# Illumina/Pisces

Hardware: AMD Instinct MI355X
Metric: candidate loci/s at 500x depth (higher is better)
Workload: dtype int32 counts + f64 likelihoods; 1 GPU; BASELINE config 2: synthetic 100000 loci x 500x amplicon pileup, SNV-only, gVCF, per GPU per step; device-resident packed tuples; depth=500, ring_batches=6, tile_loci=56, parallelism=interval-shard x1

## Files before the change

pisces_amd/csrc/device_math.hip.h:

```cpp
#pragma once
#include <hip/hip_runtime.h>
#include <stdint.h>

#include "../../include/pisces_hip.h"

namespace pisces {

struct DeviceParams {
    int32_t min_bq, noise_level, max_vq, min_vq, vq_filter, min_cov, low_depth_filter;
    int32_t min_gq, max_gq, low_gq_filter, sb_model, filter_single_strand, include_ref, emit_zero_cov;
    int32_t rmxn_max_len, rmxn_min_rep;
    float min_freq, vf_filter, gt_min_freq, target_lod, nocall_thr, rmxn_freq_limit;
    double sb_threshold;
    double err_q;
    double err_sb;
    double ln10;
    unsigned long long* totals;
    const double* q_to_p_lut;
    int32_t q_to_p_n;
    const double* gq_tail;
    int32_t gq_tail_a, gq_tail_cov;
    int32_t refs_only;
    int32_t variants_only;
    const int16_t* vq_tab;
    const double* sb_tab;
    const double* sb0_tab;
    const int16_t* gq_cap;
    int32_t vq_tab_k, sb_tab_k, tab_cov;
    const uint32_t* dirty_bits;
    int32_t dirty_first, dirty_n;
    int32_t* folded_out;
    int32_t folded_first, folded_n;
};

__device__ __forceinline__ bool locus_is_dirty(const DeviceParams& P, int pos)
{
    if (!P.dirty_bits) return false;
    const unsigned rel = (unsigned)(pos - P.dirty_first);
    return rel < (unsigned)P.dirty_n && ((P.dirty_bits[rel >> 5] >> (rel & 31u)) & 1u) != 0u;
}

__device__ __forceinline__ double lanczos_approximation(double p)
{
    double x = p;
    double tmp = x + 5.5;
    tmp = tmp - (x + 0.5) * log(tmp);
    double ser = 1.000000000190015 + 76.18009172947146 / (p + 1.0);
    ser -= 86.50532032941678 / (p + 2.0);
    ser += 24.01409824083091 / (p + 3.0);
    ser -= 1.231739572450155 / (p + 4.0);
    ser += 0.001208650973866179 / (p + 5.0);
    ser -= 5.395239384953E-06 / (p + 6.0);
    return (log(2.506628274631001 * ser / x) - tmp);
}

__device__ __forceinline__ double stirling_approximation(double n)
{
    return (0.5 * log(2.0 * 3.14159265358979323846) + (0.5 + n) * log(n) - n);
}

__device__ inline double gamma_continued_fraction(double a, double x, double g)
{
    const double kFpmin = 1.0E-50, kEpsilon = 1.0E-20;
    double b = x + 1.0 - a;
    double c = 1.0 / kFpmin;
    double d = 1.0 / b;
    double h = d;
    int i;
    for (i = 1; i <= 300; i++) {
        double an = i * (a - i);
        b += 2.0;
        d = an * d + b;
        if (fabs(d) < kFpmin) d = kFpmin;
        c = b + an / c;
        if (fabs(c) < kFpmin) c = kFpmin;
        d = 1.0 / d;
        double del = d * c;
        h *= del;
        if (fabs(del - 1.0) < kEpsilon) break;
    }
    if (i > 300) return -1.0;
    return exp(a * log(x) - x - g) * h;
}

__device__ inline double gamma_series(double a, double x, double g)
{
    const double kEpsilon = 1.0E-20;
    double retval = -1.0;
    if (x == 0.0) return 0.0;
    if (x < 0.0) return retval;
    double sum = 1.0 / a;
    double del = sum;
    bool done = false;
    for (int i = 1; i <= 300 && !done; i += 4) {
        const double ap0 = a + (double)i;
        const double q0 = x / ap0, q1 = x / (ap0 + 1.0), q2 = x / (ap0 + 2.0), q3 = x / (ap0 + 3.0);
        del *= q0; sum += del;
        if (fabs(del) < fabs(sum) * kEpsilon) { done = true; break; }
        del *= q1; sum += del;
        if (fabs(del) < fabs(sum) * kEpsilon) { done = true; break; }
        del *= q2; sum += del;
        if (fabs(del) < fabs(sum) * kEpsilon) { done = true; break; }
        del *= q3; sum += del;
        if (fabs(del) < fabs(sum) * kEpsilon) { done = true; break; }
    }
    if (done) retval = sum * exp(a * log(x) - x - g);
    return retval;
}

__device__ inline double incomplete_gamma_function(double a, double x)
{
// ... 69 lines not shown
    *gamma_ln_a = gl;
    double ax = (a * log(x)) - x - gl;
    if (ax < -709.78271289338399) return a < x ? 1.0 : 0.0;

    if (x <= 1 || x <= a) {
        double r2 = a, c2 = 1, ans2 = 1;
        do {
            r2 = r2 + 1;
            c2 = c2 * x / r2;
            ans2 += c2;
        } while ((c2 / ans2) > epsilon);
        return exp(ax) * ans2 / a;
    }

    int c = 0;
    double y = 1 - a;
    double z = x + y + 1;
    double p3 = 1, q3 = x, p2 = x + 1, q2 = z * x;
    double ans = p2 / q2;
    double error;
    do {
        c++;
        y += 1;
        z += 2;
        double yc = y * c;
        double p = (p2 * z) - (p3 * yc);
        double q = (q2 * z) - (q3 * yc);
        if (q != 0) {
            double nextans = p / q;
            error = fabs((ans - nextans) / nextans);
            ans = nextans;
        } else {
            error = 1;
        }
        p3 = p2; p2 = p; q3 = q2; q2 = q;
        if (fabs(p) > big) {
            p3 *= bigInv; p2 *= bigInv; q3 *= bigInv; q2 *= bigInv;
        }
    } while (error > epsilon);
    return 1.0 - (exp(ax) * ans);
}

struct QParams { int32_t max_vq; double ln10; };
__device__ inline int32_t poisson_qscore_core(int32_t callCount, int32_t coverage, double err, const QParams P)
{
    if ((callCount <= 0) || (coverage <= 0)) return 0;
    double callCountMinusOne = callCount - 1;
    double callCountDouble = callCount;
    double lambda = err * coverage;
    if (P.max_vq <= 110 && callCount >= 3 && callCountDouble >= 2.0 * lambda) {
        const double km1 = callCountMinusOne;
        const double need = ((double)P.max_vq + 1.0) * 0.23025850929940458 + 1e-3;
        const double r = km1 / lambda;
        if (km1 * (ln_lower_bound(r) - 1.0) >= need) return P.max_vq;
        if (km1 * (log(r) - 1.0) >= need) return P.max_vq;
    }
    double gamma_ln_k;
    double pValue = 1 - (1.0 - mathnet_gamma_lower_regularized(callCountMinusOne + 1, lambda, &gamma_ln_k));
    double rawQ;
    if (pValue > 0) {
        rawQ = p_to_q(pValue);
    } else {
        int k = (int)callCountMinusOne;
        const double fl = (k >= 171 && gamma_ln_k == gamma_ln_k) ? gamma_ln_k : mathnet_factorial_ln(k);
        double A = -lambda + (k * log(lambda)) - fl;
        double correction = (callCountDouble - lambda) / callCountDouble;
        rawQ = -10.0 * (A - log(2.0 * correction)) / P.ln10;
    }
    double qScore = fmin((double)P.max_vq, rawQ);
    qScore = fmax(qScore, 0.0);
    return (int32_t)rint(qScore);
}
__device__ inline int32_t poisson_qscore_e(int32_t callCount, int32_t coverage, double err, const DeviceParams& P)
{
    const QParams q = {P.max_vq, P.ln10};
    return poisson_qscore_core(callCount, coverage, err, q);
}
__device__ inline int32_t poisson_qscore(int32_t callCount, int32_t coverage, const DeviceParams& P)
{
    return poisson_qscore_e(callCount, coverage, P.err_q, P);
}
__device__ __forceinline__ double ln_ratio_lower_bound(double a, double x) { return (double)(ilogb(a) - ilogb(x) - 1) * 0.6931471805; }

__device__ __forceinline__ bool poisson_qscore_try(int32_t callCount, int32_t coverage, const DeviceParams& P, int32_t& vq)
{
    if ((callCount <= 0) || (coverage <= 0)) { vq = 0; return true; }
    if (P.vq_tab && callCount < P.vq_tab_k && coverage < P.tab_cov) {
        vq = P.vq_tab[(uint32_t)callCount * (uint32_t)P.tab_cov + (uint32_t)coverage];
        return true;
    }
    const double lambda = P.err_q * coverage;
    if (P.max_vq <= 110 && callCount >= 3 && (double)callCount >= 2.0 * lambda) {
        const double km1 = callCount - 1;
        const double need = ((double)P.max_vq + 1.0) * 0.23025850929940458 + 1e-3;
        if (km1 * (ln_ratio_lower_bound(km1, lambda) - 1.0) >= need) { vq = P.max_vq; return true; }
    }
    return false;
}

constexpr int32_t kNoLevel = (int32_t)0x80000000;
__device__ inline int32_t window_level(double sumOfBaseQuality, int totalCoverage)
{
    if (totalCoverage == 0) return kNoLevel;
    const double mean = sumOfBaseQuality / (double)totalCoverage;
    if (!(mean > 0.0) || isinf(mean)) return kNoLevel;
    return (int32_t)p_to_q(mean);
}
__device__ inline double window_err_of_level(int32_t level, const DeviceParams& P) { return level == kNoLevel ? -1.0 : q_to_p_int(level, P); }
__device__ inline double window_err(double sumOfBaseQuality, int totalCoverage, const DeviceParams& P)
{
    return window_err_of_level(window_level(sumOfBaseQuality, totalCoverage), P);
}
__device__ __forceinline__ int16_t noise_level_field(int32_t level) { return level == kNoLevel ? (int16_t)-32768 : (int16_t)level; }

struct SbStats { double var_gt_zero, false_pos, coverage, support; };

__device__ __noinline__ double mathnet_beta_regularized(double a, double b, double x)
{
    const double bt = (x == 0.0 || x == 1.0) ? 0.0
                      : exp(mathnet_gamma_ln(a + b) - mathnet_gamma_ln(a) - mathnet_gamma_ln(b) + (a * log(x)) + (b * log(1.0 - x)));
    const bool symmetryTransformation = x >= (a + 1.0) / (a + b + 2.0);
    const double eps = 1.1102230246251565e-16;
    const double fpmin = 4.9406564584124654e-324 / eps;
    if (symmetryTransformation) { x = 1.0 - x; const double swap = a; a = b; b = swap; }
    const double qab = a + b, qap = a + 1.0, qam = a - 1.0;
    double c = 1.0, d = 1.0 - (qab * x / qap);
    if (fabs(d) < fpmin) d = fpmin;
    d = 1.0 / d;
    double h = d;
    for (int m = 1, m2 = 2; m <= 50000; m++, m2 += 2) {
        double aa = m * (b - m) * x / ((qam + m2) * (a + m2));
        d = 1.0 + (aa * d); if (fabs(d) < fpmin) d = fpmin;
        c = 1.0 + (aa / c); if (fabs(c) < fpmin) c = fpmin;
        d = 1.0 / d;
        h *= d * c;
        aa = -(a + m) * (qab + m) * x / ((a + m2) * (qap + m2));
        d = 1.0 + (aa * d); if (fabs(d) < fpmin) d = fpmin;
        c = 1.0 + (aa / c); if (fabs(c) < fpmin) c = fpmin;
        d = 1.0 / d;
        const double del = d * c;
        h *= del;
        if (fabs(del - 1.0) <= eps) break;
    }
    return symmetryTransformation ? 1.0 - (bt * h / a) : bt * h / a;
}

template <bool kDiploidOk = false>
__device__ inline SbStats sb_create_stats(double support, double coverage, double noiseFreq, double minVariantFreq, int model)
{
    SbStats st;
    st.support = support;
    st.coverage = coverage;
    const double minDetectableSNP = (kDiploidOk && model == PISCES_SB_DIPLOID) ? minVariantFreq : noiseFreq;
    if (support == 0) {
        if (model == PISCES_SB_POISSON) {
            st.false_pos = 1;
            st.var_gt_zero = 0;
        } else {
            st.var_gt_zero = pow(1 - minDetectableSNP, coverage);
            st.false_pos = 1 - st.var_gt_zero;
        }
    } else if (kDiploidOk && model == PISCES_SB_DIPLOID) {
        const double frequency = coverage == 0 ? 0.0 : support / coverage;
        if (frequency >= minDetectableSNP) {
            st.var_gt_zero = 1;
            st.false_pos = 0;
        } else {
            const int n = (int)coverage;
            const double k = floor(support);
            const double cdf = support < 0.0 ? 0.0 : support > n ? 1.0 : mathnet_beta_regularized(n - k, k + 1, 1 - minDetectableSNP);
            st.var_gt_zero = fmax(cdf, 0.0);
            st.false_pos = fmax(0.0, 1 - poisson_cdf_sb(support, coverage * 0.1));
        }
    } else {
        st.var_gt_zero = fmax(0.0, poisson_cdf_sb(support - 1, coverage * noiseFreq));
        st.false_pos = fmax(0.0, 1 - st.var_gt_zero);
    }
    return st;
}

struct SbResult { double bias_score; int acceptable, var_both, cov_both; };

template <bool kDiploidOk = false>
__device__ __forceinline__ SbStats sb_stats_of(int which, const int32_t cov[3], const int32_t sup[3], const DeviceParams& P)
{
    const int s = which == 0 ? sup[0] + sup[1] + sup[2] : (which == 1 ? sup[0] + sup[2] / 2 : sup[1] + sup[2] / 2);
    const int c = which == 0 ? cov[0] + cov[1] + cov[2] : (which == 1 ? cov[0] + cov[2] / 2 : cov[1] + cov[2] / 2);
    return sb_create_stats<kDiploidOk>((double)s, (double)c, P.err_sb, (double)P.min_freq, P.sb_model);
}

__device__ __forceinline__ SbResult sb_combine(const SbStats& overall, const SbStats& fwd, const SbStats& rev, const DeviceParams& P)
{
    double forwardBias = (fwd.var_gt_zero * rev.false_pos) / overall.var_gt_zero;
    double reverseBias = (rev.var_gt_zero * fwd.false_pos) / overall.var_gt_zero;
    if (overall.var_gt_zero == 0) {
        forwardBias = 1;
        reverseBias = 1;
    }
    SbResult r;
    r.bias_score = forwardBias > reverseBias ? forwardBias : reverseBias;
    r.cov_both = (fwd.coverage > 0) && (rev.coverage > 0);
    r.var_both = (fwd.support > 0) && (rev.support > 0);
    if (!r.cov_both) r.bias_score = 0;
    r.acceptable = r.bias_score < P.sb_threshold;
    return r;
}

template <bool kDiploidOk = false>
__device__ inline SbResult strand_bias(const int32_t cov[3], const int32_t sup[3], const DeviceParams& P)
{
    const SbStats overall = sb_stats_of<kDiploidOk>(0, cov, sup, P);
    __builtin_amdgcn_sched_barrier(0);
    const SbStats fwd = sb_stats_of<kDiploidOk>(1, cov, sup, P);
    __builtin_amdgcn_sched_barrier(0);
    const SbStats rev = sb_stats_of<kDiploidOk>(2, cov, sup, P);
    __builtin_amdgcn_sched_barrier(0);
    return sb_combine(overall, fwd, rev, P);
}

__device__ __forceinline__ float frequency_f(int32_t support, int32_t coverage)
{
    if (coverage == 0) return 0.0f;
    float f = (float)support / (float)coverage;
    return f < 1.0f ? f : 1.0f;
}

__device__ inline int32_t somatic_genotype(bool isReference, int32_t cov, int32_t support, int32_t refSupport,
                                           const DeviceParams& P)
{
    if (cov < P.min_cov) return isReference ? PISCES_GT_REF_LIKE_NOCALL : PISCES_GT_ALT_LIKE_NOCALL;
    float freq = frequency_f(support, cov);
    if (!isReference) {
        if (frequency_f(refSupport, cov) < P.gt_min_freq) {
            if ((1 - freq) > P.gt_min_freq) return PISCES_GT_ALT_AND_NOCALL;
            return PISCES_GT_HOM_ALT;
        }
        return PISCES_GT_HET_ALT_REF;
    }
    if (freq < P.gt_min_freq) return PISCES_GT_REF_LIKE_NOCALL;
    if ((1 - freq) > P.gt_min_freq) return PISCES_GT_REF_AND_NOCALL;
    return PISCES_GT_HOM_REF;
}

__device__ __noinline__ double poisson_cdf_out_of_line(double num_occurrences, double expected)
{
    return poisson_cdf(num_occurrences, expected);
}

struct GqTail { double p2; bool used, floor; };
__device__ __forceinline__ GqTail somatic_gq_tail(int32_t genotype, int32_t cov, int32_t support, const DeviceParams& P)
{
    GqTail t = {0.0, false, false};
    if (cov == 0) return t;
    if ((genotype == PISCES_GT_HOM_REF) || (genotype == PISCES_GT_HOM_ALT)) {
        const float nonAlleleObservationsF = (1.0f - frequency_f(support, cov)) * (float)cov;
        const float expectedNonAllelObservationsF = P.target_lod * (float)cov;
        t.used = true;
        if (nonAlleleObservationsF >= expectedNonAllelObservationsF) { t.floor = true; return t; }
        const int ai = (int)((double)nonAlleleObservationsF + 1.0);
        if (P.gq_tail && ai >= 1 && ai < P.gq_tail_a && cov < P.gq_tail_cov)
            t.p2 = P.gq_tail[(size_t)ai * (size_t)P.gq_tail_cov + (size_t)cov];
        else
            t.p2 = poisson_cdf_out_of_line(nonAlleleObservationsF, expectedNonAllelObservationsF);
    }
    return t;
}

__device__ __forceinline__ int32_t somatic_gq_finish(int32_t genotype, int32_t variantQ, int32_t cov, const GqTail& t,
                                                     const DeviceParams& P)
{
    double rawQ = variantQ;
    bool noCall = (genotype == PISCES_GT_ALT12_LIKE_NOCALL || genotype == PISCES_GT_ALT_LIKE_NOCALL ||
                   genotype == PISCES_GT_REF_LIKE_NOCALL);
    if ((cov == 0) || noCall) return P.min_gq;
    if (t.used) {
        if (t.floor) return P.min_gq;
        double p1 = q_to_p_int(variantQ, P);
        rawQ = p_to_q(p1 + t.p2);
    }
    double qScore = fmin((double)P.max_gq, rawQ);
    qScore = fmax(qScore, (double)P.min_gq);
    return (int32_t)rint(qScore);
}

__device__ inline int32_t somatic_gq(int32_t genotype, int32_t variantQ, int32_t cov, int32_t support,
                                     const DeviceParams& P)
{
    const GqTail t = somatic_gq_tail(genotype, cov, support, P);
    return somatic_gq_finish(genotype, variantQ, cov, t, P);
}

__device__ __forceinline__ bool sb_stats_try(int32_t support, int32_t coverage, const DeviceParams& P, SbStats& st)
{
    st.support = (double)support;
    st.coverage = (double)coverage;
    if (support == 0) {
        if (P.sb_model == PISCES_SB_POISSON) {
            st.false_pos = 1;
            st.var_gt_zero = 0;
            return true;
        }
        if (!(P.sb0_tab && coverage >= 0 && coverage < P.tab_cov)) return false;
        st.var_gt_zero = P.sb0_tab[coverage];
        st.false_pos = 1 - st.var_gt_zero;
        return true;
    }
    if (P.sb_tab && support > 0 && support < P.sb_tab_k && coverage >= 0 && coverage < P.tab_cov) {
        st.var_gt_zero = P.sb_tab[(uint32_t)support * (uint32_t)P.tab_cov + (uint32_t)coverage];
    } else {
        const double a = (double)support, x = (double)coverage * P.err_sb;
        if (!(x > 0.0 && 2.0 * x <= a && a * (ln_ratio_lower_bound(a, x) - 1.0) + x > 51.0)) return false;
        st.var_gt_zero = 1.0;
    }
    st.false_pos = fmax(0.0, 1 - st.var_gt_zero);
    return true;
}

__device__ __forceinline__ bool strand_bias_try(const int32_t cov[3], const int32_t sup[3], const DeviceParams& P, double& bias_score,
                                                int& acceptable, int& var_both, int& cov_both)
{
    const int s2 = sup[2] / 2, c2 = cov[2] / 2;
    const int sf = sup[0] + s2, sr = sup[1] + s2, cf = cov[0] + c2, cr = cov[1] + c2;
    SbStats overall, fwd, rev;
    const bool ok0 = sb_stats_try(sup[0] + sup[1] + sup[2], cov[0] + cov[1] + cov[2], P, overall);
    const bool ok1 = sb_stats_try(sf, cf, P, fwd);
    const bool ok2 = sb_stats_try(sr, cr, P, rev);
    double forwardBias = 0.0, reverseBias = 0.0;
    if (!(fwd.false_pos == 0.0 && rev.false_pos == 0.0 && overall.var_gt_zero > 0.0)) {
        forwardBias = (fwd.var_gt_zero * rev.false_pos) / overall.var_gt_zero;
        reverseBias = (rev.var_gt_zero * fwd.false_pos) / overall.var_gt_zero;
        if (overall.var_gt_zero == 0) {
            forwardBias = 1;
            reverseBias = 1;
        }
    }
    double score = forwardBias > reverseBias ? forwardBias : reverseBias;
    cov_both = (cf > 0) && (cr > 0);
    var_both = (sf > 0) && (sr > 0);
    if (!cov_both) score = 0;
    bias_score = score;
    acceptable = score < P.sb_threshold;
    return ok0 && ok1 && ok2;
}

__device__ __forceinline__ int32_t somatic_gq_index(int32_t genotype, int32_t cov, int32_t support, const DeviceParams& P)
{
    if (cov == 0 || !((genotype == PISCES_GT_HOM_REF) || (genotype == PISCES_GT_HOM_ALT))) return -1;
    const float nonAlleleObservationsF = (1.0f - frequency_f(support, cov)) * (float)cov;
    const float expectedNonAllelObservationsF = P.target_lod * (float)cov;
    if (nonAlleleObservationsF >= expectedNonAllelObservationsF) return -1;
    const int ai = (int)((double)nonAlleleObservationsF + 1.0);
    if (ai >= 1 && ai < P.gq_tail_a && cov < P.gq_tail_cov) return ai * P.gq_tail_cov + cov;
    return -1;
}
__device__ __forceinline__ bool somatic_gq_try(int32_t genotype, int32_t variantQ, int32_t cov, int32_t support, const DeviceParams& P,
                                               int32_t gq_index, int32_t gq_cap_value , int32_t& gq)
{
    const bool noCall = (genotype == PISCES_GT_ALT12_LIKE_NOCALL || genotype == PISCES_GT_ALT_LIKE_NOCALL || genotype == PISCES_GT_REF_LIKE_NOCALL);
    if ((cov == 0) || noCall) { gq = P.min_gq; return true; }
    if ((genotype == PISCES_GT_HOM_REF) || (genotype == PISCES_GT_HOM_ALT)) {
        if (gq_index >= 0 && variantQ == P.max_vq && P.gq_cap) { gq = gq_cap_value; return true; }
        const float nonAlleleObservationsF = (1.0f - frequency_f(support, cov)) * (float)cov;
        const float expectedNonAllelObservationsF = P.target_lod * (float)cov;
        if (nonAlleleObservationsF >= expectedNonAllelObservationsF) { gq = P.min_gq; return true; }
        return false;
    }
    double qScore = fmin((double)P.max_gq, (double)variantQ);
    qScore = fmax(qScore, (double)P.min_gq);
    gq = (int32_t)rint(qScore);
    return true;
}

struct AlleleTables {
    int32_t vq;
    double sb[3];
    int32_t gq_cap;
    int32_t gq_idx;
    uint32_t have;
};
__device__ __forceinline__ bool tables_complete(const DeviceParams& P) { return P.vq_tab && P.sb_tab && P.sb0_tab && P.gq_cap; }

__device__ __forceinline__ AlleleTables request_allele_tables(bool isRef, int32_t support, int32_t total, int32_t refsup, const int32_t cov[3],
                                                              const int32_t sup[3], const DeviceParams& P)
{
    AlleleTables t;
    const uint32_t tab_cov = (uint32_t)P.tab_cov;
    const bool vq_in = support > 0 && total > 0 && support < P.vq_tab_k && total < P.tab_cov;
    const int16_t vq_v = P.vq_tab[vq_in ? (uint32_t)support * tab_cov + (uint32_t)total : 0u];
    const int s2 = sup[2] / 2, c2 = cov[2] / 2;
    const int ss[3] = {sup[0] + sup[1] + sup[2], sup[0] + s2, sup[1] + s2};
    const int cc[3] = {cov[0] + cov[1] + cov[2], cov[0] + c2, cov[1] + c2};
    double sb_v[3];
    uint32_t have = vq_in ? 1u : 0u;
#pragma unroll
    for (int w = 0; w < 3; w++) {
        const bool zero = ss[w] == 0;
        const bool in = zero ? (P.sb_model != PISCES_SB_POISSON && cc[w] >= 0 && cc[w] < P.tab_cov)
                             : (ss[w] > 0 && ss[w] < P.sb_tab_k && cc[w] >= 0 && cc[w] < P.tab_cov);
        const double* base = zero ? P.sb0_tab : P.sb_tab;
        const uint32_t idx = in ? (zero ? (uint32_t)cc[w] : (uint32_t)ss[w] * tab_cov + (uint32_t)cc[w]) : 0u;
        sb_v[w] = base[idx];
        have |= in ? (2u << w) : 0u;
    }
    t.gq_idx = somatic_gq_index(somatic_genotype(isRef, total, support, refsup, P), total, support, P);
    const int16_t gq_v = P.gq_cap[t.gq_idx >= 0 ? t.gq_idx : 0];
    t.vq = vq_v;
    t.sb[0] = sb_v[0]; t.sb[1] = sb_v[1]; t.sb[2] = sb_v[2];
    t.gq_cap = gq_v;
    t.have = have;
    return t;
}

__device__ __forceinline__ bool poisson_qscore_try(int32_t callCount, int32_t coverage, const DeviceParams& P, const AlleleTables& t, int32_t& vq)
{
    if ((callCount <= 0) || (coverage <= 0)) { vq = 0; return true; }
    if (t.have & 1u) { vq = t.vq; return true; }
    const double lambda = P.err_q * coverage;
    if (P.max_vq <= 110 && callCount >= 3 && (double)callCount >= 2.0 * lambda) {
        const double km1 = callCount - 1;
        const double need = ((double)P.max_vq + 1.0) * 0.23025850929940458 + 1e-3;
        if (km1 * (ln_ratio_lower_bound(km1, lambda) - 1.0) >= need) { vq = P.max_vq; return true; }
    }
    return false;
}

__device__ __forceinline__ bool sb_stats_try(int32_t support, int32_t coverage, const DeviceParams& P, bool have, double value, SbStats& st)
{
    st.support = (double)support;
    st.coverage = (double)coverage;
    if (support == 0) {
        if (P.sb_model == PISCES_SB_POISSON) {
            st.false_pos = 1;
            st.var_gt_zero = 0;
            return true;
        }
        if (!have) return false;
        st.var_gt_zero = value;
        st.false_pos = 1 - st.var_gt_zero;
        return true;
    }
    if (have) {
        st.var_gt_zero = value;
    } else {
        const double a = (double)support, x = (double)coverage * P.err_sb;
        if (!(x > 0.0 && 2.0 * x <= a && a * (ln_ratio_lower_bound(a, x) - 1.0) + x > 51.0)) return false;
        st.var_gt_zero = 1.0;
    }
    st.false_pos = fmax(0.0, 1 - st.var_gt_zero);
    return true;
}

__device__ __forceinline__ bool strand_bias_try(const int32_t cov[3], const int32_t sup[3], const DeviceParams& P, const AlleleTables& t,
                                                double& bias_score, int& acceptable, int& var_both, int& cov_both)
{
    const int s2 = sup[2] / 2, c2 = cov[2] / 2;
    const int sf = sup[0] + s2, sr = sup[1] + s2, cf = cov[0] + c2, cr = cov[1] + c2;
    SbStats overall, fwd, rev;
    const bool ok0 = sb_stats_try(sup[0] + sup[1] + sup[2], cov[0] + cov[1] + cov[2], P, (t.have & 2u) != 0, t.sb[0], overall);
    const bool ok1 = sb_stats_try(sf, cf, P, (t.have & 4u) != 0, t.sb[1], fwd);
    const bool ok2 = sb_stats_try(sr, cr, P, (t.have & 8u) != 0, t.sb[2], rev);
    double forwardBias = 0.0, reverseBias = 0.0;
    if (!(fwd.false_pos == 0.0 && rev.false_pos == 0.0 && overall.var_gt_zero > 0.0)) {
        forwardBias = (fwd.var_gt_zero * rev.false_pos) / overall.var_gt_zero;
        reverseBias = (rev.var_gt_zero * fwd.false_pos) / overall.var_gt_zero;
        if (overall.var_gt_zero == 0) {
            forwardBias = 1;
            reverseBias = 1;
        }
    }
    double score = forwardBias > reverseBias ? forwardBias : reverseBias;
    cov_both = (cf > 0) && (cr > 0);
    var_both = (sf > 0) && (sr > 0);
    if (!cov_both) score = 0;
    bias_score = score;
    acceptable = score < P.sb_threshold;
    return ok0 && ok1 && ok2;
}

__device__ __noinline__ int32_t poisson_qscore_out_of_line(int32_t callCount, int32_t coverage, double err, int32_t max_vq, double ln10)
{
    const QParams q = {max_vq, ln10};
    return poisson_qscore_core(callCount, coverage, err, q);
}
struct SbPair { double var_gt_zero, false_pos; };
__device__ __noinline__ SbPair sb_stats_out_of_line(double support, double coverage, double noiseFreq, int model)
{
    const SbStats st = sb_create_stats<false>(support, coverage, noiseFreq, 0.0, model);
    SbPair p = {st.var_gt_zero, st.false_pos};
    return p;
}
__device__ inline SbResult strand_bias_out_of_line(const int32_t cov[3], const int32_t sup[3], const DeviceParams& P)
{
    const int s2 = sup[2] / 2, c2 = cov[2] / 2;
    SbStats st[3];
#pragma unroll 1
    for (int which = 0; which < 3; which++) {
        const int s = which == 0 ? sup[0] + sup[1] + sup[2] : (which == 1 ? sup[0] + s2 : sup[1] + s2);
        const int c = which == 0 ? cov[0] + cov[1] + cov[2] : (which == 1 ? cov[0] + c2 : cov[1] + c2);
        const SbPair p = sb_stats_out_of_line((double)s, (double)c, P.err_sb, P.sb_model);
        st[which].var_gt_zero = p.var_gt_zero;
        st[which].false_pos = p.false_pos;
        st[which].support = (double)s;
        st[which].coverage = (double)c;
    }
    return sb_combine(st[0], st[1], st[2], P);
}

__device__ inline int rmxn_run(const uint8_t* ref, int64_t lo, int64_t hi, int64_t start, uint8_t base)
{
    int64_t back = start;
    while (back - 1 >= lo && ref[back - 1 - lo] == base) back--;
    int n = 0;
    int64_t cur = back;
    while (cur < hi && ref[cur - lo] == base) { n++; cur++; }
    return n;
}

__device__ inline bool rmxn_should_filter_snv(const uint8_t* ref, int64_t win_lo, int64_t win_hi, int32_t position,
                                              uint8_t refBase, uint8_t altBase, float freq, const DeviceParams& P)
{
    if (P.rmxn_max_len < 1) return false;
    if (freq >= P.rmxn_freq_limit) return false;
    int c1 = rmxn_run(ref, win_lo, win_hi, (int64_t)position - 1, refBase);
    int i1 = rmxn_run(ref, win_lo, win_hi, (int64_t)position, altBase);
    int i2 = rmxn_run(ref, win_lo, win_hi, (int64_t)position - 1, altBase);
    int c2 = i1 > i2 ? i1 : i2;
    return (c1 < c2 ? c1 : c2) >= P.rmxn_min_rep;
}

__device__ inline int rmxn_run_lds(const uint8_t* win, int n, int start, uint8_t base)
{
    int back = start;
    while (back - 1 >= 0 && win[back - 1] == base) back--;
    int cnt = 0;
    int cur = back;
    while (cur < n && win[cur] == base) { cnt++; cur++; }
    return cnt;
}

__device__ inline bool rmxn_should_filter_snv_lds(const uint8_t* win, int n, int idx ,
                                                  uint8_t refBase, uint8_t altBase, float freq, const DeviceParams& P)
{
    if (P.rmxn_max_len < 1) return false;
    if (freq >= P.rmxn_freq_limit) return false;
    if (idx >= 4 && idx + 4 < n) {
        const bool l1 = win[idx - 1] == refBase, l2 = win[idx - 2] == refBase, l3 = win[idx - 3] == refBase, l4 = win[idx - 4] == refBase;
        const bool r1 = win[idx + 1] == refBase, r2 = win[idx + 2] == refBase, r3 = win[idx + 3] == refBase, r4 = win[idx + 4] == refBase;
        const int left = !l1 ? 0 : !l2 ? 1 : !l3 ? 2 : !l4 ? 3 : 4;
        const int right = !r1 ? 0 : !r2 ? 1 : !r3 ? 2 : !r4 ? 3 : 4;
        if (left < 4 && right < 4 && 1 + left + right < P.rmxn_min_rep) return false;
    }
    int c1 = rmxn_run_lds(win, n, idx, refBase);
    if (c1 < P.rmxn_min_rep) return false;
    int i1 = rmxn_run_lds(win, n, idx + 1, altBase);
    int i2 = rmxn_run_lds(win, n, idx, altBase);
    int c2 = i1 > i2 ? i1 : i2;
    return (c1 < c2 ? c1 : c2) >= P.rmxn_min_rep;
}

}
```

pisces_amd/csrc/kernels.hip.h:

```cpp
#pragma once
#include <hip/hip_runtime.h>
#include <stdint.h>

#include "device_math.hip.h"
#include "genotype_core.h"

namespace pisces {

constexpr int kBlock = 256;
constexpr int kTile = 64;
constexpr int kFolded = 18;
constexpr int kUnroll = 8;
constexpr int kSlotsPerTile = 4 * kTile;
#ifndef PISCES_TOTAL_SHARDS
#define PISCES_TOTAL_SHARDS 64
#endif
constexpr int kTotalShards = PISCES_TOTAL_SHARDS;
constexpr int kTotalStride = 16;
constexpr int kRefMargin = 32;
constexpr int kRefWin = kTile + 2 * kRefMargin;
constexpr int kWaveRows = 32;
constexpr int kWaveRow = kTile;
constexpr int kWaveRegion = kWaveRows * kWaveRow;
constexpr int kQLutLds = 128;

typedef uint32_t u32x4 __attribute__((ext_vector_type(4)));

__device__ __forceinline__ int allele_of_rank(int k) { return k == 1 ? 2 : (k == 2 ? 1 : k); }
__device__ __forceinline__ int rank_of_allele(int a) { return a == 1 ? 2 : (a == 2 ? 1 : a); }

__device__ __forceinline__ int allele_type_of_base(uint8_t c)
{
    return c == 'A' ? 0 : c == 'G' ? 1 : c == 'C' ? 2 : c == 'T' ? 3 : 4;
}

__device__ __forceinline__ void accumulate_folded(int* hist, uint32_t t, uint32_t n_loci, uint32_t min_bq)
{
    uint32_t locus = PISCES_TUPLE_LOCUS(t);
    uint32_t dir = PISCES_TUPLE_DIR(t);
    uint32_t allele = PISCES_TUPLE_ALLELE(t);
    uint32_t qual = PISCES_TUPLE_QUAL(t);
    if (allele < 4u && qual < min_bq) allele = 4u;
    if (locus < n_loci && dir < 3u && allele < 6u) atomicAdd(&hist[(allele * 3u + dir) * kTile + locus], 1);
}

__device__ __forceinline__ void accumulate_wave(int* hist, uint32_t t, uint32_t min_bq_shifted)
{
    const uint32_t region = (t < min_bq_shifted) ? (uint32_t)(kWaveRegion * sizeof(int)) : 0u;
    const uint32_t off = (t & 0x1FFCu) | region;
    atomicAdd(reinterpret_cast<int*>(reinterpret_cast<char*>(hist) + off), 1);
}

template <typename Op>
__device__ __forceinline__ void stream_tuples(const uint32_t* __restrict__ tuples, int64_t begin, int64_t end, Op op)
{
    const int tid = threadIdx.x;
    int64_t abegin = (begin + 3) & ~(int64_t)3;
    int64_t aend = end & ~(int64_t)3;
    if (abegin > aend) { abegin = end; aend = end; }
    for (int64_t i = begin + tid; i < abegin; i += kBlock) op(tuples[i]);
    const u32x4* __restrict__ p4 = reinterpret_cast<const u32x4*>(tuples + abegin);
    const int64_t n4 = (aend - abegin) >> 2;
    for (int64_t i = tid; i < n4; i += (int64_t)kBlock * kUnroll) {
        u32x4 v[kUnroll];
#pragma unroll
        for (int u = 0; u < kUnroll; u++) {
            int64_t j = i + (int64_t)u * kBlock;
            v[u] = j < n4 ? __builtin_nontemporal_load(&p4[j]) : (u32x4){~0u, ~0u, ~0u, ~0u};
        }
#pragma unroll
        for (int u = 0; u < kUnroll; u++) {
            op(v[u].x); op(v[u].y); op(v[u].z); op(v[u].w);
        }
    }
    for (int64_t i = aend + tid; i < end; i += kBlock) op(tuples[i]);
}

__device__ __forceinline__ void copy_record(PiscesCalledAllele* dst, const PiscesCalledAllele* src)
{
    const unsigned long long sb = (unsigned long long)__double_as_longlong(src->strand_bias_score);
    uint4* dp = reinterpret_cast<uint4*>(dst);
    dp[0] = make_uint4((uint32_t)src->position, (uint32_t)src->total_coverage, (uint32_t)src->allele_support, (uint32_t)src->reference_support);
    dp[1] = make_uint4((uint32_t)src->num_no_calls, (uint32_t)src->coverage_by_dir[0], (uint32_t)src->coverage_by_dir[1], (uint32_t)src->coverage_by_dir[2]);
    dp[2] = make_uint4((uint32_t)src->support_by_dir[0], (uint32_t)src->support_by_dir[1], (uint32_t)src->support_by_dir[2], (uint32_t)src->variant_qscore);
    dp[3] = make_uint4((uint32_t)sb, (uint32_t)(sb >> 32), (uint32_t)(uint16_t)src->genotype_qscore | ((uint32_t)(uint16_t)src->noise_level << 16), (uint32_t)src->filter_bits | ((uint32_t)src->info << 16));
}

struct PointCounts {
    int cov[3], sup[3];
    int total, nocalls, refsup, support;
};

struct HistBlock {
    static __device__ __forceinline__ int idx(int a, int d, int l) { return (a * 3 + d) * kTile + l; }
};
struct HistWave {
    static __device__ __forceinline__ int idx(int a, int d, int l) { return (a * 4 + d) * kWaveRow + (int)PISCES_TUPLE_COLUMN(l, d); }
};

struct HistLinear {
    static __device__ __forceinline__ int idx(int a, int d, int l) { return (a * 4 + d) * kWaveRow + l; }
};

struct LocusCounts { int h[6][3]; };

template <typename H = HistBlock>
__device__ __forceinline__ LocusCounts load_counts(const int* hist, int l)
{
    LocusCounts lc;
#pragma unroll
    for (int k = 0; k < kFolded; k++) lc.h[k / 3][k % 3] = hist[H::idx(k / 3, k % 3, l)];
    return lc;
}

template <typename HistWave = pisces::HistWave>
__device__ __forceinline__ LocusCounts load_counts_wave(const int* hist, int l)
{
    LocusCounts lc;
#pragma unroll
    for (int d = 0; d < 3; d++) {
        int low = 0;
#pragma unroll
        for (int a = 0; a < 5; a++) low += hist[kWaveRegion + HistWave::idx(a, d, l)];
#pragma unroll
        for (int a = 0; a < 4; a++) lc.h[a][d] = hist[HistWave::idx(a, d, l)];
        lc.h[PISCES_ALLELE_N][d] = hist[HistWave::idx(PISCES_ALLELE_N, d, l)] + low;
        lc.h[PISCES_ALLELE_DEL][d] = hist[HistWave::idx(PISCES_ALLELE_DEL, d, l)] + hist[kWaveRegion + HistWave::idx(PISCES_ALLELE_DEL, d, l)];
    }
    return lc;
}

__device__ __forceinline__ PointCounts point_counts_of(const LocusCounts& lc, int allele, bool isRef, int refType, int gapped)
{
    PointCounts c;
    const int (&h)[6][3] = lc.h;
    c.total = 0; c.nocalls = 0; c.refsup = 0;
    const int supAllele = isRef ? refType : allele;
#pragma unroll
    for (int d = 0; d < 3; d++) {
        c.cov[d] = h[PISCES_ALLELE_A][d] + h[PISCES_ALLELE_C][d] + h[PISCES_ALLELE_G][d] + h[PISCES_ALLELE_T][d] +
                   h[PISCES_ALLELE_DEL][d];
        c.total += c.cov[d];
        c.nocalls += h[PISCES_ALLELE_N][d];
        c.sup[d] = 0;
    }
#pragma unroll
    for (int a = 0; a < 6; a++) {
        if (a == refType && a < PISCES_ALLELE_N) c.refsup += h[a][0] + h[a][1] + h[a][2];
        if (a == supAllele) { c.sup[0] = h[a][0]; c.sup[1] = h[a][1]; c.sup[2] = h[a][2]; }
    }
    c.support = c.sup[0] + c.sup[1] + c.sup[2];
    if (isRef) { c.support -= gapped; if (c.support < 0) c.support = 0; }
    else { c.refsup -= gapped; if (c.refsup < 0) c.refsup = 0; }
    return c;
}

template <typename H = HistBlock>
__device__ __forceinline__ PointCounts point_counts(const int* hist, int l, int allele, bool isRef, int refType, int gapped)
{
    return point_counts_of(load_counts<H>(hist, l), allele, isRef, refType, gapped);
}

__device__ __forceinline__ bool variant_passes_frequency(const PointCounts& c, const DeviceParams& P)
{
    if (c.total < P.min_cov && !P.include_ref) return false;
    if (c.total != 0 && frequency_f(c.support, c.total) < P.min_freq) return false;
    return true;
}

struct GqPre { int32_t idx, val; };
template <bool kMemo = false>
__device__ inline bool finish_allele(const PointCounts& c, int pos, int a, bool isRef, int rt, int vq, const SbResult& sb,
                                     const uint8_t* __restrict__ ref, int64_t win_lo, int64_t win_hi, const DeviceParams& P,
                                     PiscesCalledAllele& r, const uint8_t* s_refwin, int s_refidx,
                                     const GqTail* pre_tail = nullptr, const GqPre* pre_gq = nullptr,
                                     const int32_t* window_level_ = nullptr )
{
    const float freq = frequency_f(c.support, c.total);
    const float allReads = (float)(c.total + c.nocalls);
    const float fractionNoCalls = (allReads == 0.0f) ? 0.0f : ((float)c.nocalls / allReads);
    uint32_t filters = 0;
    if (P.low_depth_filter >= 0 && c.total < P.low_depth_filter) filters |= 1u << PISCES_FILTER_LOW_DEPTH;
    if (P.vq_filter >= 0 && vq < P.vq_filter && c.total != 0) filters |= 1u << PISCES_FILTER_LOW_VARIANT_QSCORE;
    if (!isRef) {
        if (P.nocall_thr >= 0.0f && fractionNoCalls > P.nocall_thr) filters |= 1u << PISCES_FILTER_NO_CALL;
        if (!sb.acceptable || (P.filter_single_strand && !sb.var_both)) filters |= 1u << PISCES_FILTER_STRAND_BIAS;
        auto base_of = [](int code) { return (uint8_t)((0x54434741u >> (8 * code)) & 0xFFu); };
        if (rt < 4 && a < 4) {
            const bool hit = (s_refwin && P.rmxn_min_rep <= kRefMargin)
                                 ? rmxn_should_filter_snv_lds(s_refwin, kRefWin, s_refidx, base_of(rt), base_of(a), freq, P)
                                 : rmxn_should_filter_snv(ref, win_lo, win_hi, pos, base_of(rt), base_of(a), freq, P);
            if (hit) filters |= 1u << PISCES_FILTER_RMXN;
        }
        if (P.vf_filter >= 0.0f && freq < P.vf_filter) filters |= 1u << PISCES_FILTER_LOW_VARIANT_FREQUENCY;
    }
    const int gt = somatic_genotype(isRef, c.total, c.support, c.refsup, P);
    int gq;
    if (kMemo) {
        GqPre g;
        if (pre_gq) g = *pre_gq;
        else {
            g.idx = somatic_gq_index(gt, c.total, c.support, P);
            g.val = (g.idx >= 0 && P.gq_cap) ? (int32_t)P.gq_cap[g.idx] : 0;
        }
        if (!somatic_gq_try(gt, vq, c.total, c.support, P, g.idx, g.val, gq)) return false;
    } else {
        gq = pre_tail ? somatic_gq_finish(gt, vq, c.total, *pre_tail, P) : somatic_gq(gt, vq, c.total, c.support, P);
    }
    if (P.low_gq_filter >= 0 && (float)gq < (float)P.low_gq_filter) filters |= 1u << PISCES_FILTER_LOW_GENOTYPE_QUALITY;

    r.position = pos;
    r.total_coverage = c.total;
    r.allele_support = c.support;
    r.reference_support = c.refsup;
    r.num_no_calls = c.nocalls;
    r.coverage_by_dir[0] = c.cov[0]; r.coverage_by_dir[1] = c.cov[1]; r.coverage_by_dir[2] = c.cov[2];
    r.support_by_dir[0] = c.sup[0]; r.support_by_dir[1] = c.sup[1]; r.support_by_dir[2] = c.sup[2];
    r.variant_qscore = vq;
    r.strand_bias_score = sb.bias_score;
    r.genotype_qscore = (int16_t)gq;
    r.noise_level = c.support > 0 ? (window_level_ ? noise_level_field(*window_level_) : (int16_t)P.noise_level) : (int16_t)0;
    r.filter_bits = (uint16_t)filters;
    r.info = PISCES_INFO_PACK(gt, isRef ? PISCES_CAT_REFERENCE : PISCES_CAT_SNV, rt, isRef ? rt : a, sb.acceptable, sb.var_both,
                              sb.cov_both);
    return true;
}

template <bool kDiploidOk = false, bool kFinishAnyway = false>
__device__ inline bool process_point_allele(const PointCounts& c, int pos, int a, bool isRef, int rt,
                                             const uint8_t* __restrict__ ref, int64_t win_lo, int64_t win_hi,
                                             const DeviceParams& P, PiscesCalledAllele& r,
                                             const uint8_t* s_refwin = nullptr, int s_refidx = 0, const GqTail* pre_tail = nullptr,
                                             const int32_t* window_level_ = nullptr )
{
    bool callable = true;
    if (!isRef && !variant_passes_frequency(c, P)) {
        if (!kFinishAnyway) return false;
        callable = false;
    }
    int vq = 0;
    if (window_level_) {
        const double werr = window_err_of_level(*window_level_, P);
        if (c.support > 0 && c.total != 0 && werr >= 0.0) vq = poisson_qscore_e(c.support, c.total, werr, P);
    } else if (c.support > 0 && c.total != 0) {
        vq = poisson_qscore(c.support, c.total, P);
    }
    if (!isRef && vq < P.min_vq) {
        if (!kFinishAnyway) return false;
        callable = false;
    }
    SbResult sb = {0.0, 0, 0, 0};
    if (c.support > 0) sb = strand_bias<kDiploidOk>(c.cov, c.sup, P);
    finish_allele(c, pos, a, isRef, rt, vq, sb, ref, win_lo, win_hi, P, r, s_refwin, s_refidx, pre_tail, nullptr, window_level_);
    return callable;
}

struct VarScratch {
    int vq[kTile * 4];
    double ov_var[kTile * 4], fw_var[kTile * 4], fw_fp[kTile * 4], rv_var[kTile * 4], rv_fp[kTile * 4];
};

__device__ inline void call_roles(const int* hist, const uint32_t* gapped , const int32_t* s_lvl , const PiscesTile& tile,
                                  int tile_index, const uint8_t* __restrict__ ref, int32_t ref_start, int64_t ref_len,
                                  PiscesCalledAllele* __restrict__ records, PiscesTileResult* __restrict__ tile_result,
                                  const DeviceParams& P, uint8_t* s_mask ,
                                  const uint8_t* s_refwin , VarScratch* vs)
{
    const int wave = threadIdx.x >> 6;
    if (wave == 3) return;
    const int l = threadIdx.x & 63;
    const int pos = tile.start_position + l;
    const uint8_t refb = s_refwin[kRefMargin + l];
    const bool in_ref = l < tile.n_loci && refb != 0;
    const int rt = in_ref ? allele_type_of_base(refb) : PISCES_ALLELE_N;
    const int64_t win_lo = (int64_t)ref_start - 1, win_hi = win_lo + ref_len;
    const int g = gapped ? (int)gapped[l] : 0;
    PiscesCalledAllele* const slots = records + (int64_t)tile_index * kSlotsPerTile + l * 4;

    uint32_t pass_mask = 0;
    if (in_ref && rt < 4 && !P.refs_only && !locus_is_dirty(P, pos)) {
        for (int k = 0; k < 4; k++) {
            const int a = allele_of_rank(k);
            if (a == rt) continue;
            if (hist[(a * 3 + 0) * kTile + l] + hist[(a * 3 + 1) * kTile + l] + hist[(a * 3 + 2) * kTile + l] == 0) continue;
            const PointCounts c = point_counts(hist, l, a, false, rt, g);
            if (variant_passes_frequency(c, P)) pass_mask |= 1u << k;
        }
    }
    const bool tile_has_variants = __ballot(pass_mask != 0) != 0ull;
    if (!tile_has_variants && wave != 0) return;

    bool ref_emitted = false;
    int ref_rank = 0;
    if (wave == 0) {
        if (in_ref && P.include_ref) {
            int all = 0;
#pragma unroll
            for (int c = 0; c < kFolded; c++) all += hist[c * kTile + l];
            if (P.emit_zero_cov || all > 0) {
                const int a = (rt < 4) ? rt : PISCES_ALLELE_N;
                ref_rank = (rt < 4) ? rank_of_allele(rt) : 0;
                const PointCounts c = point_counts(hist, l, a, true, rt, g);
                PiscesCalledAllele rec;
                (void)process_point_allele<true>(c, pos, a, true, rt, ref, win_lo, win_hi, P, rec, s_refwin, kRefMargin + l, nullptr, s_lvl ? &s_lvl[l] : nullptr);
                copy_record(&slots[ref_rank], &rec);
                ref_emitted = true;
            }
// ... 164 lines not shown
#pragma unroll
        for (int u = 0; u < kWaveUnroll; u++) { op(v[u].x); op(v[u].y); op(v[u].z); op(v[u].w); }
    };
    const bool streams = (uint32_t)wid < nb;
    if (NW == 2) {
        if (streams) load(cur, (uint32_t)__builtin_amdgcn_readfirstlane(wid));
        __builtin_amdgcn_sched_barrier(0);
        pre();
    } else {
        pre();
        if (streams) load(cur, (uint32_t)__builtin_amdgcn_readfirstlane(wid));
    }
    for (int64_t i = begin + tid; i < abegin; i += 64 * NW) op(tuples[i]);
    if (streams) {
        uint32_t b = (uint32_t)__builtin_amdgcn_readfirstlane(wid);
        const uint32_t m = (nb - b + NW - 1) / NW;
        for (uint32_t p = (m - 1) / 2; p > 0; p--) {
            load(nxt, b + NW);
            __builtin_amdgcn_sched_barrier(0);
            consume(cur);
            __builtin_amdgcn_sched_barrier(0);
            load(cur, b + 2 * NW);
            __builtin_amdgcn_sched_barrier(0);
            consume(nxt);
            __builtin_amdgcn_sched_barrier(0);
            b += 2 * NW;
        }
        if (((m - 1) & 1u) != 0) {
            load(nxt, b + NW);
            __builtin_amdgcn_sched_barrier(0);
            consume(cur);
            __builtin_amdgcn_sched_barrier(0);
#pragma unroll
            for (int u = 0; u < kWaveUnroll; u++) cur[u] = nxt[u];
            b += NW;
        }
        if (b == nb - 1 && (n4 % kBatch)) {
#pragma unroll
            for (int u = 0; u < kWaveUnroll; u++)
                if (b * kBatch + (uint32_t)u * 64u + (uint32_t)lane >= n4) cur[u] = (u32x4){~0u, ~0u, ~0u, ~0u};
        }
        consume(cur);
    }
    for (int64_t i = aend + tid; i < end; i += 64 * NW) op(tuples[i]);
}

__device__ __forceinline__ void wave_lds_sync()
{
    __builtin_amdgcn_fence(__ATOMIC_SEQ_CST, "workgroup");
    __builtin_amdgcn_wave_barrier();
}

template <typename H = HistWave>
__device__ __forceinline__ uint32_t slow_alleles(const int* hist, const uint8_t* s_refwin, uint32_t slow, int l, int pos, int rt, int ref_rank,
                                                 const uint8_t* __restrict__ ref, int64_t win_lo, int64_t win_hi, PiscesCalledAllele* slots,
                                                 const DeviceParams& P)
{
    uint32_t called = 0;
    const int ref_a = (rt < 4) ? rt : PISCES_ALLELE_N;
#pragma unroll 1
    for (int k = 0; k < 5; k++) {
        if (!((slow >> k) & 1u)) continue;
        const bool isRef = k == 4;
        const int a = isRef ? ref_a : allele_of_rank(k);
        const LocusCounts lc = load_counts_wave<H>(hist, l);
        const PointCounts c = point_counts_of(lc, a, isRef, rt, 0);
        int vq = 0;
        if (c.support > 0 && c.total != 0) vq = poisson_qscore_out_of_line(c.support, c.total, P.err_q, P.max_vq, P.ln10);
        if (!isRef && vq < P.min_vq) continue;
        SbResult sb = {0.0, 0, 0, 0};
        if (c.support > 0) sb = strand_bias_out_of_line(c.cov, c.sup, P);
        PiscesCalledAllele r;
        (void)finish_allele<false>(c, pos, a, isRef, rt, vq, sb, ref, win_lo, win_hi, P, r, s_refwin, kRefMargin + l);
        copy_record(&slots[isRef ? ref_rank : k], &r);
        if (!isRef) called |= 1u << k;
    }
    return called;
}

template <int NW, typename H = HistWave>
__device__ __forceinline__ void call_phase_wave(const int* hist, const uint8_t* s_refwin, uint8_t* s_vmask, const PiscesTile& tile, const int t,
                                                const int l, const int wid, const uint8_t* __restrict__ ref, const int32_t ref_start,
                                                const int64_t ref_len, PiscesCalledAllele* __restrict__ records,
                                                PiscesTileResult* __restrict__ tile_results, const DeviceParams& P
#ifdef PISCES_TIMING
                                                , const long long tc0, const long long tc1
#endif
                                                )
{
    const int pos = tile.start_position + l;
    const uint8_t refb = s_refwin[kRefMargin + l];
    const bool in_ref = l < tile.n_loci && refb != 0;
    const int rt = in_ref ? allele_type_of_base(refb) : PISCES_ALLELE_N;
    const int64_t win_lo = (int64_t)ref_start - 1, win_hi = win_lo + ref_len;
    auto slot_of = [&](int k) { return records + ((int64_t)t * kSlotsPerTile + l * 4 + k); };
    const bool dirty = locus_is_dirty(P, pos);
    const LocusCounts lc = load_counts_wave<H>(hist, l);
    const bool ref_wave = wid == 0, var_wave = wid == NW - 1;
    if (P.folded_out && ref_wave && l < tile.n_loci) {
        const unsigned rel = (unsigned)(pos - P.folded_first);
        if (rel < (unsigned)P.folded_n) {
            int32_t* const dst = P.folded_out + (size_t)rel * PISCES_FOLDED_PER_LOCUS;
#pragma unroll
            for (int a = 0; a < 6; a++)
#pragma unroll
                for (int d = 0; d < 3; d++) dst[a * 3 + d] = lc.h[a][d];
        }
    }

    const bool tabs = tables_complete(P);
    auto fast_allele = [&](const PointCounts& c, int a, bool isRef, PiscesCalledAllele& rec) -> bool {
        int vq = 0;
        double sb_score = 0.0;
        int sb_ok = 0, sb_var = 0, sb_cov = 0;
        if (!tabs) return false;
        const AlleleTables tb = request_allele_tables(isRef, c.support, c.total, c.refsup, c.cov, c.sup, P);
        if (c.support > 0 && c.total != 0 && !poisson_qscore_try(c.support, c.total, P, tb, vq)) return false;
        if (!isRef && vq < P.min_vq) return true;
        if (c.support > 0 && !strand_bias_try(c.cov, c.sup, P, tb, sb_score, sb_ok, sb_var, sb_cov)) return false;
        const GqPre g = {tb.gq_idx, tb.gq_cap};
        const SbResult sb = {sb_score, sb_ok, sb_var, sb_cov};
        if (!finish_allele<true>(c, pos, a, isRef, rt, vq, sb, ref, win_lo, win_hi, P, rec, s_refwin, kRefMargin + l, nullptr, &g)) return false;
        return true;
    };
    bool ref_emitted = false;
    int ref_rank = 0;
    uint32_t slow = 0;
    uint32_t vmask = 0;
    const int ref_a = (rt < 4) ? rt : PISCES_ALLELE_N;
    if (ref_wave) {
        const PointCounts c = point_counts_of(lc, ref_a, true, rt, 0);
        if (in_ref && P.include_ref && !P.variants_only && (P.emit_zero_cov || c.total + c.nocalls > 0)) {
            ref_rank = (rt < 4) ? rank_of_allele(rt) : 0;
            ref_emitted = true;
            PiscesCalledAllele rec;
            if (fast_allele(c, ref_a, true, rec)) copy_record(slot_of(ref_rank), &rec);
            else slow |= 16u;
        }
    }
#ifdef PISCES_TIMING
    const long long tcA = wall_clock64();
#endif
    if (var_wave && in_ref && rt < 4 && !P.refs_only && !dirty) {
#pragma unroll 1
        for (int k = 0; k < 4; k++) {
            const int a = allele_of_rank(k);
            if (a == rt) continue;
            const PointCounts c = point_counts_of(lc, a, false, rt, 0);
            if (c.support == 0) continue;
            if (!variant_passes_frequency(c, P)) continue;
            PiscesCalledAllele r;
            r.position = 0;
            if (!fast_allele(c, a, false, r)) { slow |= 1u << k; continue; }
            if (r.position == 0) continue;
            copy_record(slot_of(k), &r);
            vmask |= 1u << k;
        }
    }
    if (__builtin_expect(__ballot(slow != 0) != 0ull, 0))
        vmask |= slow_alleles<H>(hist, s_refwin, slow, l, pos, rt, ref_rank, ref, win_lo, win_hi, records + ((int64_t)t * kSlotsPerTile + l * 4), P);
    if (NW == 2) {
        if (var_wave) s_vmask[l] = (uint8_t)vmask;
        __syncthreads();
        if (!ref_wave) return;
        vmask = s_vmask[l];
    }
#ifdef PISCES_TIMING
    const long long tcB = wall_clock64();
#endif

    const uint32_t valid = vmask ? vmask : (ref_emitted ? (1u << ref_rank) : 0u);
    int n_surv = 0, n_var = 0;
#pragma unroll
    for (int k = 0; k < 4; k++) {
        n_surv += __popcll(__ballot((valid >> k) & 1u));
        n_var += __popcll(__ballot((vmask >> k) & 1u));
    }
    const int n_call_total = n_var + __popcll(__ballot(ref_emitted));
    const int n_loci_called = __popcll(__ballot(valid != 0));
    uint32_t word = valid << ((l & 7) * 4);
    word |= __shfl_xor(word, 1, 64);
    word |= __shfl_xor(word, 2, 64);
    word |= __shfl_xor(word, 4, 64);
    PiscesTileResult* const tile_result = &tile_results[t];
    if ((l & 7) == 0) tile_result->valid[l >> 3] = word;
    if (l == 0) {
        tile_result->record_begin = t * kSlotsPerTile;
        tile_result->n_records = n_surv;
        tile_result->n_candidate_loci = n_loci_called;
        tile_result->n_called = n_call_total;
        if (P.totals) {
            unsigned long long* tt = P.totals + (size_t)(t % kTotalShards) * kTotalStride;
            atomicAdd(&tt[0], (unsigned long long)n_surv);
            atomicAdd(&tt[1], (unsigned long long)n_loci_called);
            atomicAdd(&tt[2], (unsigned long long)n_call_total);
            atomicAdd(&tt[3], 1ull);
        }
#ifdef PISCES_TIMING
        const long long tc2 = wall_clock64();
        tile_result->record_begin = (int)(tc0 & 0x3FFFFFFF);
        tile_result->n_records = (int)(tc1 & 0x3FFFFFFF);
        tile_result->n_candidate_loci = (int)(tc2 & 0x3FFFFFFF);
        tile_result->n_called = (int)__builtin_amdgcn_s_getreg(63492);
        tile_result->valid[0] = __builtin_amdgcn_s_getreg(63508);
        tile_result->valid[1] = 0;
        tile_result->valid[2] = (uint32_t)(tcA - tc1);
        tile_result->valid[3] = (uint32_t)(tcB - tcA);
        tile_result->valid[4] = 0;
        tile_result->valid[5] = (uint32_t)(tc2 - tcB);
#endif
    }
}

template <int NW>
__global__ __launch_bounds__(64 * NW, NW == 1 ? PISCES_WAVE_OCC : PISCES_WAVE2_OCC) void call_tiles_wave_kernel(
    const uint32_t* __restrict__ tuples, const PiscesTile* __restrict__ tiles, int32_t n_tiles,
    const uint8_t* __restrict__ ref, int32_t ref_start, int64_t ref_len, PiscesCalledAllele* __restrict__ records,
    PiscesTileResult* __restrict__ tile_results, DeviceParams P, const DeviceParams* __restrict__ Pd )
{
    __shared__ __attribute__((aligned(16))) int hist[2 * kWaveRegion];
    __shared__ uint8_t s_refwin[kRefWin];
    __shared__ uint8_t s_vmask[kTile];

    const int t = blockIdx.x;
    if (t >= n_tiles) return;
    const int l = threadIdx.x & 63, wid = threadIdx.x >> 6;
    const PiscesTile tile = tiles[t];
#ifdef PISCES_TIMING
    const long long tc0 = wall_clock64();
#endif
    auto setup = [&]() {
        int4* h4 = reinterpret_cast<int4*>(hist);
        for (int i = threadIdx.x; i < 2 * kWaveRegion / 4; i += 64 * NW) h4[i] = make_int4(0, 0, 0, 0);
        for (int i = threadIdx.x; i < kRefWin; i += 64 * NW) {
            const int64_t ri = (int64_t)tile.start_position - kRefMargin + i - ref_start;
            s_refwin[i] = (ri >= 0 && ri < ref_len) ? ref[ri] : (uint8_t)0;
        }
        __syncthreads();
    };

    {
        if (NW == 2) __builtin_amdgcn_s_setprio(3);
        const uint32_t min_bq_shifted = (uint32_t)min(max(P.min_bq, 0), 255) << 24;
        stream_tuples_wave<NW>(tuples, tile.tuple_begin, tile.tuple_end, l, wid, [&](uint32_t v) { accumulate_wave(hist, v, min_bq_shifted); }, setup);
    }
    __syncthreads();
    if (NW == 2) __builtin_amdgcn_s_setprio(0);
#ifdef PISCES_TIMING
    const long long tc1 = wall_clock64();
#endif

    call_phase_wave<NW>(hist, s_refwin, s_vmask, tile, t, l, wid, ref, ref_start, ref_len, records, tile_results, P
#ifdef PISCES_TIMING
                        , tc0, tc1
#endif
                        );
}

__global__ __launch_bounds__(256) void build_vq_tab_kernel(int16_t* __restrict__ tab, int32_t n_k, int32_t n_cov, DeviceParams P)
{
    const int64_t i = (int64_t)blockIdx.x * blockDim.x + threadIdx.x;
    if (i >= (int64_t)n_k * n_cov) return;
    tab[i] = (int16_t)poisson_qscore((int32_t)(i / n_cov), (int32_t)(i % n_cov), P);
}
__global__ __launch_bounds__(256) void build_sb_tab_kernel(double* __restrict__ tab, double* __restrict__ tab0, int32_t n_k, int32_t n_cov, DeviceParams P)
{
    const int64_t i = (int64_t)blockIdx.x * blockDim.x + threadIdx.x;
    if (i >= (int64_t)n_k * n_cov) return;
    const int k = (int)(i / n_cov), cov = (int)(i % n_cov);
    tab[i] = k >= 1 ? fmax(0.0, poisson_cdf_sb((double)k - 1, (double)cov * P.err_sb)) : 0.0;
    if (k == 0) tab0[cov] = pow(1 - P.err_sb, (double)cov);
}
__global__ __launch_bounds__(256) void build_gq_cap_kernel(int16_t* __restrict__ tab, const double* __restrict__ gq_tail, int32_t n_a, int32_t n_cov, DeviceParams P)
{
    const int64_t i = (int64_t)blockIdx.x * blockDim.x + threadIdx.x;
    if (i >= (int64_t)n_a * n_cov) return;
    if (i < n_cov) { tab[i] = 0; return; }
    double rawQ = p_to_q(q_to_p_int(P.max_vq, P) + gq_tail[i]);
    double qScore = fmin((double)P.max_gq, rawQ);
    qScore = fmax(qScore, (double)P.min_gq);
    tab[i] = (int16_t)rint(qScore);
}

__global__ __launch_bounds__(64) void totals_collect_kernel(unsigned long long* __restrict__ shards, unsigned long long* __restrict__ out_host, int reset)
{
    const int l = threadIdx.x;
    if (l < 4) {
        unsigned long long v = 0;
        for (int sh = 0; sh < kTotalShards; sh++) v += shards[sh * kTotalStride + l];
        out_host[l] = v;
    }
    if (reset)
        for (int i = l; i < kTotalShards * kTotalStride; i += 64) shards[i] = 0ull;
    __threadfence_system();
}

__global__ __launch_bounds__(256) void read_probe_kernel(const u32x4* __restrict__ p, int64_t n4, uint32_t* __restrict__ sink)
{
    uint32_t acc = 0;
    const int64_t stride = (int64_t)gridDim.x * blockDim.x * 8;
    for (int64_t i = (int64_t)blockIdx.x * blockDim.x * 8 + threadIdx.x; i < n4; i += stride) {
        u32x4 v[8];
#pragma unroll
        for (int u = 0; u < 8; u++) {
            const int64_t j = i + (int64_t)u * blockDim.x;
            v[u] = j < n4 ? __builtin_nontemporal_load(&p[j]) : (u32x4){0u, 0u, 0u, 0u};
        }
#pragma unroll
        for (int u = 0; u < 8; u++) acc ^= v[u].x ^ v[u].y ^ v[u].z ^ v[u].w;
    }
    if (acc == 0x9E3779B9u) *sink = acc;
}

__global__ __launch_bounds__(256) void read_probe_dword_kernel(const uint32_t* __restrict__ p, int64_t n, uint32_t* __restrict__ sink)
{
    uint32_t acc = 0;
    const int64_t stride = (int64_t)gridDim.x * blockDim.x * 8;
    for (int64_t i = (int64_t)blockIdx.x * blockDim.x * 8 + threadIdx.x; i < n; i += stride) {
        uint32_t v[8];
#pragma unroll
        for (int u = 0; u < 8; u++) {
            const int64_t j = i + (int64_t)u * blockDim.x;
            v[u] = j < n ? p[j] : 0u;
        }
#pragma unroll
        for (int u = 0; u < 8; u++) acc ^= v[u];
    }
    if (acc == 0x9E3779B9u) *sink = acc;
}

__global__ void build_gq_tail_kernel(double* __restrict__ table, int32_t n_a, int32_t n_cov, float target_lod)
{
    const int64_t i = (int64_t)blockIdx.x * blockDim.x + threadIdx.x;
    if (i >= (int64_t)n_a * n_cov) return;
    const int a = (int)(i / n_cov), cov = (int)(i % n_cov);
    const float expectedF = target_lod * (float)cov;
    table[i] = a >= 1 ? incomplete_gamma_function((double)a, (double)expectedF) : -1.0;
}

template <typename T, typename R>
__host__ __device__ inline R anchor_adjusted(const T* __restrict__ row, int minAnchor, int maxAnchor, bool fromEnd)
{
    const int wellAnchoredIndex = PISCES_ANCHOR_SIZE, numAnchorIndexes = PISCES_NUM_ANCHORS;
    const int trueMinAnchor = wellAnchoredIndex < minAnchor ? wellAnchoredIndex : minAnchor;
    int initialMaxAnchor = wellAnchoredIndex;
    if (maxAnchor >= 0) {
        if (maxAnchor >= wellAnchoredIndex) initialMaxAnchor = wellAnchoredIndex - 1;
        if (maxAnchor < wellAnchoredIndex) initialMaxAnchor = maxAnchor;
    }
    R tot = 0;
    if (fromEnd) {
        for (int i = trueMinAnchor; i <= initialMaxAnchor; i++) tot += row[numAnchorIndexes - i - 1];
        if (maxAnchor < 0)
            for (int i = 0; i < initialMaxAnchor; i++) tot += row[i];
// ... 751 lines not shown
```

pisces_amd/csrc/pisces_hip.hip:

```cpp
#include <hip/hip_runtime.h>
#include <hip/hip_ext.h>
#include <dlfcn.h>
#include <link.h>

#include <algorithm>
#include <array>
#include <cctype>
#include <memory>
#include <cmath>
#include <cstdio>
#include <cstdlib>
#include <cstring>
#include <deque>
#include <ctime>
#include <map>
#include <set>
#include <string>
#include <atomic>
#include <chrono>
#include <mutex>
#include <thread>
#include <unordered_map>
#include <unordered_set>
#include <vector>
// ... 186 lines not shown
            if (e == hipSuccess) e = hipStreamSynchronize(stream);
        }
        if (old) dev_free(old);
        p = fresh;
        cap = want;
        return e;
    }
    void release()
    {
        if (p) dev_free(p);
        p = nullptr;
        cap = 0;
    }
    void swap(DeviceBuf& o)
    {
        std::swap(p, o.p);
        std::swap(cap, o.cap);
    }
};

struct ReadSegment {
    DeviceBuf<uint8_t> blob;
    DeviceBuf<uint8_t> bases, quals, dirs, cop;
    DeviceBuf<uint8_t> codes;
    DeviceBuf<uint32_t> clen;
    DeviceBuf<ReadDesc> desc;
    DeviceBuf<ReadExt> ext;
    DeviceBuf<ReadDesc> frag;
    DeviceBuf<int32_t> grid;
    int64_t grid_base = 0, grid_n = 0;
    bool grid_ok = false;
    int32_t* state = nullptr;
    const uint8_t *v_bases = nullptr, *v_quals = nullptr, *v_dirs = nullptr, *v_cop = nullptr, *v_codes = nullptr;
    const uint32_t* v_clen = nullptr;
    int64_t n_reads = 0, n_bases = 0, n_ops = 0;
    int64_t n_floored = 0, n_floored_ops = 0;
    int32_t floor = 0;
    int32_t max_key = 0;
    bool open = false;
};

}

struct PiscesHip {
    PiscesHipConfig cfg;
    DeviceParams P;
    int device = 0;
    hipStream_t stream = nullptr;
    static constexpr int kLanes = 3;
    hipStream_t lane[kLanes] = {nullptr, nullptr, nullptr};
    hipEvent_t ev0 = nullptr, ev1 = nullptr;
    std::vector<hipEvent_t> ring;
    int32_t timing = 0;
    bool chain_timing = false;
    hipEvent_t ev_chain[4] = {nullptr, nullptr, nullptr, nullptr};
    bool chain_have[2] = {false, false};
    bool chain_enqueued_since = false;
    bool chain_add_open = false;
    int64_t ring_used = 0;
    int64_t launches_seen = 0;
    DeviceBuf<unsigned long long> d_totals;
    unsigned long long* h_totals = nullptr;
    bool foreign_stream_used = false;
    bool foreign_stream_ever = false;
    bool exact_total_called = false;
    DeviceBuf<PiscesTile> d_tiles_x;
    DeviceBuf<PiscesTileResult> d_tr_x;
    DeviceBuf<PiscesCalledAllele> d_rec_x;
    DeviceBuf<int32_t> d_cnt_x, d_off_x;
    int32_t* h_cnt_x = nullptr;
    bool tables_shareable = false;
    bool poisoned = false;
    std::string poison_why;
    uint8_t* h_prep = nullptr;
    DeviceBuf<double> d_qlut;
    DeviceBuf<ulonglong2> d_bq_lut;
    DeviceBuf<unsigned long long> d_sumq_fix;
    DeviceBuf<double> d_sumq;
    DeviceBuf<double> d_gq_tail;
    DeviceBuf<int16_t> d_vq_tab;
    DeviceBuf<double> d_sb_tab;
    DeviceBuf<double> d_sb0_tab;
    DeviceBuf<int16_t> d_gq_cap;
    DeviceBuf<DeviceParams> d_params;
    int n_cus = 256;
    void* comm = nullptr;
    int comm_world = 1;
    DeviceBuf<long long> d_summary;
    DeviceBuf<int32_t> d_offsets;
    DeviceBuf<PiscesCalledAllele> d_compact;
    DeviceBuf<PiscesGenotypePosteriors> d_post, d_post_compact;
    int kernel_variant = 4;
    std::string err;

    DeviceBuf<uint8_t> d_ref;
    std::vector<uint8_t> h_ref;
    int64_t ref_len = 0;
    DeviceBuf<DevCandidate> d_cands;
    DeviceBuf<uint8_t> d_alleles;
    DeviceBuf<PiscesCalledAllele> d_cand_records;
    DeviceBuf<uint8_t> d_cand_callable;
    int32_t* h_counts = nullptr;
    size_t h_counts_cap = 0;

    std::map<int32_t, BlockObs> blocks;
    int32_t last_block_key_cache = 0;
    BlockObs* last_block = nullptr;
    int32_t last_up_to_block_key = 0;
    std::unordered_map<int32_t, int32_t> gapped_mnv_ref;
    std::vector<HostCandidate> known_variants;
    bool exclude_mnvs_from_collapsing = false;
    std::vector<HostCandidate> forced;
    size_t n_forced_added = 0;
    std::set<std::string> forced_keys;
    std::set<int32_t> forced_positions;
    std::vector<std::pair<int32_t, int32_t>> intervals;
    int32_t own_lo = 1, own_hi = 0x7FFFFFFF;
    int64_t stats[4] = {0, 0, 0, 0};
    double prof[24] = {0};
    bool prof_on = false;
    int64_t pcie[4] = {0, 0, 0, 0};
    double host_time[4] = {0, 0, 0, 0};

    struct FlushResult {
        bool valid = false;
        int32_t up_to = 0;
        PiscesCalledAllele* view = nullptr;
        size_t n_view = 0;
        std::vector<PiscesCalledAllele> rows;
        std::vector<int32_t> index;
        std::vector<PiscesGenotypePosteriors> posteriors;
        std::vector<HostCandidate> cands;
        std::vector<PiscesCandidate> exported;
        std::vector<uint8_t> alleles;
        std::vector<int32_t> keys;
        int64_t called = 0, collapsed = 0;
        bool dropped = false;
        unsigned long long kept = 0;
        const PiscesCalledAllele* data() const { return view ? view : rows.data(); }
        size_t size() const { return view ? n_view : rows.size(); }
        void clear()
        {
            valid = dropped = false;
            view = nullptr;
            n_view = 0;
            rows.clear(); index.clear(); posteriors.clear(); cands.clear(); exported.clear(); alleles.clear(); keys.clear();
            called = collapsed = 0;
            kept = 0;
        }
    } result;

    DeviceBuf<int32_t> d_log_pos[2];
    DeviceBuf<uint32_t> d_log_tup[2];
    int log_cur = 0;
    DeviceBuf<unsigned long long> d_log_n;
    int64_t log_ub = 0;
    std::vector<long long> read_slots;
    std::vector<int32_t> found_slots_host;
    DeviceBuf<int32_t> d_flags;
    struct Stage {
        DeviceBuf<uint8_t> d;
        uint8_t* h = nullptr;
        size_t h_cap = 0;
        hipEvent_t done = nullptr;
        bool in_flight = false;
    } stage[2];
// ... 200 lines not shown
        int e2 = 0;
        const double m = std::frexp(x, &e2);
        const unsigned long long mant = (unsigned long long)std::ldexp(m, 53);
        const int shift = e2 - 53 + 2 * kSumqHalfBits;
        const unsigned __int128 v = shift >= 0 ? (unsigned __int128)mant << shift : (shift > -64 ? (unsigned __int128)mant >> (-shift) : (unsigned __int128)0);
        lut[(size_t)q].x = (unsigned long long)(v >> kSumqHalfBits);
        lut[(size_t)q].y = (unsigned long long)(v & (((unsigned __int128)1 << kSumqHalfBits) - 1));
    }
    hipError_t e = h->d_bq_lut.reserve(256);
    if (e == hipSuccess) e = hipMemcpy(h->d_bq_lut.p, lut.data(), 256 * sizeof(ulonglong2), hipMemcpyHostToDevice);
    return e;
}

static void store_view(PiscesHip* h, StoreView* V);
static hipError_t accumulate_tiles(PiscesHip* h, hipStream_t s, const uint32_t* d_tuples, const PiscesTile* d_tiles, int32_t n_tiles, bool with_sums,
                                   bool with_store = false)
{
    const size_t nc = (size_t)n_tiles * kTile * PISCES_COUNTS_PER_LOCUS;
    hipError_t e = h->d_counts.reserve(nc);
    if (e == hipSuccess && with_sums) e = h->d_sumq.reserve(nc);
    if (e == hipSuccess && with_sums) e = h->d_sumq_fix.reserve(2 * nc);
    if (e == hipSuccess && with_sums) e = ensure_quality_lut(h);
    if (e != hipSuccess) return e;
    (void)hipMemsetAsync(h->d_counts.p, 0, nc * sizeof(int32_t), s);
    if (with_sums) (void)hipMemsetAsync(h->d_sumq_fix.p, 0, 2 * nc * sizeof(unsigned long long), s);
    if (with_store && h->read_path == 1) {
        StoreView V;
        store_view(h, &V);
        const int split = (int)std::min<int64_t>(16, std::max<int64_t>(1, 2 * (int64_t)h->n_cus / std::max(n_tiles, 1)));
        hipLaunchKernelGGL(accumulate_store_tiles_kernel, dim3((unsigned)n_tiles, (unsigned)split), dim3(kBlock), 0, s, V, d_tuples, d_tiles, n_tiles, h->d_counts.p,
                           h->cfg.min_base_call_quality, with_sums ? h->d_sumq_fix.p : (unsigned long long*)nullptr,
                           with_sums ? (const ulonglong2*)h->d_bq_lut.p : (const ulonglong2*)nullptr);
    } else
    hipLaunchKernelGGL(accumulate_tiles_kernel, dim3((unsigned)n_tiles), dim3(kBlock), 0, s, d_tuples, d_tiles, n_tiles, h->d_counts.p,
                       h->cfg.min_base_call_quality, with_sums ? h->d_sumq_fix.p : (unsigned long long*)nullptr,
                       with_sums ? (const ulonglong2*)h->d_bq_lut.p : (const ulonglong2*)nullptr);
    if (with_sums)
        hipLaunchKernelGGL(finish_quality_sums_kernel, dim3((unsigned)((nc + 255) / 256)), dim3(256), 0, s, h->d_sumq_fix.p, h->d_sumq.p, (int64_t)nc);
    return hipGetLastError();
}

static DeviceParams make_params(const PiscesHipConfig& c)
{
    DeviceParams P;
    P.min_bq = c.min_base_call_quality;
    P.noise_level = c.noise_level;
    P.max_vq = c.max_variant_qscore;
    P.min_vq = c.min_variant_qscore;
    P.vq_filter = c.variant_qscore_filter;
    P.min_cov = c.min_coverage;
    P.low_depth_filter = c.low_depth_filter;
    P.min_gq = c.min_genotype_qscore;
    P.max_gq = c.max_genotype_qscore;
    P.low_gq_filter = c.low_gq_filter;
    P.sb_model = c.strand_bias_model;
    P.filter_single_strand = c.filter_single_strand;
    P.include_ref = c.include_reference_calls;
    P.emit_zero_cov = c.emit_zero_coverage_refs;
    P.rmxn_max_len = c.rmxn_max_repeat_length;
    P.rmxn_min_rep = c.rmxn_min_repetitions;
    P.min_freq = c.min_frequency;
    P.vf_filter = c.variant_freq_filter;
    P.gt_min_freq = c.genotype_min_freq_filter;
    P.target_lod = c.target_lod_frequency;
    P.nocall_thr = c.no_call_filter_threshold;
    P.rmxn_freq_limit = c.rmxn_frequency_limit;
    P.sb_threshold = (double)c.strand_bias_threshold;
    P.err_q = std::pow(10.0, -1 * (double)c.noise_level / 10.0);
    P.err_sb = std::pow(10.0, (double)((float)(-1 * c.noise_level) / 10.0f));
    P.ln10 = std::log(10.0);
    P.totals = nullptr;
    P.q_to_p_lut = nullptr;
    P.q_to_p_n = 0;
    P.gq_tail = nullptr;
    P.gq_tail_a = 0;
    P.gq_tail_cov = 0;
    P.refs_only = c.call_mnvs ? 1 : 0;
    P.variants_only = 0;
    P.vq_tab = nullptr;
    P.sb_tab = nullptr;
    P.sb0_tab = nullptr;
    P.gq_cap = nullptr;
    P.vq_tab_k = P.sb_tab_k = P.tab_cov = 0;
    P.dirty_bits = nullptr;
    P.dirty_first = P.dirty_n = 0;
    P.folded_out = nullptr;
    P.folded_first = P.folded_n = 0;
    return P;
}

template <typename R, typename F>
static R abi_guard(PiscesHip* h, F&& body)
{
    try {
        return body();
    } catch (const std::exception& e) {
        return (R)fail(h, PISCES_E_INTERNAL, std::string("exception inside the library: ") + e.what());
    } catch (...) {
        return (R)fail(h, PISCES_E_INTERNAL, "unknown exception inside the library");
    }
}

namespace {
struct TableSet {
    PiscesHipConfig cfg;
    int device = 0;
    DeviceBuf<double> gq_tail, sb_tab, sb0_tab;
    DeviceBuf<int16_t> vq_tab, gq_cap;
};
std::mutex g_tables_mu;
std::vector<TableSet*>& table_cache() { static std::vector<TableSet*>* v = new std::vector<TableSet*>(); return *v; }
TableSet* take_tables(const PiscesHipConfig& cfg, int device)
{
    std::lock_guard<std::mutex> lock(g_tables_mu);
    auto& v = table_cache();
    for (size_t i = 0; i < v.size(); i++)
        if (v[i]->device == device && std::memcmp(&v[i]->cfg, &cfg, sizeof(cfg)) == 0) {
            TableSet* t = v[i];
            v.erase(v.begin() + (std::ptrdiff_t)i);
            return t;
        }
    return nullptr;
}
void leave_tables(TableSet* t)
{
    std::lock_guard<std::mutex> lock(g_tables_mu);
    auto& v = table_cache();
    v.push_back(t);
    if (v.size() > 8) { delete v.front(); v.erase(v.begin()); }
}
}

extern "C" {

int32_t pisces_hip_abi_version(void) { return PISCES_HIP_ABI_VERSION; }

int32_t pisces_hip_default_config(PiscesHipConfig* c)
{
    return abi_guard<int32_t>((PiscesHip*)nullptr, [&]() -> int32_t {
    if (!c) return PISCES_E_INVALID_ARG;
    std::memset(c, 0, sizeof(*c));
    c->abi_version = PISCES_HIP_ABI_VERSION;
    c->min_base_call_quality = 20;
    c->noise_level = 20;
    c->max_variant_qscore = 100;
    c->min_variant_qscore = 20;
    c->variant_qscore_filter = 30;
    c->min_coverage = 10;
    c->low_depth_filter = 10;
    c->min_genotype_qscore = 0;
    c->max_genotype_qscore = 100;
    c->low_gq_filter = -1;
    c->strand_bias_model = PISCES_SB_EXTENDED;
    c->filter_single_strand = 0;
    c->include_reference_calls = 1;
    c->emit_zero_coverage_refs = 0;
    c->expect_stitched_reads = 0;
    c->tile_loci = kTile;
    c->block_size = 1000;
    c->min_frequency = 0.01f;
    c->variant_freq_filter = 0.01f;
    c->genotype_min_freq_filter = 0.01f;
    c->target_lod_frequency = 0.01f;
    c->strand_bias_threshold = 0.5f;
    c->no_call_filter_threshold = 0.6f;
    c->rmxn_max_repeat_length = 5;
    c->rmxn_min_repetitions = 9;
    c->rmxn_frequency_limit = 0.35f;
    c->collapse = 1;
    c->collapse_freq_threshold = 0.0f;
    c->collapse_freq_ratio_threshold = 0.5f;
    c->call_mnvs = 0;
    c->max_mnv_length = 3;
    c->max_gap_between_mnv = 1;
    c->noise_model = PISCES_NOISE_FLAT;
    c->ploidy = PISCES_PLOIDY_SOMATIC;
    c->diploid_snv_params[0] = c->diploid_indel_params[0] = 0.20f;
    c->diploid_snv_params[1] = c->diploid_indel_params[1] = 0.70f;
    c->diploid_snv_params[2] = c->diploid_indel_params[2] = 0.80f;
    return PISCES_OK;
    });
}

int32_t pisces_hip_destroy(PiscesHip* h);

int32_t pisces_hip_device_count(void)
{
    int ndev = 0;
    const hipError_t e = hipGetDeviceCount(&ndev);
    if (e != hipSuccess) { g_create_error = std::string("pisces_hip_device_count: ") + hipGetErrorString(e); return PISCES_E_DEVICE; }
    return ndev;
// ... 17 lines not shown
    hipError_t e = hipGetDeviceCount(&ndev);
    if (e != hipSuccess || ndev <= 0)
        return fail(nullptr, PISCES_E_DEVICE, std::string("pisces_hip_create: no HIP device: ") + hipGetErrorString(e));
    if (device < 0 || device >= ndev) return fail(nullptr, PISCES_E_INVALID_ARG, "pisces_hip_create: device index out of range");
    PiscesHip* h = new PiscesHip();
    h->cfg = *cfg;
    h->cfg.tile_loci = kTile;
    h->P = make_params(h->cfg);
    adaptive_default_params(h->adaptive);
    h->device = device;
    if ((e = hipSetDevice(device)) != hipSuccess || (e = hipStreamCreateWithFlags(&h->stream, hipStreamNonBlocking)) != hipSuccess ||
        (e = hipEventCreate(&h->ev0)) != hipSuccess || (e = hipEventCreate(&h->ev1)) != hipSuccess) {
        g_create_error = std::string("pisces_hip_create: ") + hipGetErrorString(e);
        delete h;
        return PISCES_E_DEVICE;
    }
    if ((e = h->d_totals.reserve((size_t)kTotalShards * kTotalStride)) != hipSuccess ||
        (e = hipMemsetAsync(h->d_totals.p, 0, (size_t)kTotalShards * kTotalStride * sizeof(unsigned long long), h->stream)) != hipSuccess ||
        (e = hipStreamSynchronize(h->stream)) != hipSuccess) {
        g_create_error = std::string("pisces_hip_create: ") + hipGetErrorString(e);
        pisces_hip_destroy(h);
        return PISCES_E_DEVICE;
    }
    h->P.totals = h->d_totals.p;
    {
        hipDeviceProp_t prop;
        if (hipGetDeviceProperties(&prop, device) == hipSuccess && prop.multiProcessorCount > 0) h->n_cus = prop.multiProcessorCount;
        const char* kv = getenv("PISCES_HIP_KERNEL");
        if (kv && std::string(kv) == "wave") h->kernel_variant = 2;
        if (kv && std::string(kv) == "wave2") h->kernel_variant = 3;
        if (kv && std::string(kv) == "auto") h->kernel_variant = 4;
        if (kv && std::string(kv) == "block") h->kernel_variant = 0;
        h->prof_on = getenv("PISCES_HIP_HOST_PROFILE") != nullptr;
        const char* rp = getenv("PISCES_HIP_READ_PATH");
        if (rp && std::string(rp) == "log") h->read_path = 0;
        if (const char* v = getenv("PISCES_HIP_STORE_DIRECT_BYTES")) h->store_direct_bytes = (size_t)std::max(0ll, atoll(v));
        if (const char* v = getenv("PISCES_HIP_STORE_WAVES")) h->store_waves = atoi(v);
        if (const char* v = getenv("PISCES_HIP_TILE_ORDER")) h->trade_tiles = atoi(v) != 0;
        if (const char* v = getenv("PISCES_HIP_DEVICE_MERGE")) h->device_merge = atoi(v) != 0 ? 1 : 0;
        h->snv_walk = h->cfg.call_mnvs != 0 || (h->cfg.collapse != 0 && (h->cfg.collapse_freq_threshold > 0.0f || h->cfg.collapse_freq_ratio_threshold >= 1.0f));
        h->mnv_split = h->snv_walk && h->device_merge != 0;
        if (const char* v = getenv("PISCES_HIP_MNV_SPLIT")) h->mnv_split = h->mnv_split && atoi(v) != 0;
        if (const char* v = getenv("PISCES_HIP_STORE_SEAL_BYTES")) h->store_seal_bytes = (size_t)std::max(0ll, atoll(v));
        if (const char* v = getenv("PISCES_HIP_DEVICE_CHECKS")) h->device_checks = atoi(v) != 0 ? 1 : 0;
        if (const char* v = getenv("PISCES_HIP_TILE_LOCI")) h->tile_loci = atoi(v);
        if (const char* v = getenv("PISCES_HIP_DEFER_GRID")) h->defer_grid = atoi(v) != 0;
        if (const char* v = getenv("PISCES_HIP_COMPACT")) h->compact_mode = std::string(v) == "two" ? 2 : std::string(v) == "lookback" ? 3 : 0;
        if (const char* v = getenv("PISCES_HIP_MERGE_IN_PLACE")) h->merge_in_place = atoi(v) != 0;
        if (const char* v = getenv("PISCES_HIP_DEVICE_GENOTYPER")) h->device_genotyper = atoi(v) != 0;
        if (const char* v = getenv("PISCES_HIP_FINDER")) h->finder_bases = std::string(v) == "bases";
    }
    {
        const int n = std::min(std::max(h->cfg.max_variant_qscore, 0), 4095) + 1;
        std::vector<double> lut((size_t)n);
        for (int q = 0; q < n; q++) lut[(size_t)q] = std::pow(10.0, -1 * (double)q / 10.0);
        if ((e = h->d_qlut.reserve((size_t)n)) != hipSuccess ||
            (e = hipMemcpy(h->d_qlut.p, lut.data(), (size_t)n * sizeof(double), hipMemcpyHostToDevice)) != hipSuccess) {
            g_create_error = std::string("pisces_hip_create: ") + hipGetErrorString(e);
            pisces_hip_destroy(h);
            return PISCES_E_DEVICE;
        }
        h->P.q_to_p_lut = h->d_qlut.p;
        h->P.q_to_p_n = n;
    }
    if (h->cfg.noise_model == PISCES_NOISE_WINDOW) {
        if ((e = ensure_quality_lut(h)) != hipSuccess) {
            g_create_error = std::string("pisces_hip_create: ") + hipGetErrorString(e);
            pisces_hip_destroy(h);
            return PISCES_E_DEVICE;
        }
    }
    if ((e = h->d_log_n.reserve(4)) != hipSuccess || (e = h->d_flags.reserve(4)) != hipSuccess ||
        (e = hipMemset(h->d_log_n.p, 0, 4 * sizeof(unsigned long long))) != hipSuccess ||
        (e = hipMemset(h->d_flags.p, 0, 4 * sizeof(int32_t))) != hipSuccess) {
        g_create_error = std::string("pisces_hip_create: ") + hipGetErrorString(e);
        pisces_hip_destroy(h);
        return PISCES_E_DEVICE;
    }
    const bool tables_by_default = !getenv("PISCES_HIP_NO_GQ_TABLE") && !getenv("PISCES_HIP_NO_CALL_TABLES") && h->cfg.noise_model == PISCES_NOISE_FLAT &&
                                   h->cfg.strand_bias_model != PISCES_SB_DIPLOID && h->cfg.max_variant_qscore <= 32767 && h->cfg.max_genotype_qscore <= 32767 &&
                                   h->cfg.min_genotype_qscore >= -32768;
    std::unique_ptr<TableSet> kept(tables_by_default ? take_tables(h->cfg, h->device) : nullptr);
    if (kept) {
        h->d_gq_tail.swap(kept->gq_tail); h->d_vq_tab.swap(kept->vq_tab); h->d_sb_tab.swap(kept->sb_tab); h->d_sb0_tab.swap(kept->sb0_tab); h->d_gq_cap.swap(kept->gq_cap);
        h->P.gq_tail = h->d_gq_tail.p; h->P.gq_tail_a = 32; h->P.gq_tail_cov = 8192;
        h->P.vq_tab = h->d_vq_tab.p; h->P.sb_tab = h->d_sb_tab.p; h->P.sb0_tab = h->d_sb0_tab.p; h->P.gq_cap = h->d_gq_cap.p;
        h->P.vq_tab_k = h->P.sb_tab_k = 256;
        h->P.tab_cov = 8192;
        h->tables_shareable = true;
    }
    if (!kept && !getenv("PISCES_HIP_NO_GQ_TABLE")) {
        const int32_t n_a = 32, n_cov = 8192;
        if ((e = h->d_gq_tail.reserve((size_t)n_a * n_cov)) != hipSuccess) {
            g_create_error = std::string("pisces_hip_create: ") + hipGetErrorString(e);
            pisces_hip_destroy(h);
            return PISCES_E_DEVICE;
        }
        hipLaunchKernelGGL(build_gq_tail_kernel, dim3((unsigned)((n_a * n_cov + 255) / 256)), dim3(256), 0, h->stream, h->d_gq_tail.p,
                           n_a, n_cov, h->P.target_lod);
        if ((e = hipGetLastError()) != hipSuccess || (e = hipStreamSynchronize(h->stream)) != hipSuccess) {
            g_create_error = std::string("pisces_hip_create: ") + hipGetErrorString(e);
            pisces_hip_destroy(h);
            return PISCES_E_DEVICE;
        }
        h->P.gq_tail = h->d_gq_tail.p;
        h->P.gq_tail_a = n_a;
        h->P.gq_tail_cov = n_cov;
    }
    if (!kept && !getenv("PISCES_HIP_NO_CALL_TABLES") && h->cfg.noise_model == PISCES_NOISE_FLAT && h->cfg.strand_bias_model != PISCES_SB_DIPLOID &&
        h->cfg.max_variant_qscore <= 32767 && h->cfg.max_genotype_qscore <= 32767 && h->cfg.min_genotype_qscore >= -32768) {
        const int32_t n_k = 256, n_cov = 8192;
        if ((e = h->d_vq_tab.reserve((size_t)n_k * n_cov)) != hipSuccess || (e = h->d_sb_tab.reserve((size_t)n_k * n_cov)) != hipSuccess ||
            (e = h->d_sb0_tab.reserve((size_t)n_cov)) != hipSuccess ||
            (h->P.gq_tail && (e = h->d_gq_cap.reserve((size_t)h->P.gq_tail_a * h->P.gq_tail_cov)) != hipSuccess)) {
            g_create_error = std::string("pisces_hip_create: ") + hipGetErrorString(e);
            pisces_hip_destroy(h);
            return PISCES_E_DEVICE;
        }
        const unsigned nb = (unsigned)(((size_t)n_k * n_cov + 255) / 256);
        hipLaunchKernelGGL(build_vq_tab_kernel, dim3(nb), dim3(256), 0, h->stream, h->d_vq_tab.p, n_k, n_cov, h->P);
        hipLaunchKernelGGL(build_sb_tab_kernel, dim3(nb), dim3(256), 0, h->stream, h->d_sb_tab.p, h->d_sb0_tab.p, n_k, n_cov, h->P);
        if (h->P.gq_tail)
            hipLaunchKernelGGL(build_gq_cap_kernel, dim3((unsigned)((h->P.gq_tail_a * h->P.gq_tail_cov + 255) / 256)), dim3(256), 0, h->stream,
                               h->d_gq_cap.p, h->P.gq_tail, h->P.gq_tail_a, h->P.gq_tail_cov, h->P);
        if ((e = hipGetLastError()) != hipSuccess || (e = hipStreamSynchronize(h->stream)) != hipSuccess) {
            g_create_error = std::string("pisces_hip_create: ") + hipGetErrorString(e);
            pisces_hip_destroy(h);
            return PISCES_E_DEVICE;
        }
        h->P.vq_tab = h->d_vq_tab.p;
        h->P.sb_tab = h->d_sb_tab.p;
        h->P.sb0_tab = h->d_sb0_tab.p;
        h->P.gq_cap = h->P.gq_tail ? h->d_gq_cap.p : nullptr;
        h->P.vq_tab_k = h->P.sb_tab_k = n_k;
        h->P.tab_cov = n_cov;
        h->tables_shareable = tables_by_default && h->P.gq_tail != nullptr;
    }
    if ((e = h->d_params.reserve(1)) != hipSuccess || (e = hipMemcpy(h->d_params.p, &h->P, sizeof(DeviceParams), hipMemcpyHostToDevice)) != hipSuccess) {
        g_create_error = std::string("pisces_hip_create: ") + hipGetErrorString(e);
        pisces_hip_destroy(h);
        return PISCES_E_DEVICE;
    }
    *out = h;
    return PISCES_OK;
    });
}

int64_t pisces_hip_trim_memory(void)
{
    {
        std::lock_guard<std::mutex> lock(g_tables_mu);
        for (TableSet* t : table_cache()) delete t;
        table_cache().clear();
    }
    AllocCache& c = alloc_cache();
    std::lock_guard<std::mutex> lock(c.m);
    int dev = 0;
    (void)hipGetDevice(&dev);
    const size_t freed = cache_drop(c, -2);
    (void)hipSetDevice(dev);
    return (int64_t)freed;
}

int32_t pisces_hip_destroy(PiscesHip* h)
{
    return abi_guard<int32_t>(h, [&]() -> int32_t {
    if (!h) return PISCES_OK;
    if (h->prof_on) {
        static const char* names[19] = {"consume_found", "spanning: candidates of the batch", "spanning: counts to the host", "collapse", "device pass (MNVs)",
                                        "reallocate", "device pass (all)", "call_blocks", "row merge / genotypers", "copy out + DoneProcessing", "split: dirty loci + SNV store", "  of reallocate: mnv_reallocate_failed",
                                        "add_device_reads: consume_found", "add_device_reads: copies + checks", "add_device_reads: shape + discovery + commit",
                                        "add_reads: place + reserve", "add_reads: staging + upload", "add_reads: pass over the CIGARs", "add_reads: launches + commit"};
        for (int i = 0; i < 19; i++) fprintf(stderr, "pisces_hip host profile: %-36s %9.3f ms\n", names[i], h->prof[i] * 1e3);
        if (h->mnv_split)
            fprintf(stderr, "pisces_hip split form: %lld SNV groups into the store, %lld taken by flushes (dirty loci), %lld dropped unseen, %lld sweeps\n",
                    (long long)h->split_stats[0], (long long)h->split_stats[1], (long long)h->split_stats[2], (long long)h->split_stats[3]);
    }
    (void)hipSetDevice(h->device);
    bool idle = !h->stream || hipStreamSynchronize(h->stream) == hipSuccess;
    for (int k = 0; k < PiscesHip::kLanes; k++)
        if (h->lane[k] && hipStreamSynchronize(h->lane[k]) != hipSuccess) idle = false;
    if (h->foreign_stream_ever && hipDeviceSynchronize() != hipSuccess) idle = false;
    (void)pisces_hip_comm_destroy(h);
    struct KeepFreed {
        explicit KeepFreed(bool on) { tl_keep_freed = on; }
        ~KeepFreed() { tl_keep_freed = false; }
    } keep(idle);
    if (idle && h->tables_shareable && h->d_vq_tab.p && h->d_gq_tail.p && h->d_gq_cap.p) {
        TableSet* t = new TableSet();
        t->cfg = h->cfg;
        t->device = h->device;
        t->gq_tail.swap(h->d_gq_tail); t->vq_tab.swap(h->d_vq_tab); t->sb_tab.swap(h->d_sb_tab); t->sb0_tab.swap(h->d_sb0_tab); t->gq_cap.swap(h->d_gq_cap);
        leave_tables(t);
    }
    h->d_summary.release();
    h->d_ref.release(); h->d_tuples.release(); h->d_tiles.release(); h->d_tile_results.release();
    h->d_records.release(); h->d_counts.release(); h->d_gapped.release(); h->d_count.release(); h->d_totals.release(); h->d_qlut.release(); h->d_bq_lut.release(); h->d_sumq_fix.release(); h->d_sumq.release(); h->d_gq_tail.release(); h->d_vq_tab.release(); h->d_sb_tab.release(); h->d_sb0_tab.release(); h->d_gq_cap.release(); h->d_params.release(); h->d_offsets.release(); h->d_compact.release(); h->d_post.release(); h->d_post_compact.release();
    for (int i = 0; i < 2; i++) { h->d_log_pos[i].release(); h->d_log_tup[i].release(); }
    h->d_log_n.release(); h->d_flags.release(); h->d_bucket.release(); h->d_total.release();
    for (auto& st : h->stage) {
        st.d.release();
        if (st.h) host_free(st.h);
        st.h = nullptr;
        if (st.done) (void)hipEventDestroy(st.done);
        st.done = nullptr;
    }
    h->h_stage = nullptr;
    if (h->async.done) (void)hipEventDestroy(h->async.done);
    h->async.done = nullptr;
    if (h->h_dl) host_free(h->h_dl);
    h->h_dl = nullptr;
    if (h->h_post) host_free(h->h_post);
    h->h_post = nullptr;
    if (h->h_cand_dl) host_free(h->h_cand_dl);
    h->h_cand_dl = nullptr;
    if (h->h_meta) host_free(h->h_meta);
    h->h_meta = nullptr;
    if (h->h_counts) host_free(h->h_counts);
    h->h_counts = nullptr;
    if (h->found.h) host_free(h->found.h);
    h->found.h = nullptr;
    if (h->found.done) (void)hipEventDestroy(h->found.done);
    h->found.done = nullptr;
    if (h->found.counted) (void)hipEventDestroy(h->found.counted);
    h->found.counted = nullptr;
    if (h->found.h_totals) host_free(h->found.h_totals);
    h->found.h_totals = nullptr;
    h->d_found.release(); h->d_found_pool.release(); h->d_found_slots.release(); h->d_found_pool_first.release();
    h->d_merge_tab.release(); h->d_merge_acc.release();
    h->d_scan_sums.release(); h->d_prep_map.release(); h->d_fused_words.release(); h->d_fused_scan.release(); h->d_compact_state.release(); h->d_folded.release(); h->d_span_tiles.release();
    h->d_snv[0].release(); h->d_snv[1].release(); h->d_snv_n.release(); h->d_snv_sel.release(); h->d_dirty.release(); h->d_row_idx.release(); h->d_rows.release();
    if (h->h_totals) host_free(h->h_totals);
    if (h->h_cnt_x) host_free(h->h_cnt_x);
    h->h_totals = nullptr;
    if (h->h_prep) host_free(h->h_prep);
    h->h_prep = nullptr;
    if (h->h_snv_sel) host_free(h->h_snv_sel);
    h->h_snv_sel = nullptr;
    h->d_found_misc.release(); h->d_found_totals.release();
    h->d_cands.release(); h->d_alleles.release(); h->d_cand_records.release(); h->d_cand_callable.release();
    h->segments.clear();
    h->segment_pool.clear();
    h->state_pool.clear();
    for (hipGraphExec_t g : h->graphs) (void)hipGraphExecDestroy(g);
    for (hipGraph_t g : h->graph_defs) (void)hipGraphDestroy(g);
    for (hipEvent_t ev : h->ring) (void)hipEventDestroy(ev);
    for (hipEvent_t ev : h->ev_chain) if (ev) (void)hipEventDestroy(ev);
    if (h->ev0) (void)hipEventDestroy(h->ev0);
    if (h->ev1) (void)hipEventDestroy(h->ev1);
    for (int k = 0; k < PiscesHip::kLanes; k++)
        if (h->lane[k]) (void)hipStreamDestroy(h->lane[k]);
    if (h->stream) (void)hipStreamDestroy(h->stream);
    delete h;
    return PISCES_OK;
    });
}

const char* pisces_hip_last_error(const PiscesHip* h) { return h ? h->err.c_str() : g_create_error.c_str(); }

int32_t pisces_hip_set_reference(PiscesHip* h, const uint8_t* bases, int64_t length)
{
    return abi_guard<int32_t>(h, [&]() -> int32_t {
    if (!h) return PISCES_E_INVALID_ARG;
    if (!bases || length <= 0) return fail(h, PISCES_E_INVALID_ARG, "set_reference: empty reference");
    PISCES_HIP_CHECK(h, hipSetDevice(h->device));
    { int32_t rcf = consume_found(h); if (rcf) return rcf; }
    PISCES_HIP_CHECK(h, hipStreamSynchronize(h->stream));
    PISCES_HIP_CHECK(h, h->d_ref.reserve((size_t)length));
    PISCES_HIP_CHECK(h, hipMemcpyAsync(h->d_ref.p, bases, (size_t)length, hipMemcpyHostToDevice, h->stream));
    PISCES_HIP_CHECK(h, hipStreamSynchronize(h->stream));
    h->h_ref.assign(bases, bases + length);
    h->ref_len = length;
    return PISCES_OK;
    });
}

int32_t pisces_hip_set_intervals(PiscesHip* h, const int32_t* starts, const int32_t* ends, int32_t n)
{
    return abi_guard<int32_t>(h, [&]() -> int32_t {
    if (!h || n < 0 || (n > 0 && (!starts || !ends))) return fail(h, PISCES_E_INVALID_ARG, "set_intervals: bad arguments");
// ... 69 lines not shown
```

pisces_amd/csrc/store_kernels.hip.h:

```cpp
#pragma once
#include <hip/hip_runtime.h>
#include <stdint.h>
#include <type_traits>

#include "kernels.hip.h"
#include "read_walk.h"
#include "stream_kernels.hip.h"

#ifndef PISCES_ADD_OCC
#define PISCES_ADD_OCC 6
#endif
#ifdef PISCES_ADD_STAMPS
#define PISCES_STAMP(k, is_max) do { if (threadIdx.x == 0) A.stamps[(long long)blockIdx.x * 8 + ((k) == 0 ? 2 : (k) == 1 ? 3 : (k) - 2)] = (long long)wall_clock64(); } while (0)
#else
#define PISCES_STAMP(k, is_max) do { } while (0)
#endif
namespace pisces {

struct ReadDesc {
    int32_t pos0;
    uint32_t meta;
    int64_t aoff;
};
struct ReadExt {
// ... 1213 lines not shown
{
    const int b = t / R.tiles_per_block, i = t - b * R.tiles_per_block;
    const int step = R.tile_loci > 0 ? R.tile_loci : kTile;
    PiscesTile tile;
    tile.start_position = (R.first_key - 1 + b) * R.block_size + 1 + i * step;
    tile.n_loci = min(step, R.block_size - i * step);
    tile.tuple_begin = tile.tuple_end = 0;
    return tile;
}

__device__ __forceinline__ int xcd_tile_of_block(int b, int n)
{
    const int x = b & 7, j = b >> 3, q = n >> 3, rem = n & 7;
    return x * q + min(x, rem) + j;
}

__device__ __forceinline__ int exchanged_tile(const StoreView& S, const PiscesTile* __restrict__ tiles, const RegularTiles& R, int n_tiles, int cus, int b, int lane,
                                          int* pre_lo , int* pre_hi)
{
    *pre_lo = -1;
    *pre_hi = 0;
    const int x = b & 7, j = b >> 3, q = n_tiles >> 3, rem = n_tiles & 7;
    const int first = x * q + min(x, rem), cnt = q + (x < rem ? 1 : 0), own = first + j;
    const int s = cnt / cus, r = cnt - s * cus, k = j / cus, c = j - k * cus;
    if (k >= s || S.n_segments < 1) return own;
    int g, grp, m;
    if (r > 0) {
        g = min(cus / r, 8);
        if (g < 2) return own;
        if (c < r) { grp = c; m = 0; }
        else { const int d = c - r; grp = d / (g - 1); m = 1 + d - grp * (g - 1); if (grp >= r) return own; }
    } else {
        g = 4; grp = c >> 2; m = c & 3;
        if (grp * 4 + 4 > cus) return own;
    }
    const SegmentView& G = S.seg[0];
    if (G.n_frags <= 0 || G.state[kStateUnsorted] != 0 || !G.grid || (G.state[kStateFrags] & kGridBadBit)) return own;
    const int reach = G.state[kStateReach];
    const int i = lane & 31;
    int a = 0, t_i = own;
    if (i < g) {
        const int c_i = r > 0 ? (i == 0 ? grp : r + grp * (g - 1) + i - 1) : grp * 4 + i;
        t_i = first + k * cus + c_i;
        const int start = tiles ? tiles[t_i].start_position : regular_tile(R, t_i).start_position;
        const int tile_end = start + kTile - 1;
        const int xq = (lane >> 5) ? (tile_end == 0x7FFFFFFF ? 0x7FFFFFFF : tile_end + 1) : (int)max((long long)start - reach + 1, -0x7FFFFFFFll);
        const long long kk = (long long)max(xq, 0) - G.grid_base;
        a = kk < 0 ? 0 : G.n_frags;
        if (kk >= 0 && kk < G.grid_n) a = min(G.grid[kk], G.n_frags);
    }
    const int cost = __shfl_down(a, 32) - a;
    int rank = 0;
    for (int u = 0; u < g; u++) {
        const int cu = __builtin_amdgcn_readlane(cost, u);
        rank += (cu < cost || (cu == cost && u < i)) ? 1 : 0;
    }
    const int want = r > 0 ? (m == 0 ? 0 : 1 + (m - 1 + k) % (g - 1)) : (m + k) & 3;
    const unsigned long long hit = __ballot(lane < g && rank == want);
    if (hit == 0ull) return own;
    const int chosen = (int)__ffsll((long long)hit) - 1;
    *pre_lo = __builtin_amdgcn_readlane(a, chosen);
    *pre_hi = __builtin_amdgcn_readlane(a, chosen + 32);
    return __builtin_amdgcn_readlane(t_i, chosen);
}

__device__ __forceinline__ uint32_t allele_row_bytes(uint32_t c)
{
    return (c == 'A' ? (uint32_t)PISCES_ALLELE_A : c == 'C' ? (uint32_t)PISCES_ALLELE_C : c == 'G' ? (uint32_t)PISCES_ALLELE_G
            : c == 'T' ? (uint32_t)PISCES_ALLELE_T : (uint32_t)PISCES_ALLELE_N) * (4u * kWaveRow * (uint32_t)sizeof(int));
}

__device__ __forceinline__ uint32_t allele_row_bytes_of_base(uint32_t c)
{
    const uint32_t t8 = (c << 2) & 0x18u;
    const uint32_t letter = (0x47544341u >> t8) & 0xFFu;
    const uint32_t code = (0x01030200u >> t8) & 0xFFu;
    return (c == letter ? code : (uint32_t)PISCES_ALLELE_N) * (4u * kWaveRow * (uint32_t)sizeof(int));
}

template <int NW>
__global__ __launch_bounds__(64 * NW, NW == 1 ? PISCES_WAVE_OCC : PISCES_WAVE2_OCC) void call_store_tiles_kernel(
    StoreView S, const uint32_t* __restrict__ tuples, const PiscesTile* __restrict__ tiles , RegularTiles R, int32_t n_tiles,
    int32_t trade_cus , int32_t walk_prio, const uint8_t* __restrict__ ref, int32_t ref_start, int64_t ref_len, PiscesCalledAllele* __restrict__ records,
    PiscesTileResult* __restrict__ tile_results, DeviceParams P, const DeviceParams* __restrict__ Pd)
{
    __shared__ __attribute__((aligned(16))) int hist[2 * kWaveRegion];
    __shared__ uint8_t s_refwin[kRefWin];
    __shared__ uint8_t s_vmask[kTile];
    __shared__ unsigned long long s_masktab[kMaskTab];
    __shared__ uint2 s_pairs[NW][kPairSlots];

    if ((int)blockIdx.x >= n_tiles) return;
    int pre_lo = -1, pre_hi = 0;
    const int t = trade_cus > 0 ? exchanged_tile(S, tiles, R, n_tiles, trade_cus, (int)blockIdx.x, (int)(threadIdx.x & 63), &pre_lo, &pre_hi)
                                : xcd_tile_of_block((int)blockIdx.x, n_tiles);
    const int l = threadIdx.x & 63, wid = __builtin_amdgcn_readfirstlane((int)(threadIdx.x >> 6));
    const PiscesTile tile = tiles ? tiles[t] : regular_tile(R, t);
#ifdef PISCES_STORE_TIMING
    const long long tc0 = wall_clock64();
    long long stamps[6] = {0, 0, 0, 0, 0, 0};
#endif
    {
        int4* h4 = reinterpret_cast<int4*>(hist);
        for (int i = threadIdx.x; i < 2 * kWaveRegion / 4; i += 64 * NW) h4[i] = make_int4(0, 0, 0, 0);
        for (int i = threadIdx.x; i < kRefWin; i += 64 * NW) {
            const int64_t ri = (int64_t)tile.start_position - kRefMargin + i - ref_start;
            s_refwin[i] = (ri >= 0 && ri < ref_len) ? ref[ri] : (uint8_t)0;
        }
        for (int i = threadIdx.x; i < kMaskTab; i += 64 * NW) {
            const int a = i / 9, e = i - 9 * a;
            const unsigned long long ge_a = a >= 8 ? 0ull : ~0ull << (8 * a), ge_e = e >= 8 ? 0ull : ~0ull << (8 * e);
            s_masktab[i] = ge_a & ~ge_e;
        }
        __syncthreads();
    }
    if (walk_prio) __builtin_amdgcn_s_setprio(3);
    const uint32_t min_bq = (uint32_t)min(max(P.min_bq, 0), 127);
    char* const hbytes = reinterpret_cast<char*>(hist);
    constexpr uint32_t kRegionBytes = (uint32_t)(kWaveRegion * sizeof(int));
    for (int64_t i = tile.tuple_begin + threadIdx.x; i < tile.tuple_end; i += 64 * NW) {
        const uint32_t v = tuples[i];
        const uint32_t dir = PISCES_TUPLE_DIR(v), allele = PISCES_TUPLE_ALLELE(v);
        if (dir < 3u && allele < 6u)
            atomicAdd(reinterpret_cast<int*>(hbytes + ((PISCES_TUPLE_QUAL(v) < min_bq) ? kRegionBytes : 0u) +
                                             (uint32_t)HistLinear::idx((int)allele, (int)dir, (int)PISCES_TUPLE_LOCUS(v)) * (uint32_t)sizeof(int)), 1);
    }
    auto on_obs = [&](int position, uint32_t allele, uint32_t dir, int, uint32_t qual) {
        const uint32_t off = ((qual < min_bq) ? kRegionBytes : 0u) +
                             (uint32_t)HistLinear::idx((int)allele, (int)dir, position - tile.start_position) * (uint32_t)sizeof(int);
        atomicAdd(reinterpret_cast<int*>(hbytes + off), 1);
    };
    for (int sg = 0; sg < S.n_segments; sg++) {
        const SegmentView& G = S.seg[sg];
#ifdef PISCES_STORE_TIMING
        if (G.dirs) walk_segment_fast<true>(G, tile.start_position, min_bq, l, wid, NW, hbytes, s_masktab, s_pairs[wid], on_obs, sg == 0 ? pre_lo : -1, pre_hi, stamps);
        else walk_segment_fast<false>(G, tile.start_position, min_bq, l, wid, NW, hbytes, s_masktab, s_pairs[wid], on_obs, sg == 0 ? pre_lo : -1, pre_hi, stamps);
#else
        if (G.dirs) walk_segment_fast<true>(G, tile.start_position, min_bq, l, wid, NW, hbytes, s_masktab, s_pairs[wid], on_obs, sg == 0 ? pre_lo : -1, pre_hi);
        else walk_segment_fast<false>(G, tile.start_position, min_bq, l, wid, NW, hbytes, s_masktab, s_pairs[wid], on_obs, sg == 0 ? pre_lo : -1, pre_hi);
#endif
    }
#ifdef PISCES_STORE_TIMING
    const long long tc_walk = wall_clock64();
#endif
    __syncthreads();
    if (NW > 2 && wid != 0 && wid != NW - 1) return;
    if (walk_prio) __builtin_amdgcn_s_setprio(0);
    call_phase_wave<(NW == 1 ? 1 : 2), HistLinear>(hist, s_refwin, s_vmask, tile, t, l, NW == 1 ? 0 : (wid == NW - 1 ? 1 : 0), ref, ref_start, ref_len, records, tile_results, P
#ifdef PISCES_TIMING
                                    , 0ll, 0ll
#endif
                                    );
#ifdef PISCES_STORE_TIMING
    if (threadIdx.x == 0) {
        const long long tc_end = wall_clock64();
        int* tr = reinterpret_cast<int*>(&records[(int64_t)t * kSlotsPerTile + kSlotsPerTile - 1]);
        tr[0] = (int)(tc0 & 0x3FFFFFFF);
        tr[1] = (int)(stamps[0] & 0x3FFFFFFF);
        tr[2] = (int)(tc_walk & 0x3FFFFFFF);
        tr[3] = (int)(tc_end & 0x3FFFFFFF);
        tr[4] = (int)stamps[1];
        tr[7] = (int)stamps[2]; tr[8] = (int)stamps[3]; tr[9] = (int)stamps[4]; tr[10] = (int)stamps[5];
        tr[5] = (int)__builtin_amdgcn_s_getreg(63492);
        tr[6] = (int)__builtin_amdgcn_s_getreg(63508);
        tr[11] = (int)blockIdx.x;
    }
#endif
}

__global__ __launch_bounds__(64) void compact_small_kernel(const PiscesCalledAllele* __restrict__ records, const PiscesTileResult* __restrict__ tr,
                                                           int32_t n_tiles, PiscesCalledAllele* __restrict__ out, int32_t capacity)
{
    const int l = threadIdx.x, t = blockIdx.x;
    const int v = l < n_tiles ? tr[l].n_records : 0;
    int incl = v;
#pragma unroll
    for (int d = 1; d < 64; d <<= 1) {
        const int y = __shfl_up(incl, d, 64);
        if (l >= d) incl += y;
    }
    const int my_off = __shfl(incl - v, t, 64);
    if (t == 0) {
        int called = l < n_tiles ? tr[l].n_called : 0;
#pragma unroll
        for (int d = 32; d >= 1; d >>= 1) called += __shfl_xor(called, d, 64);
        if (l == 63) reinterpret_cast<int4*>(out)[0] = make_int4(incl, called, 0, 0);
    }
    const uint32_t nib = (tr[t].valid[l >> 3] >> ((l & 7) * 4)) & 0xFu;
    int x = __popc(nib);
    const int mine = x;
#pragma unroll
    for (int d = 1; d < 64; d <<= 1) {
        const int y = __shfl_up(x, d, 64);
        if (l >= d) x += y;
    }
    int64_t dst = (int64_t)my_off + (x - mine);
    const PiscesCalledAllele* src = records + (int64_t)tr[t].record_begin + l * 4;
    for (int k = 0; k < 4; k++) {
        if (!(nib & (1u << k))) continue;
        if (dst < capacity) copy_record(&out[1 + dst], &src[k]);
        dst++;
    }
}

__global__ __launch_bounds__(1024) void accumulate_store_tiles_kernel(StoreView S, const uint32_t* __restrict__ tuples, const PiscesTile* __restrict__ tiles,
                                                                        int32_t n_tiles, int32_t* __restrict__ counts, int32_t min_bq_,
                                                                        unsigned long long* __restrict__ sumq, const ulonglong2* __restrict__ bq_lut)
{
    __shared__ int hist[kTile * kAnchStride];
    const int t = blockIdx.x;
    if (t >= n_tiles) return;
    const PiscesTile tile = tiles[t];
    for (int i = threadIdx.x; i < kTile * kAnchStride; i += (int)blockDim.x) hist[i] = 0;
    __syncthreads();
    const uint32_t n_loci = (uint32_t)tile.n_loci, min_bq = (uint32_t)min_bq_;
    auto add = [&](uint32_t locus, uint32_t allele, uint32_t dir, uint32_t anchor, uint32_t qual) {
        if (allele < 4u && qual < min_bq) allele = 4u;
        if (locus < n_loci && dir < 3u && allele < 6u && anchor < (uint32_t)PISCES_NUM_ANCHORS) {
            atomicAdd(&hist[locus * kAnchStride + (allele * 3u + dir) * PISCES_NUM_ANCHORS + anchor], 1);
            if (sumq && allele < 4u) {
                const ulonglong2 q = bq_lut[qual];
                unsigned long long* cell = &sumq[2 * (((int64_t)t * kTile + locus) * PISCES_COUNTS_PER_LOCUS + (allele * 3u + dir) * PISCES_NUM_ANCHORS + anchor)];
                atomicAdd(cell, q.x);
                atomicAdd(cell + 1, q.y);
            }
        }
    };
    const int sub = (int)blockIdx.y, n_sub = (int)gridDim.y;
    for (int64_t i = tile.tuple_begin + (int64_t)sub * blockDim.x + threadIdx.x; i < tile.tuple_end; i += (int64_t)blockDim.x * n_sub) {
        const uint32_t v = tuples[i];
        add(PISCES_TUPLE_LOCUS(v), PISCES_TUPLE_ALLELE(v), PISCES_TUPLE_DIR(v), PISCES_TUPLE_ANCHOR(v), v >> 24);
// ... 25 lines not shown
```

pisces_amd/csrc/surface_flush.inc.h:

```cpp

static void tile_geometry(PiscesHip* h, const std::vector<int32_t>& keys, bool clip, std::vector<PiscesTile>& tiles,
                          std::vector<int32_t>& first_tile, std::vector<int32_t>& tol)
{
    tiles.clear();
    first_tile.clear();
    tol.clear();
    const int bs = h->cfg.block_size;
    const bool irregular = clip && !h->intervals.empty();
    if (irregular) tol.assign(keys.size() * (size_t)bs, -1);
    for (size_t ki = 0; ki < keys.size(); ki++) {
        const int32_t key = keys[ki];
        const int32_t bstart = (key - 1) * bs + 1, bend = key * bs;
        const size_t first = tiles.size();
        first_tile.push_back((int32_t)first);
        auto add_range = [&](int32_t s, int32_t e) {
            for (int32_t p = s; p <= e; p += kTile) {
                PiscesTile t;
                t.start_position = p;
                t.n_loci = std::min<int32_t>(kTile, e - p + 1);
                t.tuple_begin = t.tuple_end = 0;
                if (irregular)
                    for (int32_t q = 0; q < t.n_loci; q++) tol[ki * (size_t)bs + (size_t)(p + q - bstart)] = (int32_t)(tiles.size() - first);
                tiles.push_back(t);
            }
// ... 55 lines not shown
        return meta_upload(h, h->d_tiles.p, tiles.data(), tiles.size() * sizeof(PiscesTile));
    }
    BucketMap m;
    unsigned int* tile_cnt = nullptr;
    int32_t rc = upload_bucket_map(h, keys, first_tile, tol, &m, tiles.size(), &tile_cnt);
    if (rc) return rc;
    PISCES_HIP_CHECK(h, h->d_tiles.reserve(tiles.size()));
    PISCES_HIP_CHECK(h, h->d_tile_results.reserve(tiles.size()));
    PISCES_HIP_CHECK(h, h->d_count.reserve(4));
    PISCES_HIP_CHECK(h, h->d_total.reserve(2));
    const size_t tup_ub = (size_t)h->log_ub + 3 * tiles.size() + 4;
    PISCES_HIP_CHECK(h, h->d_tuples.reserve(tup_ub));
    { int32_t rcu = meta_upload(h, h->d_tiles.p, tiles.data(), tiles.size() * sizeof(PiscesTile)); if (rcu) return rcu; }
    const int c = h->log_cur;
    if (h->log_ub > 0) {
        hipLaunchKernelGGL(bucket_count_kernel, dim3(log_grid(h)), dim3(256), 0, h->stream, h->d_log_pos[c].p, (long long)h->log_ub, m,
                           tile_cnt);
    }
    hipLaunchKernelGGL(bucket_scan_kernel, dim3(1), dim3(1024), 0, h->stream, h->d_tiles.p, n_tiles, tile_cnt, h->d_total.p,
                       h->d_log_n.p + (c ^ 1));
    h->drop_counter_cleared = true;
    if (h->log_ub > 0) {
        hipLaunchKernelGGL(bucket_scatter_kernel, dim3(log_grid(h)), dim3(256), 0, h->stream, h->d_log_pos[c].p, h->d_log_tup[c].p,
                           (long long)h->log_ub, m, h->d_tiles.p, tile_cnt, h->d_tuples.p);
    }
    PISCES_HIP_CHECK(h, hipGetLastError());
    return PISCES_OK;
}

static int32_t enqueue_drop(PiscesHip* h, const std::vector<int32_t>& keys, int64_t hole_bound = -1)
{
    std::vector<int32_t> first_tile(keys.size(), 0), tol;
    BucketMap m;
    int32_t rc = upload_bucket_map(h, keys, first_tile, tol, &m);
    if (rc) return rc;
    const int c = h->log_cur, o = c ^ 1;
    PISCES_HIP_CHECK(h, h->d_log_pos[o].reserve((size_t)h->log_ub));
    PISCES_HIP_CHECK(h, h->d_log_tup[o].reserve((size_t)h->log_ub));
    if (!h->drop_counter_cleared) PISCES_HIP_CHECK(h, hipMemsetAsync(h->d_log_n.p + o, 0, sizeof(unsigned long long), h->stream));
    h->drop_counter_cleared = false;
    hipLaunchKernelGGL(log_drop_kernel, dim3(log_grid(h)), dim3(256), 0, h->stream, h->d_log_pos[c].p, h->d_log_tup[c].p, (long long)h->log_ub,
                       m, h->d_log_pos[o].p, h->d_log_tup[o].p, h->d_log_n.p + o);
    if (hole_bound > 0)
        hipLaunchKernelGGL(log_fill_holes_kernel, dim3((unsigned)((hole_bound + 255) / 256)), dim3(256), 0, h->stream, h->d_log_pos[o].p,
                           (const unsigned long long*)(h->d_log_n.p + o), (long long)hole_bound);
    PISCES_HIP_CHECK(h, hipGetLastError());
    return PISCES_OK;
}
static void commit_drop(PiscesHip* h, unsigned long long kept)
{
    h->log_cur ^= 1;
    h->log_ub = (int64_t)kept;
    h->log_known_holes = 0;
}
static int32_t drop_blocks(PiscesHip* h, const std::vector<int32_t>& keys)
{
    if (keys.empty() || h->log_ub == 0) return PISCES_OK;
    int32_t rc = enqueue_drop(h, keys);
    if (rc) return rc;
    unsigned long long kept = 0;
    PISCES_HIP_CHECK(h, hipMemcpyAsync(&kept, h->d_log_n.p + (h->log_cur ^ 1), sizeof(kept), hipMemcpyDeviceToHost, h->stream));
    PISCES_HIP_CHECK(h, hipStreamSynchronize(h->stream));
    commit_drop(h, kept);
    return PISCES_OK;
}

static hipError_t launch_call_tiles(PiscesHip* h, hipStream_t s, const uint32_t* d_tuples, const PiscesTile* d_tiles, int32_t n_tiles,
                              const uint8_t* d_ref, int32_t ref_start, int64_t ref_len, PiscesCalledAllele* d_records,
                              PiscesTileResult* d_tr, hipEvent_t e0 = nullptr, hipEvent_t e1 = nullptr)
{
    if (h->cfg.noise_model == PISCES_NOISE_WINDOW) {
        if (e0) (void)hipEventRecord(e0, s);
        hipError_t er = accumulate_tiles(h, s, d_tuples, d_tiles, n_tiles, true);
        if (er != hipSuccess) return er;
        hipLaunchKernelGGL(call_counts_kernel, dim3((unsigned)n_tiles), dim3(kBlock), 0, s, h->d_counts.p, (const uint32_t*)nullptr, d_tiles, n_tiles,
                           d_ref, ref_start, ref_len, d_records, d_tr, h->P, h->d_sumq.p);
        if (e1) (void)hipEventRecord(e1, s);
        return hipSuccess;
    }
    if (h->kernel_variant >= 2 && h->cfg.min_base_call_quality <= 255 && h->cfg.strand_bias_model != PISCES_SB_DIPLOID) {
        const bool two = h->kernel_variant == 3 || (h->kernel_variant == 4 && (int64_t)n_tiles <= (int64_t)h->n_cus * 32);
        if (!two && !e0 && !e1)
            hipLaunchKernelGGL(call_tiles_wave_kernel<1>, dim3((unsigned)n_tiles), dim3(64), 0, s, d_tuples, d_tiles, n_tiles, d_ref, ref_start, ref_len,
                               d_records, d_tr, h->P, (const DeviceParams*)h->d_params.p);
        else if (!two)
            hipExtLaunchKernelGGL(call_tiles_wave_kernel<1>, dim3((unsigned)n_tiles), dim3(64), 0, s, e0, e1, 0u, d_tuples, d_tiles,
                                  n_tiles, d_ref, ref_start, ref_len, d_records, d_tr, h->P, (const DeviceParams*)h->d_params.p);
        else if (!e0 && !e1)
            hipLaunchKernelGGL(call_tiles_wave_kernel<2>, dim3((unsigned)n_tiles), dim3(128), 0, s, d_tuples, d_tiles, n_tiles, d_ref, ref_start, ref_len,
                               d_records, d_tr, h->P, (const DeviceParams*)h->d_params.p);
        else
            hipExtLaunchKernelGGL(call_tiles_wave_kernel<2>, dim3((unsigned)n_tiles), dim3(128), 0, s, e0, e1, 0u, d_tuples, d_tiles,
                                  n_tiles, d_ref, ref_start, ref_len, d_records, d_tr, h->P, (const DeviceParams*)h->d_params.p);
        return hipSuccess;
    }
    hipExtLaunchKernelGGL(call_tiles_kernel, dim3((unsigned)n_tiles), dim3(kBlock), 0, s, e0, e1, 0u, d_tuples, d_tiles, n_tiles, d_ref,
                          ref_start, ref_len, d_records, d_tr, h->P);
    return hipSuccess;
}

static void launch_genotype_loci(PiscesHip* h, hipStream_t s, PiscesCalledAllele* d_records, PiscesTileResult* d_tr, int32_t n_tiles,
                                 PiscesGenotypePosteriors* d_posteriors = nullptr)
{
    GenotypeParams G;
    G.ploidy = h->cfg.ploidy;
    for (int k = 0; k < 3; k++) { G.snv[k] = h->cfg.diploid_snv_params[k]; G.indel[k] = h->cfg.diploid_indel_params[k]; }
    G.min_depth = h->cfg.min_coverage;
    G.min_gq = h->cfg.min_genotype_qscore;
    G.max_gq = h->cfg.max_genotype_qscore;
    G.low_gq_filter = h->cfg.low_gq_filter;
    if (n_tiles <= 0) return;
    if (h->cfg.ploidy == PISCES_PLOIDY_DIPLOID_ADAPTIVE)
        hipLaunchKernelGGL(genotype_loci_adaptive_kernel, dim3((unsigned)n_tiles), dim3(64), 0, s, d_records, d_tr, n_tiles, G, h->adaptive, d_posteriors, h->P.totals);
    else hipLaunchKernelGGL(genotype_loci_kernel, dim3((unsigned)n_tiles), dim3(64), 0, s, d_records, d_tr, n_tiles, G, h->P.totals);
}
static bool germline(const PiscesHip* h)
{
    return h->cfg.ploidy == PISCES_PLOIDY_DIPLOID || h->cfg.ploidy == PISCES_PLOIDY_HAPLOID || h->cfg.ploidy == PISCES_PLOIDY_DIPLOID_ADAPTIVE;
}

static int32_t launch_compaction(PiscesHip* h, hipStream_t s, const PiscesCalledAllele* d_records, const PiscesTileResult* d_tr, int32_t n_tiles,
                                 int32_t* d_offsets, PiscesCalledAllele* d_out, int32_t cap, int32_t* d_count, int32_t* d_called = nullptr)
{
    if (h->compact_mode == 2 || (n_tiles > kGatherDirectTiles && s != h->stream)) {
        hipLaunchKernelGGL(scan_tile_counts_kernel, dim3(1), dim3(1024), 0, s, d_tr, n_tiles, d_offsets, d_count, d_called);
        hipLaunchKernelGGL(gather_records_kernel, dim3((unsigned)n_tiles), dim3(64), 0, s, d_records, d_tr, n_tiles, d_offsets, d_out, cap);
        return PISCES_OK;
    }
    if (n_tiles <= kGatherDirectTiles && h->compact_mode != 3) {
        hipLaunchKernelGGL(gather_direct_kernel, dim3((unsigned)n_tiles), dim3(64), 0, s, d_records, d_tr, n_tiles, d_offsets, d_out, cap, d_count, d_called);
        return PISCES_OK;
    }
    const size_t groups = ((size_t)n_tiles + kCompactTiles - 1) / kCompactTiles;
    {
        const size_t before = h->d_compact_state.cap;
        PISCES_HIP_CHECK(h, h->d_compact_state.reserve(groups));
        if (h->d_compact_state.cap != before || h->compact_epoch >= (1u << 30) - 1u) {
            PISCES_HIP_CHECK(h, hipMemsetAsync(h->d_compact_state.p, 0, h->d_compact_state.cap * sizeof(unsigned long long), s));
            h->compact_epoch = 0;
        }
    }
    const uint32_t epoch = ++h->compact_epoch;
    hipLaunchKernelGGL(compact_records_kernel, dim3((unsigned)groups), dim3(256), 0, s, d_records, d_tr, n_tiles, h->d_compact_state.p, epoch, d_out, cap, d_count, d_called,
                       d_offsets);
    return PISCES_OK;
}

struct CallBlocksInFlight {
    bool active = false;
    bool drop_now = false;
    int32_t* hdr = nullptr;
    PiscesCalledAllele* hrec = nullptr;
    size_t spec = 0;
    bool posteriors = false;
    const int32_t* extra = nullptr;
};
static int32_t enqueue_off_interval_count(PiscesHip* h, const std::vector<int32_t>& keys, CallBlocksInFlight* st)
{
    const int bs = h->cfg.block_size;
    std::vector<PiscesTile> tiles;
    auto add_range = [&](int32_t s, int32_t e) {
        for (int32_t p = s; p <= e; p += kTile) {
            PiscesTile t;
            t.start_position = p;
            t.n_loci = std::min<int32_t>(kTile, e - p + 1);
            t.tuple_begin = t.tuple_end = 0;
            tiles.push_back(t);
        }
    };
    for (int32_t key : keys) {
        const int32_t bstart = (key - 1) * bs + 1, bend = (int32_t)std::min<int64_t>((int64_t)key * bs, h->ref_len);
        int32_t at = bstart;
        auto it = std::lower_bound(h->intervals.begin(), h->intervals.end(), bstart, [](const std::pair<int32_t, int32_t>& iv, int32_t p) { return iv.second < p; });
        for (; it != h->intervals.end() && it->first <= bend; ++it) {
            if (it->first > at) add_range(at, std::min(it->first - 1, bend));
            at = std::max(at, it->second + 1);
// ... 2349 lines not shown
```

pisces_amd/csrc/surface_store.inc.h:

```cpp

static int32_t store_run_deferred(PiscesHip* h)
{
    if (h->deferred_grid.empty()) return PISCES_OK;
    for (auto& d : h->deferred_grid) hipLaunchKernelGGL(read_shape_kernel, dim3(d.blocks), dim3(256), 0, h->stream, d.S);
    h->deferred_grid.clear();
    PISCES_HIP_CHECK(h, hipGetLastError());
    return PISCES_OK;
}

static void store_view(PiscesHip* h, StoreView* V)
{
    (void)store_run_deferred(h);
    std::memset(V, 0, sizeof(*V));
    int n = 0;
    for (auto& sp : h->segments) {
        const ReadSegment& g = *sp;
        if (g.n_reads == 0 || n == kMaxSegments) continue;
        SegmentView& v = V->seg[n++];
        v.frag = g.frag.p;
        v.desc = g.desc.p;
        v.ext = g.ext.p;
        v.bases = g.v_bases;
        v.quals = g.v_quals;
        v.codes = g.v_codes;
// ... 763 lines not shown
    if (rc) { store_unplace(h, pl); return rc; }
    uint8_t* const d = pl.direct ? pl.seg->blob.p : D_STAGE(h);
    const bool find_on_device = !h->h_ref.empty();
    const bool count_indels = find_on_device && !h->snv_walk;
    h->eqx_in_batch = false;
    std::vector<int32_t>& touched = h->touched_keys;
    touched.clear();
    int64_t found_slots = 0, found_pool = 0;
    int32_t max_key = 0, min_position = 0;
    ShapeArgs shape;
    bool shaped = false;
    if (rc == PISCES_OK && pl.direct) {
        const StoreBatchArrays A = {(const int32_t*)(d + L.off_pos), d + L.off_flags, (const int32_t*)(d + L.off_coff), d + L.off_cop, (const uint32_t*)(d + L.off_clen),
                                    (const int32_t*)(d + L.off_soff), d + L.off_bases, d + L.off_quals, has_dirs ? d + L.off_dirs : nullptr};
        rc = store_shape_begin(h, pl, A, nr, n_cig, n_seq, &shape);
        shaped = rc == PISCES_OK;
    }
    if (rc == PISCES_OK) rc = store_device_checks(h, d, L, nr, n_cig, n_seq, has_dirs, has_deldirs, count_indels, &found_slots, &found_pool, touched, &max_key, &min_position,
                                                  batch, shaped ? &shape : nullptr);
    prof_a.reset(new HostTimer(h->prof_on ? &h->prof[14] : nullptr));
    return store_finish_add(h, pl, rc, d, L, nr, n_cig, n_seq, has_dirs, has_deldirs, find_on_device, found_slots, found_pool, nullptr, touched, max_key, min_position,
                            shaped ? &shape : nullptr);
    });
}

static int32_t add_decoded_reads_store(PiscesHip* h, int64_t found_slots, int64_t found_pool, bool find_on_device)
{
    auto& B = h->bam;
    const int32_t nr = (int32_t)B.n_reads;
    const size_t n_cig = (size_t)B.n_ops, n_seq = (size_t)B.n_bases;
    int32_t max_key = 0;
    for (size_t w = B.block_map.size(); w-- > 0;)
        if (B.block_map[w]) { max_key = (int32_t)(w * 32 + (31 - (size_t)__builtin_clz(B.block_map[w]))) + 1; break; }
    StorePlace pl;
    { int32_t rc = store_place_batch(h, 2 * n_seq + 5 * n_cig, &pl); if (rc) return rc; }
    ReadSegment& g = *pl.seg;
    if (pl.direct) {
        g.bases.swap(B.bases);
        g.quals.swap(B.quals);
        g.cop.swap(B.cigar_op);
        g.clen.swap(B.cigar_len);
        if (B.has_dirs) g.dirs.swap(B.dirs);
        B.moved = true;
    }
    const StoreBatchArrays A = {B.position.p, B.flags.p, B.cigar_offset.p, pl.direct ? g.cop.p : B.cigar_op.p, pl.direct ? g.clen.p : B.cigar_len.p,
                                B.seq_offset.p, (pl.direct ? g.bases.p : B.bases.p) + kSegmentPad, (pl.direct ? g.quals.p : B.quals.p) + kSegmentPad,
                                B.has_dirs ? (pl.direct ? g.dirs.p : B.dirs.p) + kSegmentPad : nullptr};
    int32_t rc = store_append_arrays(h, pl, A, nr, n_cig, n_seq);
    if (rc == PISCES_OK && find_on_device && (h->snv_walk || found_slots > 0 || h->eqx_in_batch)) {
        DevReadBatch db;
        db.position = A.position; db.flags = A.flags; db.cigar_offset = A.cigar_offset; db.cigar_op = A.cigar_op; db.cigar_len = A.cigar_len;
        db.seq_offset = A.seq_offset; db.bases = A.bases; db.quals = A.quals; db.dirs = A.dirs; db.n_reads = nr;
        rc = enqueue_candidate_discovery(h, db, B.has_dirs ? B.del_dirs.p : nullptr, nr, (const int32_t*)B.d_fslots.p, found_slots, found_pool);
    }
    if (rc) {
        (void)hipStreamSynchronize(h->stream);
        if (pl.direct) { g.bases.swap(B.bases); g.quals.swap(B.quals); g.cop.swap(B.cigar_op); g.clen.swap(B.cigar_len); if (B.has_dirs) g.dirs.swap(B.dirs); B.moved = false; }
        store_unplace(h, pl);
        return rc;
    }
    g.n_reads += nr;
    g.n_bases += (int64_t)n_seq;
    g.n_ops += (int64_t)n_cig;
    g.max_key = std::max(g.max_key, max_key);
    store_maybe_seal(h, &g);
    return PISCES_OK;
}

static hipError_t launch_call_store_tiles(PiscesHip* h, hipStream_t s, const uint32_t* d_tuples, const PiscesTile* d_tiles ,
                                          const RegularTiles& R, int32_t n_tiles, const uint8_t* d_ref, int32_t ref_start, int64_t ref_len, PiscesCalledAllele* d_records, PiscesTileResult* d_tr,
                                          hipEvent_t e0 = nullptr, hipEvent_t e1 = nullptr)
{
    StoreView V;
    store_view(h, &V);
    int nw = h->store_waves;
    if (nw == 0) nw = h->kernel_variant == 2 ? 1 : h->kernel_variant == 3 ? 2 : (int64_t)n_tiles <= (int64_t)h->n_cus ? 16
                      : (int64_t)n_tiles * 4 <= (int64_t)h->n_cus * 12 ? 4 : (int64_t)n_tiles <= (int64_t)h->n_cus * 32 ? 2 : 1;
    int32_t trade_cus = 0;
    if (h->trade_tiles && nw <= 2 && (int64_t)n_tiles >= 4 * (int64_t)h->n_cus && (int64_t)n_tiles <= 8 * (int64_t)h->n_cus && h->n_cus >= 8)
        trade_cus = (int32_t)(h->n_cus / 8);
    const int32_t walk_prio = (nw == 2 && (int64_t)n_tiles <= 8 * (int64_t)h->n_cus) ? 1 : 0;
#define PISCES_LAUNCH_STORE(NW)                                                                                                                     \
    hipExtLaunchKernelGGL(call_store_tiles_kernel<NW>, dim3((unsigned)n_tiles), dim3(64 * NW), 0u, s, e0, e1, 0u, V, d_tuples, d_tiles, R, n_tiles, trade_cus, walk_prio, d_ref, \
                          ref_start, ref_len, d_records, d_tr, h->P, (const DeviceParams*)h->d_params.p)
    if (nw >= 16) PISCES_LAUNCH_STORE(16);
    else if (nw >= 8) PISCES_LAUNCH_STORE(8);
    else if (nw >= 4) PISCES_LAUNCH_STORE(4);
    else if (nw >= 2) PISCES_LAUNCH_STORE(2);
    else PISCES_LAUNCH_STORE(1);
#undef PISCES_LAUNCH_STORE
    return hipGetLastError();
}
```

Baseline: 2.566 billion candidate loci/s.

## Add compact call params and precomputed cap thresholds for table-driven allele calls

Introduces a slim CallParams kernel argument built from DeviceParams, with booleans packed into a flags word and fixed table dimensions baked in as constants. Adds per-coverage threshold tables (cap_from), built once at setup, so the VQ cap and strand-bias saturation checks become a single load and compare instead of double-precision log-bound math. A branch-light call_allele_from_tables path issues its table loads up front. The aims are lower kernel-argument and register pressure and less divergent f64 work in the call phase, at the cost of an extra setup kernel, more device memory, and a narrowed sb_threshold (now float).

```diff
diff --git a/pisces_amd/csrc/device_math.hip.h b/pisces_amd/csrc/device_math.hip.h
--- a/pisces_amd/csrc/device_math.hip.h
+++ b/pisces_amd/csrc/device_math.hip.h
@@ -27,6 +27,8 @@
     const double* sb0_tab;
     const int16_t* gq_cap;
     int32_t vq_tab_k, sb_tab_k, tab_cov;
+    const uint16_t* vq_cap_from;
+    const uint16_t* sb_one_from;
     const uint32_t* dirty_bits;
     int32_t dirty_first, dirty_n;
     int32_t* folded_out;
@@ -262,6 +264,17 @@
 }
 __device__ __forceinline__ double ln_ratio_lower_bound(double a, double x) { return (double)(ilogb(a) - ilogb(x) - 1) * 0.6931471805; }
 
+__device__ __forceinline__ bool vq_cap_proof(int32_t callCount, int32_t coverage, double err_q, int32_t max_vq)
+{
+    const double lambda = err_q * coverage;
+    if (max_vq <= 110 && callCount >= 3 && (double)callCount >= 2.0 * lambda) {
+        const double km1 = callCount - 1;
+        const double need = ((double)max_vq + 1.0) * 0.23025850929940458 + 1e-3;
+        if (km1 * (ln_ratio_lower_bound(km1, lambda) - 1.0) >= need) return true;
+    }
+    return false;
+}
+
 __device__ __forceinline__ bool poisson_qscore_try(int32_t callCount, int32_t coverage, const DeviceParams& P, int32_t& vq)
 {
     if ((callCount <= 0) || (coverage <= 0)) { vq = 0; return true; }
@@ -269,12 +282,7 @@
         vq = P.vq_tab[(uint32_t)callCount * (uint32_t)P.tab_cov + (uint32_t)coverage];
         return true;
     }
-    const double lambda = P.err_q * coverage;
-    if (P.max_vq <= 110 && callCount >= 3 && (double)callCount >= 2.0 * lambda) {
-        const double km1 = callCount - 1;
-        const double need = ((double)P.max_vq + 1.0) * 0.23025850929940458 + 1e-3;
-        if (km1 * (ln_ratio_lower_bound(km1, lambda) - 1.0) >= need) { vq = P.max_vq; return true; }
-    }
+    if (vq_cap_proof(callCount, coverage, P.err_q, P.max_vq)) { vq = P.max_vq; return true; }
     return false;
 }
 
@@ -405,21 +413,24 @@
     return f < 1.0f ? f : 1.0f;
 }
 
-__device__ inline int32_t somatic_genotype(bool isReference, int32_t cov, int32_t support, int32_t refSupport,
-                                           const DeviceParams& P)
-{
-    if (cov < P.min_cov) return isReference ? PISCES_GT_REF_LIKE_NOCALL : PISCES_GT_ALT_LIKE_NOCALL;
-    float freq = frequency_f(support, cov);
+__device__ __forceinline__ int32_t somatic_genotype_f(bool isReference, int32_t cov, float freq, int32_t refSupport, int32_t min_cov,
+                                                      float gt_min_freq)
+{
+    if (cov < min_cov) return isReference ? PISCES_GT_REF_LIKE_NOCALL : PISCES_GT_ALT_LIKE_NOCALL;
     if (!isReference) {
-        if (frequency_f(refSupport, cov) < P.gt_min_freq) {
-            if ((1 - freq) > P.gt_min_freq) return PISCES_GT_ALT_AND_NOCALL;
+        if (frequency_f(refSupport, cov) < gt_min_freq) {
+            if ((1 - freq) > gt_min_freq) return PISCES_GT_ALT_AND_NOCALL;
             return PISCES_GT_HOM_ALT;
         }
         return PISCES_GT_HET_ALT_REF;
     }
-    if (freq < P.gt_min_freq) return PISCES_GT_REF_LIKE_NOCALL;
-    if ((1 - freq) > P.gt_min_freq) return PISCES_GT_REF_AND_NOCALL;
+    if (freq < gt_min_freq) return PISCES_GT_REF_LIKE_NOCALL;
+    if ((1 - freq) > gt_min_freq) return PISCES_GT_REF_AND_NOCALL;
     return PISCES_GT_HOM_REF;
+}
+__device__ inline int32_t somatic_genotype(bool isReference, int32_t cov, int32_t support, int32_t refSupport, const DeviceParams& P)
+{
+    return somatic_genotype_f(isReference, cov, frequency_f(support, cov), refSupport, P.min_cov, P.gt_min_freq);
 }
 
 __device__ __noinline__ double poisson_cdf_out_of_line(double num_occurrences, double expected)
@@ -470,6 +481,12 @@
     return somatic_gq_finish(genotype, variantQ, cov, t, P);
 }
 
+__device__ __forceinline__ bool sb_one_proof(int32_t support, int32_t coverage, double err_sb)
+{
+    const double a = (double)support, x = (double)coverage * err_sb;
+    return x > 0.0 && 2.0 * x <= a && a * (ln_ratio_lower_bound(a, x) - 1.0) + x > 51.0;
+}
+
 __device__ __forceinline__ bool sb_stats_try(int32_t support, int32_t coverage, const DeviceParams& P, SbStats& st)
 {
     st.support = (double)support;
@@ -488,8 +505,7 @@
     if (P.sb_tab && support > 0 && support < P.sb_tab_k && coverage >= 0 && coverage < P.tab_cov) {
         st.var_gt_zero = P.sb_tab[(uint32_t)support * (uint32_t)P.tab_cov + (uint32_t)coverage];
     } else {
-        const double a = (double)support, x = (double)coverage * P.err_sb;
-        if (!(x > 0.0 && 2.0 * x <= a && a * (ln_ratio_lower_bound(a, x) - 1.0) + x > 51.0)) return false;
+        if (!sb_one_proof(support, coverage, P.err_sb)) return false;
         st.var_gt_zero = 1.0;
     }
     st.false_pos = fmax(0.0, 1 - st.var_gt_zero);
@@ -523,32 +539,44 @@
     return ok0 && ok1 && ok2;
 }
 
-__device__ __forceinline__ int32_t somatic_gq_index(int32_t genotype, int32_t cov, int32_t support, const DeviceParams& P)
+__device__ __forceinline__ int32_t somatic_gq_index_f(int32_t genotype, int32_t cov, float freq, float target_lod, int32_t gq_tail_a,
+                                                      int32_t gq_tail_cov)
 {
     if (cov == 0 || !((genotype == PISCES_GT_HOM_REF) || (genotype == PISCES_GT_HOM_ALT))) return -1;
-    const float nonAlleleObservationsF = (1.0f - frequency_f(support, cov)) * (float)cov;
-    const float expectedNonAllelObservationsF = P.target_lod * (float)cov;
+    const float nonAlleleObservationsF = (1.0f - freq) * (float)cov;
+    const float expectedNonAllelObservationsF = target_lod * (float)cov;
     if (nonAlleleObservationsF >= expectedNonAllelObservationsF) return -1;
     const int ai = (int)((double)nonAlleleObservationsF + 1.0);
-    if (ai >= 1 && ai < P.gq_tail_a && cov < P.gq_tail_cov) return ai * P.gq_tail_cov + cov;
+    if (ai >= 1 && ai < gq_tail_a && cov < gq_tail_cov) return ai * gq_tail_cov + cov;
     return -1;
+}
+__device__ __forceinline__ int32_t somatic_gq_index(int32_t genotype, int32_t cov, int32_t support, const DeviceParams& P)
+{
+    return somatic_gq_index_f(genotype, cov, frequency_f(support, cov), P.target_lod, P.gq_tail_a, P.gq_tail_cov);
+}
+__device__ __forceinline__ bool somatic_gq_try_f(int32_t genotype, int32_t variantQ, int32_t cov, float freq, int32_t min_gq, int32_t max_gq,
+                                                 int32_t max_vq, float target_lod, bool have_gq_cap, int32_t gq_index,
+                                                 int32_t gq_cap_value , int32_t& gq)
+{
+    const bool noCall = (genotype == PISCES_GT_ALT12_LIKE_NOCALL || genotype == PISCES_GT_ALT_LIKE_NOCALL || genotype == PISCES_GT_REF_LIKE_NOCALL);
+    if ((cov == 0) || noCall) { gq = min_gq; return true; }
+    if ((genotype == PISCES_GT_HOM_REF) || (genotype == PISCES_GT_HOM_ALT)) {
+        if (gq_index >= 0 && variantQ == max_vq && have_gq_cap) { gq = gq_cap_value; return true; }
+        const float nonAlleleObservationsF = (1.0f - freq) * (float)cov;
+        const float expectedNonAllelObservationsF = target_lod * (float)cov;
+        if (nonAlleleObservationsF >= expectedNonAllelObservationsF) { gq = min_gq; return true; }
+        return false;
+    }
+    double qScore = fmin((double)max_gq, (double)variantQ);
+    qScore = fmax(qScore, (double)min_gq);
+    gq = (int32_t)rint(qScore);
+    return true;
 }
 __device__ __forceinline__ bool somatic_gq_try(int32_t genotype, int32_t variantQ, int32_t cov, int32_t support, const DeviceParams& P,
                                                int32_t gq_index, int32_t gq_cap_value , int32_t& gq)
 {
-    const bool noCall = (genotype == PISCES_GT_ALT12_LIKE_NOCALL || genotype == PISCES_GT_ALT_LIKE_NOCALL || genotype == PISCES_GT_REF_LIKE_NOCALL);
-    if ((cov == 0) || noCall) { gq = P.min_gq; return true; }
-    if ((genotype == PISCES_GT_HOM_REF) || (genotype == PISCES_GT_HOM_ALT)) {
-        if (gq_index >= 0 && variantQ == P.max_vq && P.gq_cap) { gq = gq_cap_value; return true; }
-        const float nonAlleleObservationsF = (1.0f - frequency_f(support, cov)) * (float)cov;
-        const float expectedNonAllelObservationsF = P.target_lod * (float)cov;
-        if (nonAlleleObservationsF >= expectedNonAllelObservationsF) { gq = P.min_gq; return true; }
-        return false;
-    }
-    double qScore = fmin((double)P.max_gq, (double)variantQ);
-    qScore = fmax(qScore, (double)P.min_gq);
-    gq = (int32_t)rint(qScore);
-    return true;
+    return somatic_gq_try_f(genotype, variantQ, cov, frequency_f(support, cov), P.min_gq, P.max_gq, P.max_vq, P.target_lod, P.gq_cap != nullptr,
+                            gq_index, gq_cap_value, gq);
 }
 
 struct AlleleTables {
@@ -595,12 +623,7 @@
 {
     if ((callCount <= 0) || (coverage <= 0)) { vq = 0; return true; }
     if (t.have & 1u) { vq = t.vq; return true; }
-    const double lambda = P.err_q * coverage;
-    if (P.max_vq <= 110 && callCount >= 3 && (double)callCount >= 2.0 * lambda) {
-        const double km1 = callCount - 1;
-        const double need = ((double)P.max_vq + 1.0) * 0.23025850929940458 + 1e-3;
-        if (km1 * (ln_ratio_lower_bound(km1, lambda) - 1.0) >= need) { vq = P.max_vq; return true; }
-    }
+    if (vq_cap_proof(callCount, coverage, P.err_q, P.max_vq)) { vq = P.max_vq; return true; }
     return false;
 }
 
@@ -622,12 +645,25 @@
     if (have) {
         st.var_gt_zero = value;
     } else {
-        const double a = (double)support, x = (double)coverage * P.err_sb;
-        if (!(x > 0.0 && 2.0 * x <= a && a * (ln_ratio_lower_bound(a, x) - 1.0) + x > 51.0)) return false;
+        if (!sb_one_proof(support, coverage, P.err_sb)) return false;
         st.var_gt_zero = 1.0;
     }
     st.false_pos = fmax(0.0, 1 - st.var_gt_zero);
     return true;
+}
+
+__device__ __forceinline__ double sb_bias_score(double ov_var, double fw_var, double fw_fp, double rv_var, double rv_fp)
+{
+    double forwardBias = 0.0, reverseBias = 0.0;
+    if (!(fw_fp == 0.0 && rv_fp == 0.0 && ov_var > 0.0)) {
+        forwardBias = (fw_var * rv_fp) / ov_var;
+        reverseBias = (rv_var * fw_fp) / ov_var;
+        if (ov_var == 0) {
+            forwardBias = 1;
+            reverseBias = 1;
+        }
+    }
+    return forwardBias > reverseBias ? forwardBias : reverseBias;
 }
 
 __device__ __forceinline__ bool strand_bias_try(const int32_t cov[3], const int32_t sup[3], const DeviceParams& P, const AlleleTables& t,
@@ -639,22 +675,108 @@
     const bool ok0 = sb_stats_try(sup[0] + sup[1] + sup[2], cov[0] + cov[1] + cov[2], P, (t.have & 2u) != 0, t.sb[0], overall);
     const bool ok1 = sb_stats_try(sf, cf, P, (t.have & 4u) != 0, t.sb[1], fwd);
     const bool ok2 = sb_stats_try(sr, cr, P, (t.have & 8u) != 0, t.sb[2], rev);
-    double forwardBias = 0.0, reverseBias = 0.0;
-    if (!(fwd.false_pos == 0.0 && rev.false_pos == 0.0 && overall.var_gt_zero > 0.0)) {
-        forwardBias = (fwd.var_gt_zero * rev.false_pos) / overall.var_gt_zero;
-        reverseBias = (rev.var_gt_zero * fwd.false_pos) / overall.var_gt_zero;
-        if (overall.var_gt_zero == 0) {
-            forwardBias = 1;
-            reverseBias = 1;
-        }
-    }
-    double score = forwardBias > reverseBias ? forwardBias : reverseBias;
+    double score = sb_bias_score(overall.var_gt_zero, fwd.var_gt_zero, fwd.false_pos, rev.var_gt_zero, rev.false_pos);
     cov_both = (cf > 0) && (cr > 0);
     var_both = (sf > 0) && (sr > 0);
     if (!cov_both) score = 0;
     bias_score = score;
     acceptable = score < P.sb_threshold;
     return ok0 && ok1 && ok2;
+}
+
+constexpr int32_t kTabK = 256, kTabCov = 8192, kGqTailA = 32, kGqTailCov = 8192;
+constexpr uint32_t kCallIncludeRef = 1u, kCallEmitZeroCov = 2u, kCallFilterSingleStrand = 4u, kCallRefsOnly = 8u, kCallVariantsOnly = 16u,
+                   kCallSbPoisson = 32u, kCallRmxn = 64u , kCallTables = 128u ;
+struct CallParams {
+    int32_t min_bq, noise_level, max_vq, min_vq, vq_filter, min_cov, low_depth_filter, min_gq, max_gq, low_gq_filter, rmxn_min_rep;
+    uint32_t flags;
+    float min_freq, vf_filter, gt_min_freq, target_lod, nocall_thr, rmxn_freq_limit, sb_threshold;
+    int32_t dirty_first, dirty_n, folded_first, folded_n;
+    unsigned long long* totals;
+    const int16_t* vq_tab;
+    const double* sb_tab;
+    const double* sb0_tab;
+    const int16_t* gq_cap;
+    const uint16_t* cap_from;
+    const uint32_t* dirty_bits;
+    int32_t* folded_out;
+};
+inline CallParams make_call_params(const DeviceParams& P)
+{
+    CallParams Q;
+    Q.min_bq = P.min_bq; Q.noise_level = P.noise_level; Q.max_vq = P.max_vq; Q.min_vq = P.min_vq; Q.vq_filter = P.vq_filter;
+    Q.min_cov = P.min_cov; Q.low_depth_filter = P.low_depth_filter; Q.min_gq = P.min_gq; Q.max_gq = P.max_gq;
+    Q.low_gq_filter = P.low_gq_filter; Q.rmxn_min_rep = P.rmxn_min_rep;
+    const bool tables = P.vq_tab && P.sb_tab && P.sb0_tab && P.gq_cap && P.vq_cap_from && P.sb_one_from == P.vq_cap_from + kTabCov &&
+                        P.vq_tab_k == kTabK && P.sb_tab_k == kTabK && P.tab_cov == kTabCov && P.gq_tail_a == kGqTailA && P.gq_tail_cov == kGqTailCov;
+    Q.flags = (P.include_ref ? kCallIncludeRef : 0u) | (P.emit_zero_cov ? kCallEmitZeroCov : 0u) | (P.filter_single_strand ? kCallFilterSingleStrand : 0u) |
+              (P.refs_only ? kCallRefsOnly : 0u) | (P.variants_only ? kCallVariantsOnly : 0u) | (P.sb_model == PISCES_SB_POISSON ? kCallSbPoisson : 0u) |
+              (P.rmxn_max_len >= 1 ? kCallRmxn : 0u) | (tables ? kCallTables : 0u);
+    Q.min_freq = P.min_freq; Q.vf_filter = P.vf_filter; Q.gt_min_freq = P.gt_min_freq; Q.target_lod = P.target_lod; Q.nocall_thr = P.nocall_thr;
+    Q.rmxn_freq_limit = P.rmxn_freq_limit;
+    Q.sb_threshold = (float)P.sb_threshold;
+    Q.dirty_first = P.dirty_first; Q.dirty_n = P.dirty_n; Q.folded_first = P.folded_first; Q.folded_n = P.folded_n;
+    Q.totals = P.totals;
+    Q.vq_tab = P.vq_tab; Q.sb_tab = P.sb_tab; Q.sb0_tab = P.sb0_tab; Q.gq_cap = P.gq_cap; Q.cap_from = P.vq_cap_from;
+    Q.dirty_bits = P.dirty_bits; Q.folded_out = P.folded_out;
+    return Q;
+}
+
+__device__ __forceinline__ bool locus_is_dirty(const CallParams& Q, int pos)
+{
+    if (!Q.dirty_bits) return false;
+    const unsigned rel = (unsigned)(pos - Q.dirty_first);
+    return rel < (unsigned)Q.dirty_n && ((Q.dirty_bits[rel >> 5] >> (rel & 31u)) & 1u) != 0u;
+}
+
+struct AlleleCall { int32_t vq, gq, gt; double sb_score; int sb_ok, sb_var, sb_cov; bool callable; };
+__device__ __forceinline__ bool call_allele_from_tables(bool isRef, int32_t support, int32_t total, int32_t refsup, const int32_t cov[3],
+                                                        const int32_t sup[3], float freq, const CallParams& Q, AlleleCall& out)
+{
+    out.gt = somatic_genotype_f(isRef, total, freq, refsup, Q.min_cov, Q.gt_min_freq);
+    const int32_t gq_idx = somatic_gq_index_f(out.gt, total, freq, Q.target_lod, kGqTailA, kGqTailCov);
+    const bool vq_in = support > 0 && total > 0 && support < kTabK && total < kTabCov;
+    const int16_t vq_v = Q.vq_tab[vq_in ? (uint32_t)support * (uint32_t)kTabCov + (uint32_t)total : 0u];
+    const bool vq_thr = total >= 0 && total < kTabCov && support <= total;
+    const uint32_t vq_from = Q.cap_from[vq_thr ? (uint32_t)total : 0u];
+    const int s2 = sup[2] / 2, c2 = cov[2] / 2;
+    const int sf = sup[0] + s2, sr = sup[1] + s2, cf = cov[0] + c2, cr = cov[1] + c2;
+    const bool poisson = (Q.flags & kCallSbPoisson) != 0;
+    struct Stat { double var, fp; bool known; };
+    auto sb_stat = [&](int ss, int cc) -> Stat {
+        const bool zero = ss == 0, cc_in = cc >= 0 && cc < kTabCov;
+        const bool in = zero ? (!poisson && cc_in) : (ss > 0 && ss < kTabK && cc_in);
+        const double* base = zero ? Q.sb0_tab : Q.sb_tab;
+        const double v = base[in ? (zero ? (uint32_t)cc : (uint32_t)ss * (uint32_t)kTabCov + (uint32_t)cc) : 0u];
+        const bool thr = !zero && !in && cc_in && ss > 0 && ss <= cc;
+        const uint32_t from = Q.cap_from[(uint32_t)kTabCov + (thr ? (uint32_t)cc : 0u)];
+        const bool one = thr && (uint32_t)ss >= from;
+        const double var = in ? v : 1.0;
+        Stat st = {var, zero ? 1 - var : fmax(0.0, 1 - var), in || one};
+        if (zero && poisson) { st.var = 0; st.fp = 1; st.known = true; }
+        return st;
+    };
+    const Stat ov = sb_stat(sup[0] + sup[1] + sup[2], cov[0] + cov[1] + cov[2]), fw = sb_stat(sf, cf), rv = sb_stat(sr, cr);
+    const int16_t gq_v = Q.gq_cap[gq_idx >= 0 ? gq_idx : 0];
+    out.callable = true;
+    out.vq = 0;
+    if (support > 0 && total > 0) {
+        if (vq_in) out.vq = vq_v;
+        else if (vq_thr && (uint32_t)support >= vq_from) out.vq = Q.max_vq;
+        else return false;
+    }
+    if (!isRef && out.vq < Q.min_vq) { out.callable = false; return true; }
+    out.sb_score = 0.0; out.sb_ok = 0; out.sb_var = 0; out.sb_cov = 0;
+    if (support > 0) {
+        if (!(ov.known && fw.known && rv.known)) return false;
+        double score = sb_bias_score(ov.var, fw.var, fw.fp, rv.var, rv.fp);
+        out.sb_cov = (cf > 0) && (cr > 0);
+        out.sb_var = (sf > 0) && (sr > 0);
+        if (!out.sb_cov) score = 0;
+        out.sb_score = score;
+        out.sb_ok = score < (double)Q.sb_threshold;
+    }
+    return somatic_gq_try_f(out.gt, out.vq, total, freq, Q.min_gq, Q.max_gq, Q.max_vq, Q.target_lod, true, gq_idx, (int32_t)gq_v, out.gq);
 }
 
 __device__ __noinline__ int32_t poisson_qscore_out_of_line(int32_t callCount, int32_t coverage, double err, int32_t max_vq, double ln10)
@@ -718,24 +840,29 @@
     return cnt;
 }
 
-__device__ inline bool rmxn_should_filter_snv_lds(const uint8_t* win, int n, int idx ,
-                                                  uint8_t refBase, uint8_t altBase, float freq, const DeviceParams& P)
-{
-    if (P.rmxn_max_len < 1) return false;
-    if (freq >= P.rmxn_freq_limit) return false;
+__device__ inline bool rmxn_should_filter_snv_lds(const uint8_t* win, int n, int idx , uint8_t refBase,
+                                                  uint8_t altBase, float freq, int32_t rmxn_max_len, int32_t rmxn_min_rep, float rmxn_freq_limit)
+{
+    if (rmxn_max_len < 1) return false;
+    if (freq >= rmxn_freq_limit) return false;
     if (idx >= 4 && idx + 4 < n) {
         const bool l1 = win[idx - 1] == refBase, l2 = win[idx - 2] == refBase, l3 = win[idx - 3] == refBase, l4 = win[idx - 4] == refBase;
         const bool r1 = win[idx + 1] == refBase, r2 = win[idx + 2] == refBase, r3 = win[idx + 3] == refBase, r4 = win[idx + 4] == refBase;
         const int left = !l1 ? 0 : !l2 ? 1 : !l3 ? 2 : !l4 ? 3 : 4;
         const int right = !r1 ? 0 : !r2 ? 1 : !r3 ? 2 : !r4 ? 3 : 4;
-        if (left < 4 && right < 4 && 1 + left + right < P.rmxn_min_rep) return false;
+        if (left < 4 && right < 4 && 1 + left + right < rmxn_min_rep) return false;
     }
     int c1 = rmxn_run_lds(win, n, idx, refBase);
-    if (c1 < P.rmxn_min_rep) return false;
+    if (c1 < rmxn_min_rep) return false;
     int i1 = rmxn_run_lds(win, n, idx + 1, altBase);
     int i2 = rmxn_run_lds(win, n, idx, altBase);
     int c2 = i1 > i2 ? i1 : i2;
-    return (c1 < c2 ? c1 : c2) >= P.rmxn_min_rep;
-}
-
-}
+    return (c1 < c2 ? c1 : c2) >= rmxn_min_rep;
+}
+__device__ inline bool rmxn_should_filter_snv_lds(const uint8_t* win, int n, int idx, uint8_t refBase, uint8_t altBase, float freq,
+                                                  const DeviceParams& P)
+{
+    return rmxn_should_filter_snv_lds(win, n, idx, refBase, altBase, freq, P.rmxn_max_len, P.rmxn_min_rep, P.rmxn_freq_limit);
+}
+
+}
diff --git a/pisces_amd/csrc/kernels.hip.h b/pisces_amd/csrc/kernels.hip.h
--- a/pisces_amd/csrc/kernels.hip.h
+++ b/pisces_amd/csrc/kernels.hip.h
@@ -26,12 +26,15 @@
 
 typedef uint32_t u32x4 __attribute__((ext_vector_type(4)));
 
-__device__ __forceinline__ int allele_of_rank(int k) { return k == 1 ? 2 : (k == 2 ? 1 : k); }
-__device__ __forceinline__ int rank_of_allele(int a) { return a == 1 ? 2 : (a == 2 ? 1 : a); }
+__device__ __forceinline__ int allele_of_rank(int k) { return (int)((0x76543120u >> (4 * (k & 7))) & 0xFu); }
+__device__ __forceinline__ int rank_of_allele(int a) { return (int)((0x76543120u >> (4 * (a & 7))) & 0xFu); }
 
 __device__ __forceinline__ int allele_type_of_base(uint8_t c)
 {
-    return c == 'A' ? 0 : c == 'G' ? 1 : c == 'C' ? 2 : c == 'T' ? 3 : 4;
+    const uint32_t t8 = ((uint32_t)c << 2) & 0x18u;
+    const uint32_t letter = (0x47544341u >> t8) & 0xFFu;
+    const uint32_t code = (0x01030200u >> t8) & 0xFFu;
+    return (uint32_t)c == letter ? (int)code : 4;
 }
 
 __device__ __forceinline__ void accumulate_folded(int* hist, uint32_t t, uint32_t n_loci, uint32_t min_bq)
@@ -161,53 +164,36 @@
     return point_counts_of(load_counts<H>(hist, l), allele, isRef, refType, gapped);
 }
 
+__device__ __forceinline__ bool variant_passes_frequency_f(int32_t total, float freq, int32_t min_cov, bool include_ref, float min_freq)
+{
+    if (total < min_cov && !include_ref) return false;
+    if (total != 0 && freq < min_freq) return false;
+    return true;
+}
 __device__ __forceinline__ bool variant_passes_frequency(const PointCounts& c, const DeviceParams& P)
 {
-    if (c.total < P.min_cov && !P.include_ref) return false;
-    if (c.total != 0 && frequency_f(c.support, c.total) < P.min_freq) return false;
-    return true;
-}
-
-struct GqPre { int32_t idx, val; };
-template <bool kMemo = false>
-__device__ inline bool finish_allele(const PointCounts& c, int pos, int a, bool isRef, int rt, int vq, const SbResult& sb,
-                                     const uint8_t* __restrict__ ref, int64_t win_lo, int64_t win_hi, const DeviceParams& P,
-                                     PiscesCalledAllele& r, const uint8_t* s_refwin, int s_refidx,
-                                     const GqTail* pre_tail = nullptr, const GqPre* pre_gq = nullptr,
-                                     const int32_t* window_level_ = nullptr )
-{
-    const float freq = frequency_f(c.support, c.total);
-    const float allReads = (float)(c.total + c.nocalls);
-    const float fractionNoCalls = (allReads == 0.0f) ? 0.0f : ((float)c.nocalls / allReads);
+    return variant_passes_frequency_f(c.total, frequency_f(c.support, c.total), P.min_cov, P.include_ref != 0, P.min_freq);
+}
+
+struct FilterSettings { int32_t low_depth_filter, vq_filter, low_gq_filter; float nocall_thr, vf_filter; bool filter_single_strand; };
+__device__ __forceinline__ void filter_and_pack_allele(const PointCounts& c, int pos, int a, bool isRef, int rt, int vq, int gq, int gt, float freq,
+                                                       const SbResult& sb, bool rmxn_hit, int16_t noise_level, const FilterSettings& F,
+                                                       PiscesCalledAllele& r)
+{
     uint32_t filters = 0;
-    if (P.low_depth_filter >= 0 && c.total < P.low_depth_filter) filters |= 1u << PISCES_FILTER_LOW_DEPTH;
-    if (P.vq_filter >= 0 && vq < P.vq_filter && c.total != 0) filters |= 1u << PISCES_FILTER_LOW_VARIANT_QSCORE;
+    if (F.low_depth_filter >= 0 && c.total < F.low_depth_filter) filters |= 1u << PISCES_FILTER_LOW_DEPTH;
+    if (F.vq_filter >= 0 && vq < F.vq_filter && c.total != 0) filters |= 1u << PISCES_FILTER_LOW_VARIANT_QSCORE;
     if (!isRef) {
-        if (P.nocall_thr >= 0.0f && fractionNoCalls > P.nocall_thr) filters |= 1u << PISCES_FILTER_NO_CALL;
-        if (!sb.acceptable || (P.filter_single_strand && !sb.var_both)) filters |= 1u << PISCES_FILTER_STRAND_BIAS;
-        auto base_of = [](int code) { return (uint8_t)((0x54434741u >> (8 * code)) & 0xFFu); };
-        if (rt < 4 && a < 4) {
-            const bool hit = (s_refwin && P.rmxn_min_rep <= kRefMargin)
-                                 ? rmxn_should_filter_snv_lds(s_refwin, kRefWin, s_refidx, base_of(rt), base_of(a), freq, P)
-                                 : rmxn_should_filter_snv(ref, win_lo, win_hi, pos, base_of(rt), base_of(a), freq, P);
-            if (hit) filters |= 1u << PISCES_FILTER_RMXN;
-        }
-        if (P.vf_filter >= 0.0f && freq < P.vf_filter) filters |= 1u << PISCES_FILTER_LOW_VARIANT_FREQUENCY;
-    }
-    const int gt = somatic_genotype(isRef, c.total, c.support, c.refsup, P);
-    int gq;
-    if (kMemo) {
-        GqPre g;
-        if (pre_gq) g = *pre_gq;
-        else {
-            g.idx = somatic_gq_index(gt, c.total, c.support, P);
-            g.val = (g.idx >= 0 && P.gq_cap) ? (int32_t)P.gq_cap[g.idx] : 0;
-        }
-        if (!somatic_gq_try(gt, vq, c.total, c.support, P, g.idx, g.val, gq)) return false;
-    } else {
-        gq = pre_tail ? somatic_gq_finish(gt, vq, c.total, *pre_tail, P) : somatic_gq(gt, vq, c.total, c.support, P);
-    }
-    if (P.low_gq_filter >= 0 && (float)gq < (float)P.low_gq_filter) filters |= 1u << PISCES_FILTER_LOW_GENOTYPE_QUALITY;
+        if (F.nocall_thr >= 0.0f) {
+            const float allReads = (float)(c.total + c.nocalls);
+            const float fractionNoCalls = (allReads == 0.0f) ? 0.0f : ((float)c.nocalls / allReads);
+            if (fractionNoCalls > F.nocall_thr) filters |= 1u << PISCES_FILTER_NO_CALL;
+        }
+        if (!sb.acceptable || (F.filter_single_strand && !sb.var_both)) filters |= 1u << PISCES_FILTER_STRAND_BIAS;
+        if (rmxn_hit) filters |= 1u << PISCES_FILTER_RMXN;
+        if (F.vf_filter >= 0.0f && freq < F.vf_filter) filters |= 1u << PISCES_FILTER_LOW_VARIANT_FREQUENCY;
+    }
+    if (F.low_gq_filter >= 0 && (float)gq < (float)F.low_gq_filter) filters |= 1u << PISCES_FILTER_LOW_GENOTYPE_QUALITY;
 
     r.position = pos;
     r.total_coverage = c.total;
@@ -219,10 +205,44 @@
     r.variant_qscore = vq;
     r.strand_bias_score = sb.bias_score;
     r.genotype_qscore = (int16_t)gq;
-    r.noise_level = c.support > 0 ? (window_level_ ? noise_level_field(*window_level_) : (int16_t)P.noise_level) : (int16_t)0;
+    r.noise_level = c.support > 0 ? noise_level : (int16_t)0;
     r.filter_bits = (uint16_t)filters;
     r.info = PISCES_INFO_PACK(gt, isRef ? PISCES_CAT_REFERENCE : PISCES_CAT_SNV, rt, isRef ? rt : a, sb.acceptable, sb.var_both,
                               sb.cov_both);
+}
+__device__ __forceinline__ uint8_t base_of_allele(int code) { return (uint8_t)((0x54434741u >> (8 * code)) & 0xFFu); }
+
+struct GqPre { int32_t idx, val; };
+template <bool kMemo = false>
+__device__ inline bool finish_allele(const PointCounts& c, int pos, int a, bool isRef, int rt, int vq, const SbResult& sb,
+                                     const uint8_t* __restrict__ ref, int64_t win_lo, int64_t win_hi, const DeviceParams& P,
+                                     PiscesCalledAllele& r, const uint8_t* s_refwin, int s_refidx,
+                                     const GqTail* pre_tail = nullptr, const GqPre* pre_gq = nullptr,
+                                     const int32_t* window_level_ = nullptr )
+{
+    const float freq = frequency_f(c.support, c.total);
+    bool rmxn_hit = false;
+    if (!isRef && rt < 4 && a < 4) {
+        rmxn_hit = (s_refwin && P.rmxn_min_rep <= kRefMargin)
+                       ? rmxn_should_filter_snv_lds(s_refwin, kRefWin, s_refidx, base_of_allele(rt), base_of_allele(a), freq, P)
+                       : rmxn_should_filter_snv(ref, win_lo, win_hi, pos, base_of_allele(rt), base_of_allele(a), freq, P);
+    }
+    const int gt = somatic_genotype(isRef, c.total, c.support, c.refsup, P);
+    int gq;
+    if (kMemo) {
+        GqPre g;
+        if (pre_gq) g = *pre_gq;
+        else {
+            g.idx = somatic_gq_index(gt, c.total, c.support, P);
+            g.val = (g.idx >= 0 && P.gq_cap) ? (int32_t)P.gq_cap[g.idx] : 0;
+        }
+        if (!somatic_gq_try(gt, vq, c.total, c.support, P, g.idx, g.val, gq)) return false;
+    } else {
+        gq = pre_tail ? somatic_gq_finish(gt, vq, c.total, *pre_tail, P) : somatic_gq(gt, vq, c.total, c.support, P);
+    }
+    const FilterSettings F = {P.low_depth_filter, P.vq_filter, P.low_gq_filter, P.nocall_thr, P.vf_filter, P.filter_single_strand != 0};
+    filter_and_pack_allele(c, pos, a, isRef, rt, vq, gq, gt, freq, sb, rmxn_hit,
+                           window_level_ ? noise_level_field(*window_level_) : (int16_t)P.noise_level, F, r);
     return true;
 }
 
@@ -553,7 +573,8 @@
 __device__ __forceinline__ void call_phase_wave(const int* hist, const uint8_t* s_refwin, uint8_t* s_vmask, const PiscesTile& tile, const int t,
                                                 const int l, const int wid, const uint8_t* __restrict__ ref, const int32_t ref_start,
                                                 const int64_t ref_len, PiscesCalledAllele* __restrict__ records,
-                                                PiscesTileResult* __restrict__ tile_results, const DeviceParams& P
+                                                PiscesTileResult* __restrict__ tile_results, const CallParams& Q,
+                                                const DeviceParams* __restrict__ Pd
 #ifdef PISCES_TIMING
                                                 , const long long tc0, const long long tc1
 #endif
@@ -563,15 +584,14 @@
     const uint8_t refb = s_refwin[kRefMargin + l];
     const bool in_ref = l < tile.n_loci && refb != 0;
     const int rt = in_ref ? allele_type_of_base(refb) : PISCES_ALLELE_N;
-    const int64_t win_lo = (int64_t)ref_start - 1, win_hi = win_lo + ref_len;
     auto slot_of = [&](int k) { return records + ((int64_t)t * kSlotsPerTile + l * 4 + k); };
-    const bool dirty = locus_is_dirty(P, pos);
+    const bool dirty = locus_is_dirty(Q, pos);
     const LocusCounts lc = load_counts_wave<H>(hist, l);
     const bool ref_wave = wid == 0, var_wave = wid == NW - 1;
-    if (P.folded_out && ref_wave && l < tile.n_loci) {
-        const unsigned rel = (unsigned)(pos - P.folded_first);
-        if (rel < (unsigned)P.folded_n) {
-            int32_t* const dst = P.folded_out + (size_t)rel * PISCES_FOLDED_PER_LOCUS;
+    if (Q.folded_out && ref_wave && l < tile.n_loci) {
+        const unsigned rel = (unsigned)(pos - Q.folded_first);
+        if (rel < (unsigned)Q.folded_n) {
+            int32_t* const dst = Q.folded_out + (size_t)rel * PISCES_FOLDED_PER_LOCUS;
 #pragma unroll
             for (int a = 0; a < 6; a++)
 #pragma unroll
@@ -579,20 +599,19 @@
         }
     }
 
-    const bool tabs = tables_complete(P);
-    auto fast_allele = [&](const PointCounts& c, int a, bool isRef, PiscesCalledAllele& rec) -> bool {
-        int vq = 0;
-        double sb_score = 0.0;
-        int sb_ok = 0, sb_var = 0, sb_cov = 0;
-        if (!tabs) return false;
-        const AlleleTables tb = request_allele_tables(isRef, c.support, c.total, c.refsup, c.cov, c.sup, P);
-        if (c.support > 0 && c.total != 0 && !poisson_qscore_try(c.support, c.total, P, tb, vq)) return false;
-        if (!isRef && vq < P.min_vq) return true;
-        if (c.support > 0 && !strand_bias_try(c.cov, c.sup, P, tb, sb_score, sb_ok, sb_var, sb_cov)) return false;
-        const GqPre g = {tb.gq_idx, tb.gq_cap};
-        const SbResult sb = {sb_score, sb_ok, sb_var, sb_cov};
-        if (!finish_allele<true>(c, pos, a, isRef, rt, vq, sb, ref, win_lo, win_hi, P, rec, s_refwin, kRefMargin + l, nullptr, &g)) return false;
-        return true;
+    const bool tabs = (Q.flags & kCallTables) != 0;
+    auto fast_allele = [&](const PointCounts& c, int a, bool isRef, float freq, PiscesCalledAllele& r) -> int {
+        if (!tabs) return 0;
+        AlleleCall ac;
+        if (!call_allele_from_tables(isRef, c.support, c.total, c.refsup, c.cov, c.sup, freq, Q, ac)) return 0;
+        if (!ac.callable) return 2;
+        const bool rmxn_hit = !isRef && rt < 4 && a < 4 &&
+                              rmxn_should_filter_snv_lds(s_refwin, kRefWin, kRefMargin + l, base_of_allele(rt), base_of_allele(a), freq,
+                                                         (Q.flags & kCallRmxn) ? 1 : 0, Q.rmxn_min_rep, Q.rmxn_freq_limit);
+        const FilterSettings F = {Q.low_depth_filter, Q.vq_filter, Q.low_gq_filter, Q.nocall_thr, Q.vf_filter, (Q.flags & kCallFilterSingleStrand) != 0};
+        const SbResult sb = {ac.sb_score, ac.sb_ok, ac.sb_var, ac.sb_cov};
+        filter_and_pack_allele(c, pos, a, isRef, rt, ac.vq, ac.gq, ac.gt, freq, sb, rmxn_hit, (int16_t)Q.noise_level, F, r);
+        return 1;
     };
     bool ref_emitted = false;
     int ref_rank = 0;
@@ -601,35 +620,39 @@
     const int ref_a = (rt < 4) ? rt : PISCES_ALLELE_N;
     if (ref_wave) {
         const PointCounts c = point_counts_of(lc, ref_a, true, rt, 0);
-        if (in_ref && P.include_ref && !P.variants_only && (P.emit_zero_cov || c.total + c.nocalls > 0)) {
+        if (in_ref && (Q.flags & (kCallIncludeRef | kCallVariantsOnly)) == kCallIncludeRef && ((Q.flags & kCallEmitZeroCov) || c.total + c.nocalls > 0)) {
             ref_rank = (rt < 4) ? rank_of_allele(rt) : 0;
             ref_emitted = true;
             PiscesCalledAllele rec;
-            if (fast_allele(c, ref_a, true, rec)) copy_record(slot_of(ref_rank), &rec);
+            if (fast_allele(c, ref_a, true, frequency_f(c.support, c.total), rec) == 1) copy_record(slot_of(ref_rank), &rec);
             else slow |= 16u;
         }
     }
 #ifdef PISCES_TIMING
     const long long tcA = wall_clock64();
 #endif
-    if (var_wave && in_ref && rt < 4 && !P.refs_only && !dirty) {
+    if (var_wave && in_ref && rt < 4 && !(Q.flags & kCallRefsOnly) && !dirty) {
+        const bool rmxn_far = (Q.flags & kCallRmxn) && Q.rmxn_min_rep > kRefMargin;
 #pragma unroll 1
         for (int k = 0; k < 4; k++) {
             const int a = allele_of_rank(k);
             if (a == rt) continue;
             const PointCounts c = point_counts_of(lc, a, false, rt, 0);
             if (c.support == 0) continue;
-            if (!variant_passes_frequency(c, P)) continue;
+            const float freq = frequency_f(c.support, c.total);
+            if (!variant_passes_frequency_f(c.total, freq, Q.min_cov, (Q.flags & kCallIncludeRef) != 0, Q.min_freq)) continue;
             PiscesCalledAllele r;
-            r.position = 0;
-            if (!fast_allele(c, a, false, r)) { slow |= 1u << k; continue; }
-            if (r.position == 0) continue;
+            const int made = rmxn_far ? 0 : fast_allele(c, a, false, freq, r);
+            if (made == 0) { slow |= 1u << k; continue; }
+            if (made == 2) continue;
             copy_record(slot_of(k), &r);
             vmask |= 1u << k;
         }
     }
-    if (__builtin_expect(__ballot(slow != 0) != 0ull, 0))
-        vmask |= slow_alleles<H>(hist, s_refwin, slow, l, pos, rt, ref_rank, ref, win_lo, win_hi, records + ((int64_t)t * kSlotsPerTile + l * 4), P);
+    if (__builtin_expect(__ballot(slow != 0) != 0ull, 0)) {
+        const int64_t win_lo = (int64_t)ref_start - 1, win_hi = win_lo + ref_len;
+        vmask |= slow_alleles<H>(hist, s_refwin, slow, l, pos, rt, ref_rank, ref, win_lo, win_hi, records + ((int64_t)t * kSlotsPerTile + l * 4), *Pd);
+    }
     if (NW == 2) {
         if (var_wave) s_vmask[l] = (uint8_t)vmask;
         __syncthreads();
@@ -660,8 +683,8 @@
         tile_result->n_records = n_surv;
         tile_result->n_candidate_loci = n_loci_called;
         tile_result->n_called = n_call_total;
-        if (P.totals) {
-            unsigned long long* tt = P.totals + (size_t)(t % kTotalShards) * kTotalStride;
+        if (Q.totals) {
+            unsigned long long* tt = Q.totals + (size_t)(t % kTotalShards) * kTotalStride;
             atomicAdd(&tt[0], (unsigned long long)n_surv);
             atomicAdd(&tt[1], (unsigned long long)n_loci_called);
             atomicAdd(&tt[2], (unsigned long long)n_call_total);
@@ -687,7 +710,8 @@
 __global__ __launch_bounds__(64 * NW, NW == 1 ? PISCES_WAVE_OCC : PISCES_WAVE2_OCC) void call_tiles_wave_kernel(
     const uint32_t* __restrict__ tuples, const PiscesTile* __restrict__ tiles, int32_t n_tiles,
     const uint8_t* __restrict__ ref, int32_t ref_start, int64_t ref_len, PiscesCalledAllele* __restrict__ records,
-    PiscesTileResult* __restrict__ tile_results, DeviceParams P, const DeviceParams* __restrict__ Pd )
+    PiscesTileResult* __restrict__ tile_results, CallParams Q ,
+    const DeviceParams* __restrict__ Pd )
 {
     __shared__ __attribute__((aligned(16))) int hist[2 * kWaveRegion];
     __shared__ uint8_t s_refwin[kRefWin];
@@ -712,7 +736,7 @@
 
     {
         if (NW == 2) __builtin_amdgcn_s_setprio(3);
-        const uint32_t min_bq_shifted = (uint32_t)min(max(P.min_bq, 0), 255) << 24;
+        const uint32_t min_bq_shifted = (uint32_t)min(max(Q.min_bq, 0), 255) << 24;
         stream_tuples_wave<NW>(tuples, tile.tuple_begin, tile.tuple_end, l, wid, [&](uint32_t v) { accumulate_wave(hist, v, min_bq_shifted); }, setup);
     }
     __syncthreads();
@@ -721,7 +745,7 @@
     const long long tc1 = wall_clock64();
 #endif
 
-    call_phase_wave<NW>(hist, s_refwin, s_vmask, tile, t, l, wid, ref, ref_start, ref_len, records, tile_results, P
+    call_phase_wave<NW>(hist, s_refwin, s_vmask, tile, t, l, wid, ref, ref_start, ref_len, records, tile_results, Q, Pd
 #ifdef PISCES_TIMING
                         , tc0, tc1
 #endif
@@ -741,6 +765,25 @@
     const int k = (int)(i / n_cov), cov = (int)(i % n_cov);
     tab[i] = k >= 1 ? fmax(0.0, poisson_cdf_sb((double)k - 1, (double)cov * P.err_sb)) : 0.0;
     if (k == 0) tab0[cov] = pow(1 - P.err_sb, (double)cov);
+}
+__global__ __launch_bounds__(64) void build_cap_from_kernel(uint16_t* __restrict__ vq_cap_from, uint16_t* __restrict__ sb_one_from, int32_t n_cov, DeviceParams P)
+{
+    const int cov = (int)blockIdx.x, l = (int)threadIdx.x;
+    if (cov >= n_cov) return;
+    int vq_fail = 0, sb_fail = 0;
+    for (int s = 1 + l; s <= cov; s += 64) {
+        if (!vq_cap_proof(s, cov, P.err_q, P.max_vq)) vq_fail = s;
+        if (!sb_one_proof(s, cov, P.err_sb)) sb_fail = s;
+    }
+#pragma unroll
+    for (int d = 32; d >= 1; d >>= 1) {
+        vq_fail = max(vq_fail, __shfl_xor(vq_fail, d, 64));
+        sb_fail = max(sb_fail, __shfl_xor(sb_fail, d, 64));
+    }
+    if (l == 0) {
+        vq_cap_from[cov] = (uint16_t)((cov == 0 || vq_fail >= cov) ? 0xFFFF : vq_fail + 1);
+        sb_one_from[cov] = (uint16_t)((cov == 0 || sb_fail >= cov) ? 0xFFFF : sb_fail + 1);
+    }
 }
 __global__ __launch_bounds__(256) void build_gq_cap_kernel(int16_t* __restrict__ tab, const double* __restrict__ gq_tail, int32_t n_a, int32_t n_cov, DeviceParams P)
 {
diff --git a/pisces_amd/csrc/pisces_hip.hip b/pisces_amd/csrc/pisces_hip.hip
--- a/pisces_amd/csrc/pisces_hip.hip
+++ b/pisces_amd/csrc/pisces_hip.hip
@@ -292,6 +292,7 @@
     DeviceBuf<double> d_sb_tab;
     DeviceBuf<double> d_sb0_tab;
     DeviceBuf<int16_t> d_gq_cap;
+    DeviceBuf<uint16_t> d_cap_from;
     DeviceBuf<DeviceParams> d_params;
     int n_cus = 256;
     void* comm = nullptr;
@@ -658,6 +659,7 @@
     P.sb0_tab = nullptr;
     P.gq_cap = nullptr;
     P.vq_tab_k = P.sb_tab_k = P.tab_cov = 0;
+    P.vq_cap_from = P.sb_one_from = nullptr;
     P.dirty_bits = nullptr;
     P.dirty_first = P.dirty_n = 0;
     P.folded_out = nullptr;
@@ -683,6 +685,7 @@
     int device = 0;
     DeviceBuf<double> gq_tail, sb_tab, sb0_tab;
     DeviceBuf<int16_t> vq_tab, gq_cap;
+    DeviceBuf<uint16_t> cap_from;
 };
 std::mutex g_tables_mu;
 std::vector<TableSet*>& table_cache() { static std::vector<TableSet*>* v = new std::vector<TableSet*>(); return *v; }
@@ -866,15 +869,16 @@
                                    h->cfg.min_genotype_qscore >= -32768;
     std::unique_ptr<TableSet> kept(tables_by_default ? take_tables(h->cfg, h->device) : nullptr);
     if (kept) {
-        h->d_gq_tail.swap(kept->gq_tail); h->d_vq_tab.swap(kept->vq_tab); h->d_sb_tab.swap(kept->sb_tab); h->d_sb0_tab.swap(kept->sb0_tab); h->d_gq_cap.swap(kept->gq_cap);
-        h->P.gq_tail = h->d_gq_tail.p; h->P.gq_tail_a = 32; h->P.gq_tail_cov = 8192;
+        h->d_gq_tail.swap(kept->gq_tail); h->d_vq_tab.swap(kept->vq_tab); h->d_sb_tab.swap(kept->sb_tab); h->d_sb0_tab.swap(kept->sb0_tab); h->d_gq_cap.swap(kept->gq_cap); h->d_cap_from.swap(kept->cap_from);
+        h->P.gq_tail = h->d_gq_tail.p; h->P.gq_tail_a = kGqTailA; h->P.gq_tail_cov = kGqTailCov;
         h->P.vq_tab = h->d_vq_tab.p; h->P.sb_tab = h->d_sb_tab.p; h->P.sb0_tab = h->d_sb0_tab.p; h->P.gq_cap = h->d_gq_cap.p;
-        h->P.vq_tab_k = h->P.sb_tab_k = 256;
-        h->P.tab_cov = 8192;
+        h->P.vq_tab_k = h->P.sb_tab_k = kTabK;
+        h->P.tab_cov = kTabCov;
+        h->P.vq_cap_from = h->d_cap_from.p; h->P.sb_one_from = h->d_cap_from.p + kTabCov;
         h->tables_shareable = true;
     }
     if (!kept && !getenv("PISCES_HIP_NO_GQ_TABLE")) {
-        const int32_t n_a = 32, n_cov = 8192;
+        const int32_t n_a = kGqTailA, n_cov = kGqTailCov;
         if ((e = h->d_gq_tail.reserve((size_t)n_a * n_cov)) != hipSuccess) {
             g_create_error = std::string("pisces_hip_create: ") + hipGetErrorString(e);
             pisces_hip_destroy(h);
@@ -893,9 +897,9 @@
     }
     if (!kept && !getenv("PISCES_HIP_NO_CALL_TABLES") && h->cfg.noise_model == PISCES_NOISE_FLAT && h->cfg.strand_bias_model != PISCES_SB_DIPLOID &&
         h->cfg.max_variant_qscore <= 32767 && h->cfg.max_genotype_qscore <= 32767 && h->cfg.min_genotype_qscore >= -32768) {
-        const int32_t n_k = 256, n_cov = 8192;
+        const int32_t n_k = kTabK, n_cov = kTabCov;
         if ((e = h->d_vq_tab.reserve((size_t)n_k * n_cov)) != hipSuccess || (e = h->d_sb_tab.reserve((size_t)n_k * n_cov)) != hipSuccess ||
-            (e = h->d_sb0_tab.reserve((size_t)n_cov)) != hipSuccess ||
+            (e = h->d_sb0_tab.reserve((size_t)n_cov)) != hipSuccess || (e = h->d_cap_from.reserve((size_t)2 * n_cov)) != hipSuccess ||
             (h->P.gq_tail && (e = h->d_gq_cap.reserve((size_t)h->P.gq_tail_a * h->P.gq_tail_cov)) != hipSuccess)) {
             g_create_error = std::string("pisces_hip_create: ") + hipGetErrorString(e);
             pisces_hip_destroy(h);
@@ -904,6 +908,7 @@
         const unsigned nb = (unsigned)(((size_t)n_k * n_cov + 255) / 256);
         hipLaunchKernelGGL(build_vq_tab_kernel, dim3(nb), dim3(256), 0, h->stream, h->d_vq_tab.p, n_k, n_cov, h->P);
         hipLaunchKernelGGL(build_sb_tab_kernel, dim3(nb), dim3(256), 0, h->stream, h->d_sb_tab.p, h->d_sb0_tab.p, n_k, n_cov, h->P);
+        hipLaunchKernelGGL(build_cap_from_kernel, dim3((unsigned)n_cov), dim3(64), 0, h->stream, h->d_cap_from.p, h->d_cap_from.p + n_cov, n_cov, h->P);
         if (h->P.gq_tail)
             hipLaunchKernelGGL(build_gq_cap_kernel, dim3((unsigned)((h->P.gq_tail_a * h->P.gq_tail_cov + 255) / 256)), dim3(256), 0, h->stream,
                                h->d_gq_cap.p, h->P.gq_tail, h->P.gq_tail_a, h->P.gq_tail_cov, h->P);
@@ -918,6 +923,8 @@
         h->P.gq_cap = h->P.gq_tail ? h->d_gq_cap.p : nullptr;
         h->P.vq_tab_k = h->P.sb_tab_k = n_k;
         h->P.tab_cov = n_cov;
+        h->P.vq_cap_from = h->d_cap_from.p;
+        h->P.sb_one_from = h->d_cap_from.p + n_cov;
         h->tables_shareable = tables_by_default && h->P.gq_tail != nullptr;
     }
     if ((e = h->d_params.reserve(1)) != hipSuccess || (e = hipMemcpy(h->d_params.p, &h->P, sizeof(DeviceParams), hipMemcpyHostToDevice)) != hipSuccess) {
@@ -970,16 +977,16 @@
         explicit KeepFreed(bool on) { tl_keep_freed = on; }
         ~KeepFreed() { tl_keep_freed = false; }
     } keep(idle);
-    if (idle && h->tables_shareable && h->d_vq_tab.p && h->d_gq_tail.p && h->d_gq_cap.p) {
+    if (idle && h->tables_shareable && h->d_vq_tab.p && h->d_gq_tail.p && h->d_gq_cap.p && h->d_cap_from.p) {
         TableSet* t = new TableSet();
         t->cfg = h->cfg;
         t->device = h->device;
-        t->gq_tail.swap(h->d_gq_tail); t->vq_tab.swap(h->d_vq_tab); t->sb_tab.swap(h->d_sb_tab); t->sb0_tab.swap(h->d_sb0_tab); t->gq_cap.swap(h->d_gq_cap);
+        t->gq_tail.swap(h->d_gq_tail); t->vq_tab.swap(h->d_vq_tab); t->sb_tab.swap(h->d_sb_tab); t->sb0_tab.swap(h->d_sb0_tab); t->gq_cap.swap(h->d_gq_cap); t->cap_from.swap(h->d_cap_from);
         leave_tables(t);
     }
     h->d_summary.release();
     h->d_ref.release(); h->d_tuples.release(); h->d_tiles.release(); h->d_tile_results.release();
-    h->d_records.release(); h->d_counts.release(); h->d_gapped.release(); h->d_count.release(); h->d_totals.release(); h->d_qlut.release(); h->d_bq_lut.release(); h->d_sumq_fix.release(); h->d_sumq.release(); h->d_gq_tail.release(); h->d_vq_tab.release(); h->d_sb_tab.release(); h->d_sb0_tab.release(); h->d_gq_cap.release(); h->d_params.release(); h->d_offsets.release(); h->d_compact.release(); h->d_post.release(); h->d_post_compact.release();
+    h->d_records.release(); h->d_counts.release(); h->d_gapped.release(); h->d_count.release(); h->d_totals.release(); h->d_qlut.release(); h->d_bq_lut.release(); h->d_sumq_fix.release(); h->d_sumq.release(); h->d_gq_tail.release(); h->d_vq_tab.release(); h->d_sb_tab.release(); h->d_sb0_tab.release(); h->d_gq_cap.release(); h->d_cap_from.release(); h->d_params.release(); h->d_offsets.release(); h->d_compact.release(); h->d_post.release(); h->d_post_compact.release();
     for (int i = 0; i < 2; i++) { h->d_log_pos[i].release(); h->d_log_tup[i].release(); }
     h->d_log_n.release(); h->d_flags.release(); h->d_bucket.release(); h->d_total.release();
     for (auto& st : h->stage) {
diff --git a/pisces_amd/csrc/store_kernels.hip.h b/pisces_amd/csrc/store_kernels.hip.h
--- a/pisces_amd/csrc/store_kernels.hip.h
+++ b/pisces_amd/csrc/store_kernels.hip.h
@@ -1319,7 +1319,7 @@
 __global__ __launch_bounds__(64 * NW, NW == 1 ? PISCES_WAVE_OCC : PISCES_WAVE2_OCC) void call_store_tiles_kernel(
     StoreView S, const uint32_t* __restrict__ tuples, const PiscesTile* __restrict__ tiles , RegularTiles R, int32_t n_tiles,
     int32_t trade_cus , int32_t walk_prio, const uint8_t* __restrict__ ref, int32_t ref_start, int64_t ref_len, PiscesCalledAllele* __restrict__ records,
-    PiscesTileResult* __restrict__ tile_results, DeviceParams P, const DeviceParams* __restrict__ Pd)
+    PiscesTileResult* __restrict__ tile_results, CallParams Q, const DeviceParams* __restrict__ Pd)
 {
     __shared__ __attribute__((aligned(16))) int hist[2 * kWaveRegion];
     __shared__ uint8_t s_refwin[kRefWin];
@@ -1352,7 +1352,7 @@
         __syncthreads();
     }
     if (walk_prio) __builtin_amdgcn_s_setprio(3);
-    const uint32_t min_bq = (uint32_t)min(max(P.min_bq, 0), 127);
+    const uint32_t min_bq = (uint32_t)min(max(Q.min_bq, 0), 127);
     char* const hbytes = reinterpret_cast<char*>(hist);
     constexpr uint32_t kRegionBytes = (uint32_t)(kWaveRegion * sizeof(int));
     for (int64_t i = tile.tuple_begin + threadIdx.x; i < tile.tuple_end; i += 64 * NW) {
@@ -1383,7 +1383,7 @@
     __syncthreads();
     if (NW > 2 && wid != 0 && wid != NW - 1) return;
     if (walk_prio) __builtin_amdgcn_s_setprio(0);
-    call_phase_wave<(NW == 1 ? 1 : 2), HistLinear>(hist, s_refwin, s_vmask, tile, t, l, NW == 1 ? 0 : (wid == NW - 1 ? 1 : 0), ref, ref_start, ref_len, records, tile_results, P
+    call_phase_wave<(NW == 1 ? 1 : 2), HistLinear>(hist, s_refwin, s_vmask, tile, t, l, NW == 1 ? 0 : (wid == NW - 1 ? 1 : 0), ref, ref_start, ref_len, records, tile_results, Q, Pd
 #ifdef PISCES_TIMING
                                     , 0ll, 0ll
 #endif
diff --git a/pisces_amd/csrc/surface_flush.inc.h b/pisces_amd/csrc/surface_flush.inc.h
--- a/pisces_amd/csrc/surface_flush.inc.h
+++ b/pisces_amd/csrc/surface_flush.inc.h
@@ -161,16 +161,16 @@
         const bool two = h->kernel_variant == 3 || (h->kernel_variant == 4 && (int64_t)n_tiles <= (int64_t)h->n_cus * 32);
         if (!two && !e0 && !e1)
             hipLaunchKernelGGL(call_tiles_wave_kernel<1>, dim3((unsigned)n_tiles), dim3(64), 0, s, d_tuples, d_tiles, n_tiles, d_ref, ref_start, ref_len,
-                               d_records, d_tr, h->P, (const DeviceParams*)h->d_params.p);
+                               d_records, d_tr, make_call_params(h->P), (const DeviceParams*)h->d_params.p);
         else if (!two)
             hipExtLaunchKernelGGL(call_tiles_wave_kernel<1>, dim3((unsigned)n_tiles), dim3(64), 0, s, e0, e1, 0u, d_tuples, d_tiles,
-                                  n_tiles, d_ref, ref_start, ref_len, d_records, d_tr, h->P, (const DeviceParams*)h->d_params.p);
+                                  n_tiles, d_ref, ref_start, ref_len, d_records, d_tr, make_call_params(h->P), (const DeviceParams*)h->d_params.p);
         else if (!e0 && !e1)
             hipLaunchKernelGGL(call_tiles_wave_kernel<2>, dim3((unsigned)n_tiles), dim3(128), 0, s, d_tuples, d_tiles, n_tiles, d_ref, ref_start, ref_len,
-                               d_records, d_tr, h->P, (const DeviceParams*)h->d_params.p);
+                               d_records, d_tr, make_call_params(h->P), (const DeviceParams*)h->d_params.p);
         else
             hipExtLaunchKernelGGL(call_tiles_wave_kernel<2>, dim3((unsigned)n_tiles), dim3(128), 0, s, e0, e1, 0u, d_tuples, d_tiles,
-                                  n_tiles, d_ref, ref_start, ref_len, d_records, d_tr, h->P, (const DeviceParams*)h->d_params.p);
+                                  n_tiles, d_ref, ref_start, ref_len, d_records, d_tr, make_call_params(h->P), (const DeviceParams*)h->d_params.p);
         return hipSuccess;
     }
     hipExtLaunchKernelGGL(call_tiles_kernel, dim3((unsigned)n_tiles), dim3(kBlock), 0, s, e0, e1, 0u, d_tuples, d_tiles, n_tiles, d_ref,
diff --git a/pisces_amd/csrc/surface_store.inc.h b/pisces_amd/csrc/surface_store.inc.h
--- a/pisces_amd/csrc/surface_store.inc.h
+++ b/pisces_amd/csrc/surface_store.inc.h
@@ -869,7 +869,7 @@
     const int32_t walk_prio = (nw == 2 && (int64_t)n_tiles <= 8 * (int64_t)h->n_cus) ? 1 : 0;
 #define PISCES_LAUNCH_STORE(NW)                                                                                                                     \
     hipExtLaunchKernelGGL(call_store_tiles_kernel<NW>, dim3((unsigned)n_tiles), dim3(64 * NW), 0u, s, e0, e1, 0u, V, d_tuples, d_tiles, R, n_tiles, trade_cus, walk_prio, d_ref, \
-                          ref_start, ref_len, d_records, d_tr, h->P, (const DeviceParams*)h->d_params.p)
+                          ref_start, ref_len, d_records, d_tr, make_call_params(h->P), (const DeviceParams*)h->d_params.p)
     if (nw >= 16) PISCES_LAUNCH_STORE(16);
     else if (nw >= 8) PISCES_LAUNCH_STORE(8);
     else if (nw >= 4) PISCES_LAUNCH_STORE(4);
```

Measured after the change: 2.620 billion candidate loci/s (median of 6 runs). 2.1% higher.
